# tinycrops/x-transformers-rl

Hardware: AMD Instinct MI355X
Metric: env-steps/s (rollout+update) (higher is better)
Workload: dtype f32; 1 GPU; C3: LunarLander-shaped VecSim (S=8, A=4, hazard 1/64), 1024 episodes x 128 steps per update per GPU, depth-4 d=256 4x16-head gated value-residual world-model policy, batch 128 episodes, 4 epochs, dropout 0.25; no EPO (BASELINE.json configs[2] names no gene pool: one policy, actor / critic heads on [embed | state embed], in = 2d); global_batch=1024, seq_len=128, parallelism=dp1, env_steps=1302236

## Files before the change

### include/xtrl_hip.h

```cpp
#ifndef XTRL_HIP_H
#define XTRL_HIP_H

#include <stdint.h>

#ifdef __cplusplus
extern "C" {
#endif

#define XTRL_OK 0
#define XTRL_E_ARG 1
#define XTRL_E_HIP 2

#define XTRL_ABI_VERSION 25

int xtrl_abi_version(void);
int64_t xtrl_struct_size(const char* name);
const char* xtrl_last_error(void);
const char* xtrl_source_hash(void);

#define XTRL_ACT_NONE 0
#define XTRL_ACT_GELU 1
#define XTRL_ACT_SILU 2
#define XTRL_ACT_RELU 3

int xtrl_gemm_f32(const float* X, int ldx, const float* W, int ldw, const float* bias, const float* ln_gamma,
                  const float* R, int ldr, float* Y, int ldy, const int32_t* t_dev, int64_t y_t_stride, int M,
                  int N, int K, int act, void* stream);

int xtrl_gemm_ex(int trans_a, int trans_b, const float* A, int lda, const float* B, int ldb, const float* bias,
                 float* C, int ldc, int M, int N, int K, float beta, void* stream);

int xtrl_gemm_wgrad(const float* dY, int ldy, const float* X, int ldx, float* dW, int ldw, int M, int N, int K,
                    float beta, float* ws, int64_t ws_floats, void* stream);
int xtrl_gemm_wgrad_db(const float* dY, int ldy, const float* X, int ldx, float* dW, int ldw, int M, int N, int K,
                       float beta, float* ws, int64_t ws_floats, float* db, int db_n0, void* stream);

int xtrl_layernorm_f32(const float* X, int ldx, const float* gamma, float* Y, int ldy, int M, int D, void* stream);

typedef struct XtrlDecodeLayer {
  const float* ln_attn;
  const float* w_qkv;
  const float* b_qkv;
  const float* w_out;
  const float* ln_ff;
  const float* w_ff1;
  const float* b_ff1;
  const float* w_ff2;
  const float* b_ff2;
  float* k_cache;
  float* v_cache;
  const float* w_out_t;
  const uint16_t* w_ff1x;
  const uint16_t* w_ff2x;
  const float* w_qkv_t;
  const float* w_ff1_t;
  const float* w_ff2_t;
  const float* w_ff1f;
  const float* w_ff2f;
  const float* mem_k;
  const float* mem_v;
} XtrlDecodeLayer;

typedef struct XtrlRngState {
  uint64_t seed;
  uint32_t update;
  uint32_t slot_offset;
} XtrlRngState;

typedef struct XtrlDecodeDesc {
  int E, S, A, B, d, L, H, dh, Tmax, G, ff, in_dim, n_qkv;
  int continuous, squash, evolutionary, gate_values, value_residual, learned_mix;
  int rotary_abs;
  int rot_dim;
  int sim_mode;
  int hazard_log2;
  int no_reward_cond;
  int state_only;
  float rs_eps;
  float clamp_lo, clamp_hi; int has_clamp;
  const float* w_pin; const float* b_pin;
  const float* act_emb; const float* act_emb_b;
  const float* reward_embed;
  const float* w_se; const float* b_se;
  const float* ln_final;
  const float* w_h1; const float* b_h1;
  const float* w_h2; const float* b_h2;
  const float* inv_freq;
  const XtrlDecodeLayer* layers;
  const float* rs_mean; const float* rs_var;
  float* state;
  int32_t* prev_action;
  float* prev_action_f;
  float* prev_reward;
  uint8_t* alive;
  int32_t* lens;
  double* cum_reward;
// ... 186 lines not shown
  float* flat;
  float* grad;
  int64_t w_pin, act_emb, act_emb_b, reward_embed, w_se, b_se, ln_final;
  int64_t w_pd, b_pd;
  int64_t w_pred2, b_pred2, w_lat, b_lat, w_h1, b_h1, w_a2, b_a2, w_c2, b_c2;
  const float* inv_freq;
  const float* swr;
  const int32_t* prev_action;
  const int32_t* next_action;
  const float* prev_action_f;
  const float* next_action_f;
  const float* latent;
  const int32_t* lens;
  float* raw;
  float* values;
  float* pred;
  float* done;
  float* x_final;
  float* st_final;
  float* ac_in;
  float* ewa;
  float* zp;
  float* hp;
  float* z1;
  float* h1;
  float* lat_e;
  const float* d_raw;
  const float* d_values;
  const float* d_pred;
  const float* d_done;
  float* dx;
  float* dx2;
  float* dxn;
  float* dff;
  float* dproj;
  float* dog;
  float* dvfirst;
  float* dz1;
  float* dac;
  float* dzp;
  float* dewa;
  float* delta;
  float* part;
  int64_t part_floats;
  float* ws;
  int64_t ws_floats;
  const XtrlTrainLayer* layers;
  void** prof_events;
  double* prof_flops;
  int prof_cap;
  int* prof_n;
  void** grad_events;
  int ld_ff;
  int scratch_per_layer;
  int ff_glu;
  int ld_u2;
  float* glu_dh;
  int qk_norm;
  float xpos_base;
  int rms_norm;
  int Tv;
  int32_t* vrows;
  int32_t* vinv;
  float* ewa_v;
  float* hp_v;
  float* zp_v;
  float* pred_v;
  float* d_pred_v;
  float* dzp_v;
  float* dewa_v;
  float* dq_part;
  int64_t dq_part_floats;
  int packed;
  int32_t* ep_off;
  float* pack_ws;
  int64_t pack_ws_floats;
  int attn_window;
  int Hkv;
  void* wimg;
  int64_t wimg_bytes;
  const XtrlWimgEntry* wimg_tab;
  const XtrlWimgEntry* wimg_tab_host;
  int wimg_n;
  int num_mem_kv;
  int add_zero_kv;
  float* sink_ws;
  int64_t sink_ws_floats;
} XtrlTrainDesc;

struct XtrlWimgEntry {
  int64_t w_off;
  int64_t img_off;
  int N, K, ld, trans_b, BN, blk0;
};
#define XTRL_WIMG_TILE_BYTES(BN) (3 * (BN) * 40 * 2)
int xtrl_train_wimg_plan(const XtrlTrainDesc* desc, XtrlWimgEntry* tab, int cap, int64_t* bytes);
int xtrl_wimg_build(const float* flat, const XtrlWimgEntry* tab_host, const XtrlWimgEntry* tab_dev, int n,
                    void* arena, int64_t arena_bytes, void* stream);

int64_t xtrl_wimg_launch_count(void);

int xtrl_train_forward(const XtrlTrainDesc* desc, void* stream);
int xtrl_train_backward(const XtrlTrainDesc* desc, void* stream);

typedef struct XtrlFractalTrainLevel {
  int64_t w_qkv;
  int64_t w_out, w_gv, w_go;
  int64_t ln1_w, ln1_b, ln2_w, ln2_b, ln3_w, ln3_b;
  int64_t w_ff1, b_ff1, w_ff2, b_ff2, w_proj, b_proj, level_embed;
  float* xin;
  float* qkv;
  float* o;
  float* lse;
  float* s1; float* x1; float* st1;
  float* g;
  float* gv;
  float* s2; float* x2; float* st2;
  float* h; float* u;
  float* s3; float* x3; float* st3;
  float* mean;
} XtrlFractalTrainLevel;

typedef struct XtrlFractalTrainDesc {
  int levels;
  int64_t b_in;
  int64_t g_init, w_gu, b_gu, w_fa0, b_fa0, w_fa2, b_fa2;
  const float* scale_embeds;
  float* le;
  float* bias0;
  float* cat;
  float* hfa;
  float* dxa; float* dxb; float* dmean;
  float* ds;
  float* dga;
  float* dgb;
  float* dgv;
  float* dz;
  float* dqkv;
  float* dob;
  float* dcat;
  float* dhfa;
  const XtrlFractalTrainLevel* level;
} XtrlFractalTrainDesc;

int xtrl_fractal_train_forward(const XtrlTrainDesc* base, const XtrlFractalTrainDesc* f, void* stream);
int xtrl_fractal_train_backward(const XtrlTrainDesc* base, const XtrlFractalTrainDesc* f, void* stream);
int xtrl_linear_gelu_drop(const float* X, int ldx, const float* W, const float* bias, float* Y, int ldy, float* deriv,
                          int ld_deriv, int M, int N, int K, float p, uint64_t seed, uint32_t offset, uint32_t layer,
                          void* stream);
int xtrl_ff_dropout_mask(uint8_t* mask, int M, int N, float p, uint64_t seed, uint32_t offset, uint32_t layer,
                         void* stream);
int xtrl_glu_drop_fwd(const float* u, int ldu, float* h, int ldh, int M, int ff, float p, uint64_t seed,
                      uint32_t offset, uint32_t layer, void* stream);
int xtrl_glu_drop_bwd(const float* dh, int lddh, const float* u, int ldu, float* du, int lddu, int M, int ff, float p,
                      uint64_t seed, uint32_t offset, uint32_t layer, void* stream);
int64_t xtrl_train_part_floats(int T, int b, int d, int A);
int64_t xtrl_train_pack_floats(int T, int S, int A, int n_out, int B);

typedef struct XtrlBatchDesc {
  int N, Tmax, n, b, S, A, B, continuous;
  const float* states;
  const int32_t* actions;
  const float* actions_f;
  const float* rewards;
  const float* logp;
  const uint8_t* bounds;
  const float* values;
  const float* returns;
  const int32_t* lens;
  const int64_t* idx;
  const float* rs_mean;
  const float* rs_var;
  float* swr;
  int32_t* prev_action;
  int32_t* action;
  float* prev_action_f;
  float* action_f;
  float* old_logp;
  float* mb_returns;
  float* old_values;
  uint8_t* dones;
  int32_t* mb_lens;
  float* rs_part;
// ... 78 lines not shown
```

### x-transformers-rl_amd/csrc/attn.hip

```cpp
#include "kernels.h"
#include "philox.h"

namespace xtrl {
namespace {

constexpr int TQ = 64, TK = 64, PST = 66;

typedef float f32x4v __attribute__((ext_vector_type(4)));

__device__ __forceinline__ f32x4v mfma16(float a, float b, f32x4v c) {
  return __builtin_amdgcn_mfma_f32_16x16x4f32(a, b, c, 0, 0, 0);
}

__device__ __forceinline__ uint32_t keep_word(uint64_t seed, uint32_t off, uint32_t c3, int i, int j) {
  const u32x4_t r = philox4x32_10((uint32_t)(i >> 2), (uint32_t)j, off, c3, seed);
  const int w = i & 3;
  return w == 0 ? r.x : (w == 1 ? r.y : (w == 2 ? r.z : r.w));
}
__device__ __forceinline__ uint32_t qword(const u32x4_t& u, int r) {
  return r == 0 ? u.x : (r == 1 ? u.y : (r == 2 ? u.z : u.w));
}
__device__ __forceinline__ uint32_t qbyte(const u32x4_t& u, int word, int r) {
  return (qword(u, word) >> (8 * r)) & 0xFFu;
}
// ... 589 lines not shown
        for (int sub = 0; sub < 4; ++sub) {
          f32x4v st = f32x4v{0.f, 0.f, 0.f, 0.f}, dpt = f32x4v{0.f, 0.f, 0.f, 0.f};
#pragma unroll
          for (int s = 0; s < KS; ++s) {
            st = mfma16(ka[s], Qs[16 * sub + lr][4 * s + lg], st);
            dpt = mfma16(va[s], dOs[16 * sub + lr][4 * s + lg], dpt);
          }
          const int il = 16 * sub + lr, i = qt * TQ + il;
          uint32_t kq[4] = {0u, 0u, 0u, 0u};
          if (a.thresh8) {
            const u32x4_t kb = philox4x32_10((uint32_t)(i >> 2), (uint32_t)((j0 >> 6) * 16 + 4 * lg + (lr & 3)), off,
                                             a.c3, a.seed);
            const uint32_t wd = qword(kb, w);
#pragma unroll
            for (int c = 0; c < 4; ++c) kq[c] = (wd >> (8 * c)) & 0xFFu;
            quad_transpose(kq, lane);
          } else if (a.thresh) {
            const u32x4_t kb = philox4x32_10((uint32_t)(i >> 2), (uint32_t)(j0 + 16 * w + 4 * lg + (lr & 3)), off,
                                             a.c3, a.seed);
            kq[0] = kb.x;
            kq[1] = kb.y;
            kq[2] = kb.z;
            kq[3] = kb.w;
            quad_transpose(kq, lane);
          }
#pragma unroll
          for (int r = 0; r < 4; ++r) {
            const int j = j0 + 16 * w + 4 * lg + r;
            const bool ok = ((unsigned)(i - j) <= (unsigned)a.window) && (j < len) && (i < n);
            const float p = ok ? expf(st[r] * a.scale - Ls[il]) : 0.f;
            float z = 1.f;
            if (a.thresh8 && ok) z = (kq[r] >= a.thresh8) ? a.inv_keep : 0.f;
            else if (a.thresh && ok) z = (kq[r] >= a.thresh) ? a.inv_keep : 0.f;
            Ps[w][4 * lg + r][il] = p * z;
            dsr[sub][r] = p * (dpt[r] * z - Dls[il]);
          }
        }
        wave_sync();
#pragma unroll
        for (int d = 0; d < ND; ++d)
#pragma unroll
          for (int s = 0; s < TQ / 4; ++s) dv[d] = mfma16(Ps[w][lr][4 * s + lg], dOs[4 * s + lg][16 * d + lr], dv[d]);
        wave_sync();
#pragma unroll
        for (int sub = 0; sub < 4; ++sub)
#pragma unroll
          for (int r = 0; r < 4; ++r) Ps[w][4 * lg + r][16 * sub + lr] = dsr[sub][r];
        wave_sync();
#pragma unroll
        for (int d = 0; d < ND; ++d)
#pragma unroll
          for (int s = 0; s < TQ / 4; ++s) dk[d] = mfma16(Ps[w][lr][4 * s + lg], Qs[4 * s + lg][16 * d + lr], dk[d]);
        __syncthreads();
#pragma unroll
        for (int d = 0; d < ND; ++d)
#pragma unroll
          for (int s = 0; s < TK / 4; ++s) {
            const int j = 4 * s + lg;
            dq[qt][d] = mfma16(Ps[j >> 4][j & 15][16 * w + lr], Ks[j][16 * d + lr], dq[qt][d]);
          }
      }
    }
#pragma unroll
    for (int r = 0; r < 4; ++r) {
      const int j = j0 + 16 * w + 4 * lg + r;
      if (j < n) {
#pragma unroll
        for (int d = 0; d < ND; ++d) {
          a.dK[gb + (int64_t)j * gsi + 16 * d + lr] = dk[d][r] * a.scale;
          a.dV[gb + (int64_t)j * gsi + 16 * d + lr] = dv[d][r];
        }
      }
    }
  }
#pragma unroll
  for (int qt = 0; qt < FB_QT; ++qt)
#pragma unroll
    for (int r = 0; r < 4; ++r) {
      const int i = qt * TQ + 16 * w + 4 * lg + r;
      if (qt < nq && i < n) {
#pragma unroll
        for (int d = 0; d < ND; ++d) a.dQ[gb + (int64_t)i * gsi + 16 * d + lr] = dq[qt][d][r] * a.scale;
      }
    }
}

__device__ __forceinline__ float keep_scale(const AttnArgs& a, uint32_t off, int i, int j) {
  if (a.thresh8) {
    const u32x4_t r = philox4x32_10((uint32_t)(i >> 2), (uint32_t)(16 * (j >> 6) + (j & 15)), off, a.c3, a.seed);
    return qbyte(r, (j >> 4) & 3, i & 3) >= a.thresh8 ? a.inv_keep : 0.f;
  }
  if (a.thresh) return keep_word(a.seed, off, a.c3, i, j) >= a.thresh ? a.inv_keep : 0.f;
  return 1.f;
}

template <int DH, bool GQA = false>
__global__ __launch_bounds__(256) void k_attn_dead_fwd(const AttnArgs a) {
  const int c = threadIdx.x % DH, i = blockIdx.x * (256 / DH) + threadIdx.x / DH;
  const int bh = blockIdx.y, b = bh / a.H, h = bh - b * a.H, n = a.n;
  const int len = a.lens[b];
  if (len <= 0 || i >= n || i < len + a.window) return;
  const int64_t ob = ebase(a, a.out, b) + h * a.out.sh;
  const int64_t ib = GQA ? ebase(a, a.kv, b) + kv_head_of(h, a.Hkv) * a.kv.sh : ebase(a, a.in, b) + h * a.in.sh;
  const int isi = GQA ? a.kv.si : a.in.si;
  const uint32_t off = a.offset + (uint32_t)bh;
  float acc = 0.f;
  for (int j0 = 0; j0 < n; j0 += DH) {
    const float zm = j0 + c < n ? keep_scale(a, off, i, j0 + c) : 0.f;
    for (int jj = 0; jj < DH; ++jj) {
      const float z = __shfl(zm, jj, DH);
      if (j0 + jj < n) acc += z * a.V[ib + (int64_t)(j0 + jj) * isi + c];
    }
  }
  const float ov = acc / (float)n;
  const int64_t at = ob + (int64_t)i * a.out.si + c;
  a.Oout[at] = ov;
  if (a.OGout) a.OGout[at] = ov * sigmoidf_(a.G[ebase(a, a.gate, b) + h * a.gate.sh + (int64_t)i * a.gate.si + c]);
}

template <int DH, bool GQA = false>
__global__ __launch_bounds__(256) void k_attn_dead_bwd(const AttnArgs a) {
  const int c = threadIdx.x % DH, j = blockIdx.x * (256 / DH) + threadIdx.x / DH;
  const int nhk = GQA ? a.Hkv : a.H;
  const int b = blockIdx.y / nhk, hk = blockIdx.y - b * nhk, n = a.n;
  const int len = a.lens[b];
  if (len <= 0 || j >= n) return;
  const int64_t gb = GQA ? ebase(a, a.kvgrad, b) + hk * a.kvgrad.sh : ebase(a, a.grad, b) + hk * a.grad.sh;
  const int gsi = GQA ? a.kvgrad.si : a.grad.si;
  float acc = 0.f;
  for (int g = 0; g < (GQA ? a.H : 1); ++g) {
    const int h = GQA ? g : hk;
    if (GQA && kv_head_of(h, a.Hkv) != hk) continue;
    const int64_t ob = ebase(a, a.out, b) + h * a.out.sh;
    const uint32_t off = a.offset + (uint32_t)(b * a.H + h);
    for (int i0 = len + a.window; i0 < n; i0 += DH) {
      const float zm = i0 + c < n ? keep_scale(a, off, i0 + c, j) : 0.f;
      for (int ii = 0; ii < DH; ++ii) {
        const float z = __shfl(zm, ii, DH);
        if (i0 + ii < n) acc += z * a.dO[ob + (int64_t)(i0 + ii) * a.out.si + c];
      }
    }
  }
  if (len + a.window < n) a.dV[gb + (int64_t)j * gsi + c] += acc / (float)n;
}

constexpr int SB_ROWS = 256, SB_ST = kMaxMemKV + 1;
template <int DH>
__global__ __launch_bounds__(256) void k_attn_sink_bwd(const AttnArgs a) {
  constexpr int EU = kMaxMemKV * DH / 256;
  __shared__ float mk[kMaxMemKV][DH], mv[kMaxMemKV][DH];
  __shared__ float dSs[SB_ROWS][SB_ST], Pds[SB_ROWS][SB_ST];
  const int tid = threadIdx.x;
  const int bh = blockIdx.x, b = bh / a.H, h = bh - b * a.H, ns = a.n;
  const int len = a.lens[b];
  const int n = a.ep_off ? min(len, ns) : ns;
  const int M = a.M;
  const int64_t ib = ebase(a, a.in, b) + h * a.in.sh, ob = ebase(a, a.out, b) + h * a.out.sh, gb = ebase(a, a.grad, b) + h * a.grad.sh;
  const int isi = a.in.si, osi = a.out.si, gsi = a.grad.si;
  const uint32_t off = a.offset + (uint32_t)bh;
  {
    const int64_t mb = (int64_t)kv_head_of(h, a.Hkv) * M * DH;
    for (int x = tid; x < M * DH; x += 256) {
      mk[x / DH][x % DH] = a.MK[mb + x];
      mv[x / DH][x % DH] = a.MV[mb + x];
    }
  }
// ... 170 lines not shown
  a.LSEout = lse;
  a.G = gate;
  a.OGout = og;
  const bool gqa = is_gqa(p);
  dim3 grid((p.n + TQ - 1) / TQ, p.b * p.H);
  if (attn_has_sinks(p)) {
    if (p.dh == 16) hipLaunchKernelGGL((k_attn_fwd<16, true, true>), grid, dim3(256), 0, s, a);
    else if (p.dh == 32) hipLaunchKernelGGL((k_attn_fwd<32, true, true>), grid, dim3(256), 0, s, a);
    else hipLaunchKernelGGL((k_attn_fwd<64, true, true>), grid, dim3(256), 0, s, a);
  } else {
    XTRL_ATTN_LAUNCH_DH(k_attn_fwd, gqa, p.dh, grid);
  }
  XTRL_LAUNCHED("attn_fwd");
  if (has_dead_rows(p)) {
    dim3 dgrid((p.n + 256 / p.dh - 1) / (256 / p.dh), p.b * p.H);
    XTRL_ATTN_LAUNCH_DH(k_attn_dead_fwd, gqa, p.dh, dgrid);
    XTRL_LAUNCHED("attn_dead_fwd");
  }
  return XTRL_OK;
}

int attn_bwd_ex(const AttnProblem& p, const float* q, const float* k, const float* v, const float* o,
                const float* lse, const float* dout, float* dq, float* dk, float* dv, float* delta_ws,
                hipStream_t s) {
  AttnArgs a{};
  if (int rc = fill_args(a, p)) return rc;
  XTRL_REQUIRE(q && k && v && o && lse && dout && dq && dk && dv && delta_ws, "attn_bwd: null operand");
  XTRL_REQUIRE(p.causal, "attn_bwd: bidirectional attention is forward-only");
  a.Q = q;
  a.K = k;
  a.V = v;
  a.O = o;
  a.LSE = lse;
  a.dO = dout;
  a.Dl = delta_ws;
  a.Dout = delta_ws;
  a.dQ = dq;
  a.dK = dk;
  a.dV = dv;
  dim3 grid((p.n + TQ - 1) / TQ, p.b * p.H);
  const int64_t part_need = attn_dq_part_floats(p.b, p.H, p.n, p.dh);
  const bool gqa = is_gqa(p);
  if (gqa) {
    dim3 kgrid((p.n + TK - 1) / TK, p.b * p.Hkv);
    if (p.dh == 16 && p.dq_part && p.dq_part_floats >= part_need && attn_fused_bwd_on()) {
      a.dQp = p.dq_part;
      hipLaunchKernelGGL((k_attn_bwd_dkdv<16, true, true, true>), kgrid, dim3(256), 0, s, a);
      const int64_t units = (int64_t)p.b * p.H * p.n * 4;
      hipLaunchKernelGGL(k_attn_dq_reduce<16>, dim3((unsigned)((units + 255) / 256)), dim3(256), 0, s, a, p.b * p.H);
    } else {
      if (p.dh == 16) hipLaunchKernelGGL((k_attn_bwd_dkdv<16, false, true, true>), kgrid, dim3(256), 0, s, a);
      else if (p.dh == 32) hipLaunchKernelGGL((k_attn_bwd_dkdv<32, false, true, true>), kgrid, dim3(256), 0, s, a);
      else hipLaunchKernelGGL((k_attn_bwd_dkdv<64, false, true, true>), kgrid, dim3(256), 0, s, a);
      XTRL_ATTN_LAUNCH_DH(k_attn_bwd_dq, true, p.dh, grid);
    }
  } else if (p.dh == 16 && p.n <= FB_MAXN && attn_fused_bwd_on()) {
    hipLaunchKernelGGL(k_attn_bwd_fused<16>, dim3(p.b * p.H), dim3(256), 0, s, a);
  } else if (p.dh == 16 && p.dq_part && p.dq_part_floats >= part_need && attn_fused_bwd_on()) {
    a.dQp = p.dq_part;
    if (p.window > 0) hipLaunchKernelGGL((k_attn_bwd_dkdv<16, true>), grid, dim3(256), 0, s, a);
    else hipLaunchKernelGGL((k_attn_bwd_dkdv<16, true, false>), grid, dim3(256), 0, s, a);
    const int64_t units = (int64_t)p.b * p.H * p.n * 4;
    hipLaunchKernelGGL(k_attn_dq_reduce<16>, dim3((unsigned)((units + 255) / 256)), dim3(256), 0, s, a, p.b * p.H);
  } else if (p.dh == 16) {
    if (p.window > 0) hipLaunchKernelGGL(k_attn_bwd_dkdv<16>, grid, dim3(256), 0, s, a);
    else hipLaunchKernelGGL((k_attn_bwd_dkdv<16, false, false>), grid, dim3(256), 0, s, a);
    hipLaunchKernelGGL(k_attn_bwd_dq<16>, grid, dim3(256), 0, s, a);
  } else if (p.dh == 32) {
    hipLaunchKernelGGL(k_attn_bwd_dkdv<32>, grid, dim3(256), 0, s, a);
    hipLaunchKernelGGL(k_attn_bwd_dq<32>, grid, dim3(256), 0, s, a);
  } else {
    hipLaunchKernelGGL(k_attn_bwd_dkdv<64>, grid, dim3(256), 0, s, a);
    hipLaunchKernelGGL(k_attn_bwd_dq<64>, grid, dim3(256), 0, s, a);
  }
  XTRL_LAUNCHED("attn_bwd");
  if (has_dead_rows(p)) {
    dim3 dgrid((p.n + 256 / p.dh - 1) / (256 / p.dh), p.b * (gqa ? p.Hkv : p.H));
    XTRL_ATTN_LAUNCH_DH(k_attn_dead_bwd, gqa, p.dh, dgrid);
    XTRL_LAUNCHED("attn_dead_bwd");
  }
  return sink_bwd(a, p, s);
}

int64_t attn_dq_part_floats(int b, int H, int n, int dh) {
  return (int64_t)((n + TK - 1) / TK) * b * H * n * dh;
}

int64_t attn_sink_ws_floats(int b, int H, int mem_kv, int dh) { return 2 * (int64_t)b * H * mem_kv * dh; }

AttnProblem contiguous_problem(const int32_t* lens, int b, int H, int n, int dh, float scale, float p, uint64_t seed,
                               uint32_t offset, uint32_t sub, int window, int Hkv) {
  AttnProblem pr{b, H, n, dh, lens, scale, p, seed, offset, {}, {}, {}, {}};
  pr.sub = sub;
  pr.window = window;
  pr.in = pr.out = pr.grad = attn_layout_bhnd(H, n, dh);
  pr.Hkv = Hkv;
  if (Hkv > 0) pr.kv = pr.kvgrad = attn_layout_bhnd(Hkv, n, dh);
  return pr;
}

}

extern "C" int xtrl_attn_fwd_sink(const float* q, const float* k, const float* v, const int32_t* lens, float* o,
                                  float* lse, const float* mem_k, const float* mem_v, int b, int H, int Hkv, int n,
                                  int dh, float scale, float dropout_p, uint64_t seed, uint32_t offset, uint32_t sub,
                                  int window, int num_mem_kv, int add_zero_kv, void* stream) {
  XTRL_REQUIRE(Hkv >= 1, "attn_fwd: kv heads %d < 1", Hkv);
  xtrl::AttnProblem pr = xtrl::contiguous_problem(lens, b, H, n, dh, scale, dropout_p, seed, offset, sub, window, Hkv);
  pr.mem_k = mem_k;
  pr.mem_v = mem_v;
  pr.mem_kv = num_mem_kv;
  pr.zero_kv = add_zero_kv;
  return xtrl::attn_fwd_ex(pr, q, k, v, o, lse, nullptr, nullptr, xtrl::as_stream(stream));
}

extern "C" int xtrl_attn_fwd_gqa(const float* q, const float* k, const float* v, const int32_t* lens, float* o,
                                 float* lse, int b, int H, int Hkv, int n, int dh, float scale, float dropout_p,
                                 uint64_t seed, uint32_t offset, uint32_t sub, int window, void* stream) {
  return xtrl_attn_fwd_sink(q, k, v, lens, o, lse, nullptr, nullptr, b, H, Hkv, n, dh, scale, dropout_p, seed, offset,
                            sub, window, 0, 0, stream);
}

extern "C" int xtrl_attn_fwd_win(const float* q, const float* k, const float* v, const int32_t* lens, float* o,
                                 float* lse, int b, int H, int n, int dh, float scale, float dropout_p, uint64_t seed,
                                 uint32_t offset, uint32_t sub, int window, void* stream) {
  return xtrl_attn_fwd_gqa(q, k, v, lens, o, lse, b, H, H, n, dh, scale, dropout_p, seed, offset, sub, window, stream);
}

extern "C" int xtrl_attn_fwd(const float* q, const float* k, const float* v, const int32_t* lens, float* o,
                             float* lse, int b, int H, int n, int dh, float scale, float dropout_p, uint64_t seed,
                             uint32_t offset, uint32_t sub, void* stream) {
  return xtrl_attn_fwd_win(q, k, v, lens, o, lse, b, H, n, dh, scale, dropout_p, seed, offset, sub, 0, stream);
}

extern "C" int64_t xtrl_attn_bwd_part_floats(int b, int H, int n, int dh) {
  return xtrl::attn_dq_part_floats(b, H, n, dh);
}

extern "C" int64_t xtrl_attn_sink_ws_floats(int b, int H, int num_mem_kv, int dh) {
  return xtrl::attn_sink_ws_floats(b, H, num_mem_kv, dh);
}

extern "C" int xtrl_attn_bwd_part_sink(const float* q, const float* k, const float* v, const int32_t* lens,
                                       const float* o, const float* lse, const float* dout, float* dq, float* dk,
                                       float* dv, float* delta_ws, float* dq_part, int64_t dq_part_floats,
                                       const float* mem_k, const float* mem_v, float* dmem_k, float* dmem_v,
                                       float* sink_ws, int64_t sink_ws_floats, int b, int H, int Hkv, int n, int dh,
                                       float scale, float dropout_p, uint64_t seed, uint32_t offset, uint32_t sub,
                                       int window, int num_mem_kv, int add_zero_kv, void* stream) {
  XTRL_REQUIRE(Hkv >= 1, "attn_bwd: kv heads %d < 1", Hkv);
  xtrl::AttnProblem pr = xtrl::contiguous_problem(lens, b, H, n, dh, scale, dropout_p, seed, offset, sub, window, Hkv);
  pr.dq_part = dq_part;
  pr.dq_part_floats = dq_part_floats;
  pr.mem_k = mem_k;
  pr.mem_v = mem_v;
  pr.mem_kv = num_mem_kv;
  pr.zero_kv = add_zero_kv;
  pr.dmem_k = dmem_k;
  pr.dmem_v = dmem_v;
  pr.sink_ws = sink_ws;
  pr.sink_ws_floats = sink_ws_floats;
  return xtrl::attn_bwd_ex(pr, q, k, v, o, lse, dout, dq, dk, dv, delta_ws, xtrl::as_stream(stream));
}

extern "C" int xtrl_attn_bwd_sink(const float* q, const float* k, const float* v, const int32_t* lens, const float* o,
                                  const float* lse, const float* dout, float* dq, float* dk, float* dv, float* delta_ws,
                                  const float* mem_k, const float* mem_v, float* dmem_k, float* dmem_v, float* sink_ws,
                                  int64_t sink_ws_floats, int b, int H, int Hkv, int n, int dh, float scale,
                                  float dropout_p, uint64_t seed, uint32_t offset, uint32_t sub, int window,
                                  int num_mem_kv, int add_zero_kv, void* stream) {
  return xtrl_attn_bwd_part_sink(q, k, v, lens, o, lse, dout, dq, dk, dv, delta_ws, nullptr, 0, mem_k, mem_v, dmem_k,
                                 dmem_v, sink_ws, sink_ws_floats, b, H, Hkv, n, dh, scale, dropout_p, seed, offset, sub,
                                 window, num_mem_kv, add_zero_kv, stream);
}

extern "C" int xtrl_attn_bwd_part_gqa(const float* q, const float* k, const float* v, const int32_t* lens,
                                      const float* o, const float* lse, const float* dout, float* dq, float* dk,
                                      float* dv, float* delta_ws, float* dq_part, int64_t dq_part_floats, int b, int H,
                                      int Hkv, int n, int dh, float scale, float dropout_p, uint64_t seed,
                                      uint32_t offset, uint32_t sub, int window, void* stream) {
  return xtrl_attn_bwd_part_sink(q, k, v, lens, o, lse, dout, dq, dk, dv, delta_ws, dq_part, dq_part_floats, nullptr,
                                 nullptr, nullptr, nullptr, nullptr, 0, b, H, Hkv, n, dh, scale, dropout_p, seed,
                                 offset, sub, window, 0, 0, stream);
}

extern "C" int xtrl_attn_bwd_part_win(const float* q, const float* k, const float* v, const int32_t* lens,
                                      const float* o, const float* lse, const float* dout, float* dq, float* dk,
                                      float* dv, float* delta_ws, float* dq_part, int64_t dq_part_floats, int b, int H,
                                      int n, int dh, float scale, float dropout_p, uint64_t seed, uint32_t offset,
                                      uint32_t sub, int window, void* stream) {
  return xtrl_attn_bwd_part_gqa(q, k, v, lens, o, lse, dout, dq, dk, dv, delta_ws, dq_part, dq_part_floats, b, H, H, n,
                                dh, scale, dropout_p, seed, offset, sub, window, stream);
}

extern "C" int xtrl_attn_bwd_part(const float* q, const float* k, const float* v, const int32_t* lens, const float* o,
                                  const float* lse, const float* dout, float* dq, float* dk, float* dv, float* delta_ws,
                                  float* dq_part, int64_t dq_part_floats, int b, int H, int n, int dh, float scale,
                                  float dropout_p, uint64_t seed, uint32_t offset, uint32_t sub, void* stream) {
  return xtrl_attn_bwd_part_win(q, k, v, lens, o, lse, dout, dq, dk, dv, delta_ws, dq_part, dq_part_floats, b, H, n, dh,
                                scale, dropout_p, seed, offset, sub, 0, stream);
}

extern "C" int xtrl_attn_bwd_gqa(const float* q, const float* k, const float* v, const int32_t* lens, const float* o,
                                 const float* lse, const float* dout, float* dq, float* dk, float* dv, float* delta_ws,
                                 int b, int H, int Hkv, int n, int dh, float scale, float dropout_p, uint64_t seed,
                                 uint32_t offset, uint32_t sub, int window, void* stream) {
  return xtrl_attn_bwd_sink(q, k, v, lens, o, lse, dout, dq, dk, dv, delta_ws, nullptr, nullptr, nullptr, nullptr,
                            nullptr, 0, b, H, Hkv, n, dh, scale, dropout_p, seed, offset, sub, window, 0, 0, stream);
}

extern "C" int xtrl_attn_bwd_win(const float* q, const float* k, const float* v, const int32_t* lens, const float* o,
                                 const float* lse, const float* dout, float* dq, float* dk, float* dv, float* delta_ws,
                                 int b, int H, int n, int dh, float scale, float dropout_p, uint64_t seed,
                                 uint32_t offset, uint32_t sub, int window, void* stream) {
  return xtrl_attn_bwd_gqa(q, k, v, lens, o, lse, dout, dq, dk, dv, delta_ws, b, H, H, n, dh, scale, dropout_p, seed,
                           offset, sub, window, stream);
}

extern "C" int xtrl_attn_bwd(const float* q, const float* k, const float* v, const int32_t* lens, const float* o,
                             const float* lse, const float* dout, float* dq, float* dk, float* dv, float* delta_ws,
                             int b, int H, int n, int dh, float scale, float dropout_p, uint64_t seed,
                             uint32_t offset, uint32_t sub, void* stream) {
  return xtrl_attn_bwd_win(q, k, v, lens, o, lse, dout, dq, dk, dv, delta_ws, b, H, n, dh, scale, dropout_p, seed,
                           offset, sub, 0, stream);
}

extern "C" int xtrl_attn_fwd_tokens(const float* q, int ldq, const float* k, int ldk, const float* v, int ldv,
                                    const int32_t* lens, float* o, int ldo, float* lse, int b, int H, int n, int dh,
                                    float scale, int causal, void* stream) {
  XTRL_REQUIRE(ldq == ldk && ldk == ldv, "attn_fwd_tokens: q, k, v share one row stride (got %d %d %d)", ldq, ldk,
               ldv);
  xtrl::AttnProblem pr{b, H, n, dh, lens, scale, 0.f, 0, 0, {}, {}, {}, {}};
  pr.in = xtrl::attn_layout_tokens(n, ldq, dh);
  pr.out = xtrl::attn_layout_tokens(n, ldo, dh);
  pr.causal = causal;
  return xtrl::attn_fwd_ex(pr, q, k, v, o, lse, nullptr, nullptr, (hipStream_t)stream);
}
```

### x-transformers-rl_amd/csrc/common.h

```cpp
#pragma once
#include <hip/hip_runtime.h>
#include <stdint.h>

#include "../../include/xtrl_hip.h"

namespace xtrl {

constexpr int kWave = 64;

typedef float f32x4 __attribute__((ext_vector_type(4)));
typedef float f32x16 __attribute__((ext_vector_type(16)));

void set_error(const char* fmt, ...);
int check_launch(const char* what);

#define XTRL_REQUIRE(cond, ...)                                                                   \
  do {                                                                                            \
    if (!(cond)) {                                                                                \
      ::xtrl::set_error(__VA_ARGS__);                                                             \
      return XTRL_E_ARG;                                                                          \
    }                                                                                             \
  } while (0)

#define XTRL_LAUNCHED(what)                                                                       \
// ... 24 lines not shown
__device__ __forceinline__ float dpp_mov(float v) {
  return __builtin_bit_cast(float, __builtin_amdgcn_update_dpp(0, __builtin_bit_cast(int, v), CTRL, 0xF, 0xF, false));
}
#ifndef XTRL_DPP_BCAST
#define XTRL_DPP_BCAST 1
#endif
template <int CTRL, int ROWS>
__device__ __forceinline__ float dpp_bcast(float v, float fill) {
  return __builtin_bit_cast(float, __builtin_amdgcn_update_dpp(__builtin_bit_cast(int, fill), __builtin_bit_cast(int, v),
                                                                CTRL, ROWS, 0xF, false));
}
__device__ __forceinline__ float wave_sum_dpp(float v) {
  v += dpp_mov<0xB1>(v);
  v += dpp_mov<0x4E>(v);
  v += dpp_mov<0x141>(v);
  v += dpp_mov<0x140>(v);
#if XTRL_DPP_BCAST
  v += dpp_bcast<0x142, 0xA>(v, 0.f);
  v += dpp_bcast<0x143, 0xC>(v, 0.f);
  return __builtin_bit_cast(float, __builtin_amdgcn_readlane(__builtin_bit_cast(int, v), 63));
#else
  v += __shfl_xor(v, 16, kWave);
  v += __shfl_xor(v, 32, kWave);
  return v;
#endif
}
__device__ __forceinline__ float wave_max_dpp(float v) {
  v = fmaxf(v, dpp_mov<0xB1>(v));
  v = fmaxf(v, dpp_mov<0x4E>(v));
  v = fmaxf(v, dpp_mov<0x141>(v));
  v = fmaxf(v, dpp_mov<0x140>(v));
#if XTRL_DPP_BCAST
  v = fmaxf(v, dpp_bcast<0x142, 0xA>(v, -INFINITY));
  v = fmaxf(v, dpp_bcast<0x143, 0xC>(v, -INFINITY));
  return __builtin_bit_cast(float, __builtin_amdgcn_readlane(__builtin_bit_cast(int, v), 63));
#else
  v = fmaxf(v, __shfl_xor(v, 16, kWave));
  v = fmaxf(v, __shfl_xor(v, 32, kWave));
  return v;
#endif
}

template <typename T>
__device__ __forceinline__ void quad_transpose(T (&x)[4], int lane) {
  const bool b1 = (lane & 2) != 0, b0 = (lane & 1) != 0;
  T s0 = b1 ? x[0] : x[2], s1 = b1 ? x[1] : x[3];
  T r0 = __shfl_xor(s0, 2, kWave), r1 = __shfl_xor(s1, 2, kWave);
  if (b1) {
    x[0] = r0;
    x[1] = r1;
  } else {
    x[2] = r0;
    x[3] = r1;
  }
  s0 = b0 ? x[0] : x[1];
  s1 = b0 ? x[2] : x[3];
  r0 = __shfl_xor(s0, 1, kWave);
  r1 = __shfl_xor(s1, 1, kWave);
  if (b0) {
    x[0] = r0;
    x[2] = r1;
  } else {
    x[1] = r0;
    x[3] = r1;
  }
}

__device__ __forceinline__ void wave_sync() {
  __builtin_amdgcn_fence(__ATOMIC_RELEASE, "wavefront");
  __builtin_amdgcn_wave_barrier();
  __builtin_amdgcn_fence(__ATOMIC_ACQUIRE, "wavefront");
}

__device__ __forceinline__ float norm_rstd(float sq, float d, bool rms) {
  return rms ? sqrtf(d) / fmaxf(sqrtf(sq), 1e-12f) : 1.0f / sqrtf(sq / d + 1e-5f);
}
__device__ __forceinline__ float sigmoidf_(float x) { return 1.0f / (1.0f + expf(-x)); }
__device__ __forceinline__ float geluf_(float x) { return 0.5f * x * (1.0f + erff(x * 0.70710678118654752f)); }
__device__ __forceinline__ float siluf_(float x) { return x / (1.0f + expf(-x)); }
__device__ __forceinline__ float lerpf_(float s, float e, float w) {
  return (fabsf(w) < 0.5f) ? s + w * (e - s) : e - (e - s) * (1.0f - w);
}

}
```

### x-transformers-rl_amd/csrc/kernels.h

```cpp
#pragma once
#include "common.h"

namespace xtrl {

enum GemmEpi : int {
  EPI_NONE = 0,
  EPI_GELU = 1,
  EPI_SILU = 2,
  EPI_GELU_DROP = 3,
  EPI_SILU_SAVE = 4,
  EPI_MUL_AUX = 5,
  EPI_RELU = 8,
  EPI_DGATE = 7,
  EPI_RES_LN = 9,
  EPI_LN_BWD = 10,
  EPI_MASK_POS = 11,
  EPI_LN_BWD2 = 12,
};

struct GemmArgs {
  const float* A = nullptr;
  const float* B = nullptr;
  const float* bias = nullptr;
  const float* gamma = nullptr;
// ... 92 lines not shown
  const float* gamma = nullptr; int ln_k = 0;
  int ln_rms = 0;
  const float* R = nullptr; int ldr = 0;
  float* C = nullptr; int ldc = 0;
  const int32_t* row_map = nullptr;
  const int32_t* m_dev = nullptr;
  int M = 0, N = 0, K = 0;
  int n_split = 1 << 30;
  float* C2 = nullptr; int ldc2 = 0;
  const int32_t* row_map2 = nullptr;
};
int dgemm_run(const DGemmArgs& a, int rows, int epi, hipStream_t s);
int dg_ks(int N, int K);
int64_t dgemm_packed_floats(int N, int K);
int dgemm_pack(const float* W, int ldw, int N, int K, float* Wp, hipStream_t s);

void rows_add_launch(const float* x, int ldx, const float* v, float* y, int ldy, int M, int D, hipStream_t s);
void add_layernorm_launch(const float* x, int ldx, const float* r, int ldr, const float* g, const float* b, float* y,
                          int ldy, int M, int D, float eps, hipStream_t s);

inline uint32_t dropout_thresh8(float p) {
  const double t = (double)p * 256.0;
  return (t >= 1.0 && t <= 255.0 && t == (double)(int)t) ? (uint32_t)t : 0u;
}

inline uint32_t dropout_thresh(float p) {
  if (!(p > 0.f)) return 0u;
  const double th = (double)p * 4294967296.0;
  const uint32_t t = (uint32_t)fmin(th, 4294967295.0);
  return t ? t : 1u;
}

struct AttnLayout {
  int64_t sb, sh;
  int si;
};
inline AttnLayout attn_layout_bhnd(int H, int n, int dh) {
  return AttnLayout{(int64_t)H * n * dh, (int64_t)n * dh, dh};
}
inline AttnLayout attn_layout_tokens(int n, int ld, int dh) {
  return AttnLayout{(int64_t)n * ld, (int64_t)dh, ld};
}

struct AttnProblem {
  int b, H, n, dh;
  const int32_t* lens;
  float scale, dropout;
  uint64_t seed;
  uint32_t offset;
  AttnLayout in, out, grad;
  AttnLayout gate;
  int causal = 1;
  uint32_t sub = 0;
  float* dq_part = nullptr;
  int64_t dq_part_floats = 0;
  const int32_t* ep_off = nullptr;
  int window = 0;
  int Hkv = 0;
  AttnLayout kv = {}, kvgrad = {};
  const float *mem_k = nullptr, *mem_v = nullptr;
  int mem_kv = 0, zero_kv = 0;
  float *dmem_k = nullptr, *dmem_v = nullptr;
  int dmem_accum = 0;
  float* sink_ws = nullptr;
  int64_t sink_ws_floats = 0;
};
constexpr int kMaxMemKV = 16;
inline bool attn_has_sinks(const AttnProblem& p) { return p.mem_kv > 0 || p.zero_kv != 0; }
int64_t attn_sink_ws_floats(int b, int H, int mem_kv, int dh);
__host__ __device__ inline int kv_head_of(int h, int Hkv) { return h % Hkv; }
__host__ __device__ inline bool kv_head_owner(int h, int Hkv) {
  for (int x = 0; x < h; ++x)
    if (kv_head_of(x, Hkv) == kv_head_of(h, Hkv)) return false;
  return true;
}
int64_t attn_dq_part_floats(int b, int H, int n, int dh);

int attn_fwd_ex(const AttnProblem& p, const float* q, const float* k, const float* v, float* o, float* lse,
                const float* gate, float* og, hipStream_t s);
int attn_bwd_ex(const AttnProblem& p, const float* q, const float* k, const float* v, const float* o,
                const float* lse, const float* dout, float* dq, float* dk, float* dv, float* delta_ws,
                hipStream_t s);

}
```

### x-transformers-rl_amd/csrc/train.hip

```cpp
#include <cstdlib>
#include <vector>

#include <hip/hip_ext.h>

#include "kernels.h"
#include "philox.h"

namespace xtrl {
namespace {

constexpr int kMaxDPerLane = 8;

__device__ __forceinline__ float ldg(const float* p) { return __builtin_nontemporal_load(p); }

struct EmbedArgs {
  const float *swr, *w_pin, *act_emb, *act_emb_b, *reward_embed, *w_se, *b_se, *lat_e, *prev_af, *next_af;
  const int32_t *prev_a, *next_a;
  float *x0, *ac_in, *ewa;
  int T, n, S, A, d, in_dim, continuous, evolutionary;
  float keep;
  const float* ln_g;
  float *xn, *st;
  int rms;
  const int32_t* rows;
};

constexpr int EMB_TOK = 32, EMB_U = 8, EMB_MAXS = 32;
template <int S_>
__global__ __launch_bounds__(256) void k_embed(const EmbedArgs a) {
  constexpr int MS = S_ > 0 ? S_ : EMB_MAXS;
  const int S = S_ > 0 ? S_ : a.S;
  for (int c = threadIdx.x; c < a.d; c += 256) {
    float wp[MS], ws[MS];
#pragma unroll
    for (int s = 0; s < MS; ++s) {
      wp[s] = s < S ? a.w_pin[(int64_t)c * S + s] : 0.f;
      ws[s] = s < S ? a.w_se[(int64_t)c * S + s] : 0.f;
    }
    const float bse = a.b_se[c], re = a.reward_embed[c];
    const float bemb = a.continuous ? a.act_emb_b[c] : 0.f;
    for (int t0 = blockIdx.x * EMB_TOK; t0 < min(a.T, (int)(blockIdx.x + 1) * EMB_TOK); t0 += EMB_U) {
      float pin[EMB_U], se[EMB_U], rw[EMB_U], ap[EMB_U], an[EMB_U], le[EMB_U];
#pragma unroll
      for (int u = 0; u < EMB_U; ++u) {
        const int t = min(t0 + u, a.T - 1);
        const float* st = a.swr + (int64_t)t * (S + 1);
        float sp = 0.f, ss = 0.f;
#pragma unroll
        for (int s = 0; s < MS; ++s) {
          if (s < S) {
            const float x = st[s];
            sp += x * wp[s];
            ss += x * ws[s];
          }
        }
        pin[u] = sp;
        se[u] = ss + bse;
        rw[u] = st[S];
        if (a.continuous) {
          const float* w = a.act_emb + (int64_t)c * a.A;
          float p = 0.f, q = 0.f;
          for (int k = 0; k < a.A; ++k) {
            p += a.prev_af[(int64_t)t * a.A + k] * w[k];
            q += a.next_af[(int64_t)t * a.A + k] * w[k];
          }
          ap[u] = p + bemb;
          an[u] = q + bemb;
        } else {
          const int p = a.prev_a[t], q = a.next_a[t];
          ap[u] = p >= 0 ? a.act_emb[(int64_t)p * a.d + c] : 0.f;
          an[u] = q >= 0 ? a.act_emb[(int64_t)q * a.d + c] : 0.f;
        }
        le[u] = a.evolutionary ? a.lat_e[(int64_t)((a.rows ? a.rows[t] : t) / a.n) * a.d + c] : 0.f;
      }
#pragma unroll
      for (int u = 0; u < EMB_U; ++u) {
        const int t = t0 + u;
        if (t >= a.T) break;
        a.x0[(int64_t)t * a.d + c] = pin[u] + (ap[u] + (rw[u] * re) * a.keep);
        a.ac_in[(int64_t)t * a.in_dim + a.d + c] = se[u];
        a.ewa[(int64_t)t * 2 * a.d + a.d + c] = an[u];
        if (a.evolutionary) a.ac_in[(int64_t)t * a.in_dim + 2 * a.d + c] = le[u];
      }
// ... 157 lines not shown
    db[k] = 0.f;
  }
  const int r0 = blockIdx.x * LN_ROWS;
  for (int rb = w * LN_R; rb < LN_ROWS; rb += LN_WAVES * LN_R) {
    float g[LN_R][DPL], xv[LN_R][DPL], dr[LN_R][DPL], rs[LN_R], mu[LN_R];
#pragma unroll
    for (int q = 0; q < LN_R; ++q) {
      const int t = r0 + rb + q;
      const bool ok = t < T;
      mu[q] = ok ? stats[2 * t] : 0.f;
      rs[q] = ok ? stats[2 * t + 1] : 0.f;
#pragma unroll
      for (int k = 0; k < DPL; ++k) {
        const int c = lane + 64 * k;
        const bool in = ok && c < d;
        float gv = in ? s1 * g1[(int64_t)t * ldg1 + c] : 0.f;
        if (g2 && in) gv += g2[(int64_t)t * ldg2 + c];
        g[q][k] = gv;
        xv[q][k] = in ? x[(int64_t)t * d + c] : 0.f;
        dr[q][k] = (dres && in) ? dres[(int64_t)t * d + c] : 0.f;
      }
    }
#pragma unroll
    for (int q = 0; q < LN_R; ++q) {
      const int t = r0 + rb + q;
      float sa = 0.f, sb = 0.f;
      float gm[DPL], xh[DPL];
#pragma unroll
      for (int k = 0; k < DPL; ++k) {
        const int c = lane + 64 * k;
        xh[k] = c < d ? (xv[q][k] - mu[q]) * rs[q] : 0.f;
        gm[k] = g[q][k] * gam[k];
        dg[k] += g[q][k] * xh[k];
        db[k] += g[q][k];
        sa += gm[k];
        sb += gm[k] * xh[k];
      }
      const float ma = rms ? 0.f : wave_sum(sa) / (float)d, mb = wave_sum(sb) / (float)d;
      if (t < T) {
#pragma unroll
        for (int k = 0; k < DPL; ++k) {
          const int c = lane + 64 * k;
          if (c < d) {
            float v = rs[q] * (gm[k] - ma - xh[k] * mb);
            if (dres) v += dr[q][k];
            dx[(int64_t)t * d + c] = v;
          }
        }
      }
    }
  }
#pragma unroll
  for (int k = 0; k < DPL; ++k) red[w][lane + 64 * k] = dg[k];
  __syncthreads();
  for (int c = threadIdx.x; c < d; c += 64 * LN_WAVES) {
    float v = 0.f;
#pragma unroll
    for (int j = 0; j < LN_WAVES; ++j) v += red[j][c];
    part[(int64_t)blockIdx.x * pstride + c] = v;
  }
  if (!part_b) return;
  __syncthreads();
#pragma unroll
  for (int k = 0; k < DPL; ++k) red[w][lane + 64 * k] = db[k];
  __syncthreads();
  for (int c = threadIdx.x; c < d; c += 64 * LN_WAVES) {
    float v = 0.f;
#pragma unroll
    for (int j = 0; j < LN_WAVES; ++j) v += red[j][c];
    part_b[(int64_t)blockIdx.x * pstride + c] = v;
  }
}

struct PrepArgs {
  const float* proj;
  const float* vfirst;
  float* qkv;
  const float* inv_freq;
  int T, n, H, dh, I, n_qkv, ld_vfirst, rot_dim, mix_col;
  int qk_norm;
  float xpos_base;
  const int32_t* rows;
  int Ikv;
};

__device__ __forceinline__ void qkv_segment(int col, int I, int Ikv, int& seg, int& within) {
  seg = col < I ? 0 : (col < I + Ikv ? 1 : 2);
  within = col - (seg == 0 ? 0 : (seg == 1 ? I : I + Ikv));
}

__device__ __forceinline__ float xpos_factor(int j, int rot, int pos, int n, float base) {
  const float sc = ((float)j + 0.4f * (float)rot) / (1.4f * (float)rot);
  return powf(sc, (float)(pos - n / 2) / base);
}

__device__ __forceinline__ float head_norm(float2 x, int dh) {
  float ss = x.x * x.x + x.y * x.y;
  for (int o = dh >> 2; o > 0; o >>= 1) ss += __shfl_xor(ss, o, 64);
  return fmaxf(sqrtf(ss), 1e-12f);
}

constexpr int PREP_T = 128;
__global__ __launch_bounds__(PREP_T) void k_qkv_prep(const PrepArgs a) {
  const int P = (a.I + 2 * a.Ikv) / 2;
  const int pair = blockIdx.x * PREP_T + threadIdx.x;
  if (pair >= P) return;
  const int t = a.rows ? (int)blockIdx.y : blockIdx.z * a.n + blockIdx.y;
  const int pos = a.rows ? a.rows[t] % a.n : (int)blockIdx.y, col = 2 * pair;
  int seg, within;
  qkv_segment(col, a.I, a.Ikv, seg, within);
  const int h = within / a.dh, j = within - h * a.dh;
  float2 x = *reinterpret_cast<const float2*>(a.proj + (int64_t)t * a.n_qkv + col);
  float2 y;
  if (seg < 2) {
    if (a.qk_norm) {
      const float nrm = head_norm(x, a.dh);
      x.x = x.x / nrm;
      x.y = x.y / nrm;
    }
    if (j < a.rot_dim) {
      const float f = (float)pos * a.inv_freq[j >> 1];
      float sn, cs;
      sincosf(f, &sn, &cs);
      y.x = x.x * cs + (-x.y) * sn;
      y.y = x.y * cs + x.x * sn;
      if (a.xpos_base > 0.f) {
        const float xf = xpos_factor(j, a.rot_dim, pos, a.n, a.xpos_base);
        const float sf = seg == 0 ? xf : 1.0f / xf;
        y.x *= sf;
        y.y *= sf;
      }
    } else {
      y = x;
    }
  } else if (a.mix_col >= 0) {
    const float m = sigmoidf_(a.proj[(int64_t)t * a.n_qkv + a.mix_col + h]);
    const float2 vf = *reinterpret_cast<const float2*>(a.vfirst + (int64_t)t * a.ld_vfirst + a.I + a.Ikv + within);
    y.x = lerpf_(x.x, vf.x, m);
    y.y = lerpf_(x.y, vf.y, m);
  } else {
    y = x;
  }
  *reinterpret_cast<float2*>(a.qkv + (int64_t)t * (a.I + 2 * a.Ikv) + col) = y;
}

struct PrepBwdArgs {
  float* dproj;
  const float* proj;
  const float* vfirst;
  float* dvfirst;
  const float* inv_freq;
  int T, n, H, dh, I, n_qkv, ld_vfirst, rot_dim, mix_col, first_layer, accumulate;
  int qk_norm;
  float xpos_base;
  const int32_t* rows;
  int Ikv;
};

__global__ __launch_bounds__(PREP_T) void k_qkv_prep_bwd(const PrepBwdArgs a) {
  const int P = (a.I + 2 * a.Ikv) / 2;
  const int pair0 = blockIdx.x * PREP_T + threadIdx.x;
  const bool valid = pair0 < P;
  const int pair = valid ? pair0 : 0;
  const int t = a.rows ? (int)blockIdx.y : blockIdx.z * a.n + blockIdx.y;
  const int pos = a.rows ? a.rows[t] % a.n : (int)blockIdx.y, col = 2 * pair;
  int seg, within;
  qkv_segment(col, a.I, a.Ikv, seg, within);
  const int h = within / a.dh, j = within - h * a.dh;
  float* g = a.dproj + (int64_t)t * a.n_qkv + col;
  float dm = 0.f, m = 0.f;
  float2 gqk = make_float2(0.f, 0.f);
  if (valid) {
    float2 gv = *reinterpret_cast<float2*>(g);
    if (seg < 2) {
      if (j < a.rot_dim) {
        const float f = (float)pos * a.inv_freq[j >> 1];
        float sn, cs;
        sincosf(f, &sn, &cs);
        float g0 = gv.x, g1 = gv.y;
        if (a.xpos_base > 0.f) {
          const float xf = xpos_factor(j, a.rot_dim, pos, a.n, a.xpos_base);
          const float sf = seg == 0 ? xf : 1.0f / xf;
          g0 *= sf;
          g1 *= sf;
        }
        gv.x = g0 * cs + g1 * sn;
        gv.y = g1 * cs + (-g0) * sn;
        if (!a.qk_norm) *reinterpret_cast<float2*>(g) = gv;
      }
      gqk = gv;
    } else {
      float2* dvf = reinterpret_cast<float2*>(a.dvfirst + (int64_t)t * a.Ikv + within);
      if (a.mix_col >= 0) {
        const float* pr = a.proj + (int64_t)t * a.n_qkv;
        m = sigmoidf_(pr[a.mix_col + h]);
        const float2 v = *reinterpret_cast<const float2*>(pr + col);
        const float2 vf = *reinterpret_cast<const float2*>(a.vfirst + (int64_t)t * a.ld_vfirst + col);
        dm = gv.x * (vf.x - v.x) + gv.y * (vf.y - v.y);
        float2 f;
        f.x = gv.x * m;
        f.y = gv.y * m;
        if (a.accumulate) {
          const float2 o = *dvf;
          f.x += o.x;
          f.y += o.y;
        }
        *dvf = f;
        gv.x = gv.x * (1.0f - m);
        gv.y = gv.y * (1.0f - m);
        *reinterpret_cast<float2*>(g) = gv;
      } else if (a.first_layer && a.accumulate) {
        const float2 o = *dvf;
        gv.x += o.x;
        gv.y += o.y;
        *reinterpret_cast<float2*>(g) = gv;
      }
    }
  }
  if (a.qk_norm) {
    const float2 x = valid ? *reinterpret_cast<const float2*>(a.proj + (int64_t)t * a.n_qkv + col) : make_float2(0.f, 0.f);
    float ss = x.x * x.x + x.y * x.y;
    for (int o = a.dh >> 2; o > 0; o >>= 1) ss += __shfl_xor(ss, o, 64);
    const float r = sqrtf(ss), nrm = fmaxf(r, 1e-12f);
    const float hx = x.x / nrm, hy = x.y / nrm;
    const float2 gg = gqk;
    float dot = hx * gg.x + hy * gg.y;
    for (int o = a.dh >> 2; o > 0; o >>= 1) dot += __shfl_xor(dot, o, 64);
    if (valid && seg < 2) {
      float2 dx;
      if (r >= 1e-12f) {
        dx.x = (gg.x - hx * dot) / nrm;
        dx.y = (gg.y - hy * dot) / nrm;
      } else {
        dx.x = gg.x / nrm;
        dx.y = gg.y / nrm;
      }
      *reinterpret_cast<float2*>(g) = dx;
    }
  }
  if (a.mix_col >= 0) {
    for (int o = a.dh >> 2; o > 0; o >>= 1) dm += __shfl_xor(dm, o, 64);
    if (valid && seg == 2 && j == 0) a.dproj[(int64_t)t * a.n_qkv + a.mix_col + h] = dm * (1.0f - m) * m;
  }
}

__global__ __launch_bounds__(256) void k_colsum_part(const float* src, int ld, int rows, int cols, int chunk_rows,
                                                     const float* rw, int ld_rw, float rw_scale, float* part) {
  const int c = blockIdx.x * 256 + threadIdx.x;
  if (c >= cols) return;
  const int r0 = blockIdx.y * chunk_rows, r1 = min(rows, r0 + chunk_rows);
  float s = 0.f;
  if (rw) {
#pragma unroll 8
    for (int r = r0; r < r1; ++r) s += src[(int64_t)r * ld + c] * (rw[(int64_t)r * ld_rw] * rw_scale);
  } else {
#pragma unroll 8
    for (int r = r0; r < r1; ++r) s += src[(int64_t)r * ld + c];
  }
  part[(int64_t)blockIdx.y * cols + c] = s;
}

constexpr int CS_WAVES = 16, CS_COLS = 16, CS_G = 64 * CS_WAVES / CS_COLS;
__device__ __forceinline__ void colsum_final_body(const float* part, int chunks, int cols, float* dst, int bx) {
  __shared__ float red[CS_G][CS_COLS];
  const int lane = threadIdx.x & 63, w = threadIdx.x >> 6;
  const int cl = lane % CS_COLS, g = w * (64 / CS_COLS) + lane / CS_COLS;
  const int c = bx * CS_COLS + cl;
  float s0 = 0.f, s1 = 0.f, s2 = 0.f, s3 = 0.f;
  if (c < cols) {
    int k = g;
    for (; k + 3 * CS_G < chunks; k += 4 * CS_G) {
      s0 += part[(int64_t)k * cols + c];
      s1 += part[(int64_t)(k + CS_G) * cols + c];
      s2 += part[(int64_t)(k + 2 * CS_G) * cols + c];
      s3 += part[(int64_t)(k + 3 * CS_G) * cols + c];
    }
    for (; k < chunks; k += CS_G) s0 += part[(int64_t)k * cols + c];
  }
  red[g][cl] = (s0 + s1) + (s2 + s3);
  __syncthreads();
  if (threadIdx.x < CS_COLS) {
    const int cc = bx * CS_COLS + threadIdx.x;
    if (cc < cols) {
      float v = 0.f;
#pragma unroll 8
      for (int j2 = 0; j2 < CS_G; ++j2) v += red[j2][threadIdx.x];
      dst[cc] += v;
    }
  }
}
__global__ __launch_bounds__(64 * CS_WAVES) void k_colsum_final(const float* part, int chunks, int cols, float* dst) {
  colsum_final_body(part, chunks, cols, dst, blockIdx.x);
}

constexpr int kMaxColsumJobs = 16;
struct ColsumJobs {
  const float* part[kMaxColsumJobs];
  float* dst[kMaxColsumJobs];
  int chunks[kMaxColsumJobs];
  int cols[kMaxColsumJobs];
};
__global__ __launch_bounds__(64 * CS_WAVES) void k_colsum_final_multi(const ColsumJobs J) {
  const int j = blockIdx.y;
  if ((int)blockIdx.x * CS_COLS >= J.cols[j]) return;
  colsum_final_body(J.part[j], J.chunks[j], J.cols[j], J.dst[j], blockIdx.x);
}
struct ColsumQueue {
  ColsumJobs J{};
  int n = 0, max_cols = 0;
  float* base = nullptr;
  int64_t cap = 0, used = 0;
  float* take_or_flush(int chunks, int cols, float* dst, hipStream_t s, int* rc) {
    *rc = XTRL_OK;
    float* P = take(chunks, cols, dst);
    if (!P && base && n > 0) {
      if ((*rc = flush(s))) return nullptr;
      P = take(chunks, cols, dst);
    }
    return P;
  }
  float* take(int chunks, int cols, float* dst) {
    const int64_t need = (int64_t)chunks * cols;
    if (!base || n == kMaxColsumJobs || used + need > cap) return nullptr;
    float* P = base + used;
    used += (need + 3) & ~(int64_t)3;
// ... 420 lines not shown
bool ln_fusable(const XtrlTrainDesc* D) {
  static const bool on = [] {
    const char* e = getenv("XTRL_FUSED_LN");
    return !(e && atoi(e) == 0);
  }();
  if (!on || D->d % 4 || D->d > 256 || (D->H * D->dh) % 4 || D->ff % 4 || D->in_dim % 4) return false;
  for (int li = 0; li < D->L; ++li)
    if (D->layers[li].n_qkv % 4) return false;
  return true;
}

int linear_res_ln(const Ctx& c, const float* A, int lda, const float* W, const float* bias, const float* R,
                  float* x_out, int K, const float* gamma, float* y1, int ld1, float* y2, int ld2, float* st) {
  const int d = c.D->d;
  GemmArgs g;
  g.A = A; g.lda = lda; g.B = W; g.ldb = K; g.bias = bias; g.C = x_out; g.ldc = d; g.M = c.T; g.N = d; g.K = K;
  g.R = R; g.ldr = d; g.ln_g = gamma; g.ln_y1 = y1; g.ln_ld1 = ld1; g.ln_y2 = y2; g.ln_ld2 = ld2; g.ln_stats = st;
  g.ln_rms = c.D->rms_norm;
  c.img(g, 0, EPI_RES_LN);
  return gemm_run(g, 0, 0, EPI_RES_LN, c.s);
}

int dgrad_ln_bwd(const Ctx& c, const float* dY, int ldy, const float* W, int N, const float* x, const float* st,
                 const float* gamma, const float* dres, float* dx, float* dgamma, ColsumQueue* cq = nullptr) {
  const int d = c.D->d, nb = (c.T + gemm_ln_rows(d) - 1) / gemm_ln_rows(d);
  XTRL_REQUIRE((int64_t)nb * d <= c.D->part_floats, "train: partial-sum workspace too small");
  int rc = XTRL_OK;
  float* P = cq ? cq->take_or_flush(nb, d, dgamma, c.s, &rc) : nullptr;
  if (rc) return rc;
  GemmArgs g;
  g.A = dY; g.lda = ldy; g.B = W; g.ldb = d; g.C = dx; g.ldc = d; g.M = c.T; g.N = d; g.K = N;
  g.ln_g = gamma; g.ln_x = x; g.ln_stats = const_cast<float*>(st); g.ln_dres = dres; g.ln_part = P ? P : c.D->part;
  g.ln_rms = c.D->rms_norm;
  c.img(g, 1, EPI_LN_BWD);
  if ((rc = gemm_run(g, 0, 1, EPI_LN_BWD, c.s))) return rc;
  if (!P)
    hipLaunchKernelGGL(k_colsum_final, dim3(blocks(d, CS_COLS)), dim3(64 * CS_WAVES), 0, c.s, c.D->part, nb, d, dgamma);
  XTRL_LAUNCHED("train dgrad_ln_bwd");
  return XTRL_OK;
}

inline int kv_heads(const XtrlTrainDesc* D) { return D->Hkv > 0 ? D->Hkv : D->H; }
inline int kv_inner(const XtrlTrainDesc* D) { return kv_heads(D) * D->dh; }

AttnProblem attn_problem(const Ctx& c, const XtrlTrainLayer& Ly, int li) {
  const XtrlTrainDesc* D = c.D;
  const int I = D->H * D->dh;
  AttnProblem p{};
  p.b = D->b;
  p.H = D->H;
  p.n = D->n;
  p.dh = D->dh;
  p.lens = D->lens;
  p.scale = D->attn_scale;
  p.dropout = D->dropout;
  p.seed = D->seed;
  p.offset = D->attn_offset;
  p.sub = (uint32_t)li;
  p.in = attn_layout_tokens(D->n, I + 2 * kv_inner(D), D->dh);
  p.out = attn_layout_tokens(D->n, I, D->dh);
  p.grad = attn_layout_tokens(D->n, Ly.n_qkv, D->dh);
  p.gate = attn_layout_tokens(D->n, Ly.n_qkv, D->dh);
  p.ep_off = D->packed ? D->ep_off : nullptr;
  p.dq_part = D->dq_part;
  p.dq_part_floats = D->dq_part_floats;
  p.window = D->attn_window;
  p.Hkv = kv_heads(D);
  p.kv = p.in;
  p.kvgrad = p.grad;
  p.mem_kv = D->num_mem_kv;
  p.zero_kv = D->add_zero_kv;
  if (D->num_mem_kv > 0) {
    p.mem_k = c.P(Ly.mem_k);
    p.mem_v = c.P(Ly.mem_v);
    p.dmem_k = c.G(Ly.mem_k);
    p.dmem_v = c.G(Ly.mem_v);
    p.dmem_accum = 1;
    p.sink_ws = D->sink_ws;
    p.sink_ws_floats = D->sink_ws_floats;
  }
  return p;
}

int validate(const XtrlTrainDesc* D) {
  XTRL_REQUIRE(D && D->layers && D->flat && D->grad, "train: null descriptor / layers / parameters");
  XTRL_REQUIRE(D->b > 0 && D->n > 0 && D->d > 0 && D->L > 0 && D->H > 0 && D->dh > 0, "train: bad sizes");
  XTRL_REQUIRE(D->d <= 64 * kMaxDPerLane, "train: d = %d > %d unsupported", D->d, 64 * kMaxDPerLane);
  XTRL_REQUIRE(D->dh % 2 == 0 && D->rot_dim <= D->dh, "train: bad rotary dims");
  XTRL_REQUIRE(D->Hkv >= 0 && D->Hkv <= D->H && D->H % kv_heads(D) == 0, "train: Hkv %d must divide H %d (0 = H)", D->Hkv,
               D->H);
  XTRL_REQUIRE(D->num_mem_kv >= 0 && D->num_mem_kv <= kMaxMemKV, "train: num_mem_kv %d outside [0, %d]", D->num_mem_kv,
               kMaxMemKV);
  for (int li = 0; li < D->L; ++li)
    XTRL_REQUIRE(D->num_mem_kv == 0 || (D->layers[li].mem_k >= 0 && D->layers[li].mem_v >= 0 && D->sink_ws),
                 "train: layer %d num_mem_kv %d without mem_k / mem_v offsets or the sink workspace", li, D->num_mem_kv);
  for (int li = 0; li < D->L; ++li)
    XTRL_REQUIRE(D->layers[li].n_qkv == D->H * D->dh + 2 * kv_inner(D) + (D->gate_values ? D->H * D->dh : 0) +
                                            (D->layers[li].mix ? kv_heads(D) : 0),
                 "train: layer %d n_qkv %d is not I + 2 Ikv (+ I gate) (+ Hkv mix)", li, D->layers[li].n_qkv);
  XTRL_REQUIRE(D->in_dim == D->d * (D->evolutionary ? 3 : 2), "train: in_dim mismatch");
  XTRL_REQUIRE(D->ld_ff == 0 || (D->ld_ff >= D->ff && D->ld_ff % 4 == 0), "train: ld_ff %d (ff %d)", D->ld_ff, D->ff);
  XTRL_REQUIRE(!D->ff_glu || (D->ld_u2 >= 2 * D->ff && D->ld_u2 % 4 == 0 && D->glu_dh),
               "train: ff_glu needs ld_u2 >= 2 ff (a multiple of 4) and glu_dh");
  XTRL_REQUIRE(!D->evolutionary || (D->latent && D->lat_e), "train: evolutionary needs latent buffers");
  XTRL_REQUIRE(D->S <= EMB_MAXS, "train: state_dim %d > %d unsupported", D->S, EMB_MAXS);
  XTRL_REQUIRE(D->continuous || D->A <= EMB_MAXA, "train: %d discrete actions > %d unsupported", D->A, EMB_MAXA);
  XTRL_REQUIRE(D->continuous ? (D->prev_action_f && D->next_action_f) : (D->prev_action && D->next_action),
               "train: missing action inputs");
  return XTRL_OK;
}

}

namespace {
constexpr int VR_MAXB = 4096;
__global__ __launch_bounds__(1024) void k_valid_rows(const int32_t* lens, int b, int n, int Tv, int32_t* vrows,
                                                     int32_t* vinv, int32_t* ep_off = nullptr) {
  __shared__ int off[VR_MAXB + 1];
  for (int e = threadIdx.x; e < b; e += 1024) off[e + 1] = min(max(lens[e], 0), n);
  __syncthreads();
  if (threadIdx.x == 0) {
    off[0] = 0;
    for (int e = 0; e < b; ++e) off[e + 1] += off[e];
  }
  __syncthreads();
  for (int r = threadIdx.x; r < b * n; r += 1024) {
    const int e = r / n, t = r - e * n;
    const int j = off[e] + t;
    if (t < off[e + 1] - off[e] && j < Tv) {
      vrows[j] = r;
      vinv[r] = j;
    } else {
      vinv[r] = -1;
    }
  }
  for (int j = off[b] + threadIdx.x; j < Tv; j += 1024) vrows[j] = 0;
  if (ep_off)
    for (int e = threadIdx.x; e <= b; e += 1024) ep_off[e] = min(off[e], Tv);
}
template <int V>
__global__ void k_gather_rows(const float* src, int lds, const int32_t* rows, int nr, int cols, float* dst, int ldd) {
  const int cv = cols / V;
  const int64_t i = (int64_t)blockIdx.x * 256 + threadIdx.x;
  if (i >= (int64_t)nr * cv) return;
  const int r = (int)(i / cv), c = V * (int)(i - (int64_t)r * cv);
  const float* sp = src + (int64_t)rows[r] * lds + c;
  float* dp = dst + (int64_t)r * ldd + c;
  if constexpr (V == 4) *reinterpret_cast<float4*>(dp) = *reinterpret_cast<const float4*>(sp);
  else *dp = *sp;
}
template <int V>
__global__ void k_scatter_rows(const float* src, int lds, const int32_t* inv, int T, int cols, float* dst, int ldd) {
  const int cv = cols / V;
  const int64_t i = (int64_t)blockIdx.x * 256 + threadIdx.x;
  if (i >= (int64_t)T * cv) return;
  const int r = (int)(i / cv), c = V * (int)(i - (int64_t)r * cv);
  const int j = inv[r];
  float* dp = dst + (int64_t)r * ldd + c;
  if constexpr (V == 4)
    *reinterpret_cast<float4*>(dp) = j >= 0 ? *reinterpret_cast<const float4*>(src + (int64_t)j * lds + c)
                                            : make_float4(0.f, 0.f, 0.f, 0.f);
  else
    *dp = j >= 0 ? src[(int64_t)j * lds + c] : 0.f;
}
bool vec4_ok(const float* a, int lda, const float* b, int ldb, int cols) {
  return cols % 4 == 0 && lda % 4 == 0 && ldb % 4 == 0 && ((uintptr_t)a % 16) == 0 && ((uintptr_t)b % 16) == 0;
// ... 79 lines not shown
    return rc;
  if ((rc = F.fork())) return rc;
  if ((rc = wgrad(cw, D->dz1, 4 * d, D->ac_in, D->in_dim, c.G(D->w_h1), T, 4 * d, D->in_dim, c.G(D->b_h1)))) return rc;
  if (embed_cols) {
    if ((rc = linear_dgrad(c, D->dz1, 4 * d, c.P(D->w_h1), D->dac, D->in_dim, T, 4 * d, D->in_dim, EPI_NONE))) return rc;
  } else {
    GemmArgs g;
    g.A = D->dz1; g.lda = 4 * d; g.B = c.P(D->w_h1) + d; g.ldb = D->in_dim; g.C = D->dac + d; g.ldc = D->in_dim;
    g.M = T; g.N = D->in_dim - d; g.K = 4 * d;
    c.img(g, 1, EPI_NONE);
    if ((rc = gemm_run(g, 0, 1, EPI_NONE, c.s))) return rc;
  }
  if ((rc = F.fork())) return rc;
  if ((rc = wgrad(cw, D->dac + d, D->in_dim, D->swr, D->S + 1, c.G(D->w_se), T, d, D->S, c.G(D->b_se)))) return rc;
  if (D->evolutionary) {
    XTRL_REQUIRE((int64_t)D->b * d <= D->part_floats, "train: partial-sum workspace too small");
    hipLaunchKernelGGL(k_latent_grad, dim3(D->b, (d + 63) / 64), dim3(64 * LG_G), 0, s, D->dac, D->in_dim, 2 * d,
                       D->b, D->n, d, D->part, D->packed ? D->ep_off : nullptr);
    hipLaunchKernelGGL(k_latent_wgrad, dim3(blocks(d * (D->G + 1), 256)), dim3(256), 0, s, D->part, D->latent, D->b,
                       d, D->G, c.G(D->w_lat), c.G(D->b_lat));
    XTRL_LAUNCHED("train latent grad");
  }
  if (cmp) {
    const int Tv = D->Tv;
    if ((rc = wgrad(cw, D->d_pred_v, S1x2, D->hp_v, ldp, c.G(D->w_pred2), Tv, S1x2, d, c.G(D->b_pred2)))) return rc;
    if ((rc = linear_dgrad(c, D->d_pred_v, S1x2, c.P(D->w_pred2), D->dzp_v, ldp, Tv, S1x2, d, EPI_MUL_AUX, D->zp_v,
                           ldp)))
      return rc;
    if ((rc = F.fork())) return rc;
    if ((rc = wgrad(cw, D->dzp_v, ldp, D->ewa_v, 2 * d, c.G(D->w_pd), Tv, d + 1, 2 * d, c.G(D->b_pd)))) return rc;
    if ((rc = linear_dgrad(c, D->dzp_v, ldp, c.P(D->w_pd), D->dewa_v, 2 * d, Tv, d + 1, 2 * d, EPI_NONE))) return rc;
    scatter_rows(D->dewa_v, 2 * d, D->vinv, T, 2 * d, D->dewa, 2 * d, s);
    XTRL_LAUNCHED("train heads backward (compact)");
    return XTRL_OK;
  }
  if ((rc = wgrad(cw, D->d_pred, S1x2, D->hp, ldp, c.G(D->w_pred2), T, S1x2, d, c.G(D->b_pred2)))) return rc;
  if ((rc = linear_dgrad(c, D->d_pred, S1x2, c.P(D->w_pred2), D->dzp, ldp, T, S1x2, d, EPI_MUL_AUX, D->zp, ldp))) return rc;
  hipLaunchKernelGGL(k_copy_col, dim3(blocks(T, 256)), dim3(256), 0, s, D->d_done, 1, D->dzp + d, ldp, T);
  if ((rc = F.fork())) return rc;
  if ((rc = wgrad(cw, D->dzp, ldp, D->ewa, 2 * d, c.G(D->w_pd), T, d + 1, 2 * d, c.G(D->b_pd)))) return rc;
  if ((rc = linear_dgrad(c, D->dzp, ldp, c.P(D->w_pd), D->dewa, 2 * d, T, d + 1, 2 * d, EPI_NONE))) return rc;
  return XTRL_OK;
}

int train_forward_rows(const XtrlTrainDesc* D, int Trows, hipStream_t s) {
  if (int rc = validate(D)) return rc;
  const Ctx c{D, s, Trows};
  const int32_t* rows = D->packed ? D->vrows : nullptr;
  const int T = c.T, d = D->d, I = D->H * D->dh, ff = D->ff, lf = ld_ff(D);
  const int Ikv = kv_inner(D), nq3 = I + 2 * Ikv;
  int rc;
  if (D->wimg && D->wimg_tab && D->wimg_tab_host && D->wimg_n > 0 && wimg_enabled())
    if ((rc = wimg_build(D->flat, D->wimg_tab_host, D->wimg_tab, D->wimg_n, D->wimg, D->wimg_bytes, s))) return rc;
  if (D->evolutionary) {
    hipLaunchKernelGGL(k_latent_embed, dim3(blocks(D->b * d, 256)), dim3(256), 0, s, D->latent, c.P(D->w_lat),
                       c.P(D->b_lat), D->lat_e, D->b, D->G, d);
  }
  EmbedArgs ea{D->swr, c.P(D->w_pin), c.P(D->act_emb), c.P(D->act_emb_b), c.P(D->reward_embed), c.P(D->w_se),
               c.P(D->b_se), D->lat_e, D->prev_action_f, D->next_action_f, D->prev_action, D->next_action,
               D->layers[0].x_attn, D->ac_in, D->ewa, T, D->n, D->S, D->A, d, D->in_dim, D->continuous,
               D->evolutionary, D->reward_keep, nullptr, nullptr, nullptr, D->rms_norm, rows};
  const bool fuse = ln_fusable(D);
  if (fuse) {
    const XtrlTrainLayer& L0 = D->layers[0];
    ea.ln_g = c.P(L0.ln_attn);
    ea.xn = L0.xn_attn;
    ea.st = L0.st_attn;
    if (D->S == 8) hipLaunchKernelGGL(k_embed_ln<8>, dim3(blocks(T, EMB_LN_TOK)), dim3(256), 0, s, ea);
    else hipLaunchKernelGGL(k_embed_ln<0>, dim3(blocks(T, EMB_LN_TOK)), dim3(256), 0, s, ea);
  } else if (D->S == 8) {
    hipLaunchKernelGGL(k_embed<8>, dim3(blocks(T, EMB_TOK)), dim3(256), 0, s, ea);
  } else {
    hipLaunchKernelGGL(k_embed<0>, dim3(blocks(T, EMB_TOK)), dim3(256), 0, s, ea);
  }
  XTRL_LAUNCHED("train embed");
  for (int li = 0; li < D->L; ++li) {
    const XtrlTrainLayer& Ly = D->layers[li];
    if (!fuse)
      if ((rc = ln_fwd(c, Ly.x_attn, c.P(Ly.ln_attn), Ly.xn_attn, d, nullptr, 0, Ly.st_attn))) return rc;
    if ((rc = linear_fwd(c, Ly.xn_attn, d, c.P(Ly.w_proj), c.P(Ly.b_proj), Ly.proj, Ly.n_qkv, T, Ly.n_qkv, d,
                         EPI_NONE, nullptr, nullptr, 0, 1 << 30, nq3)))
      return rc;
    const int mix_col = Ly.mix ? nq3 + (D->gate_values ? I : 0) : -1;
    PrepArgs pa{Ly.proj, D->layers[0].proj, Ly.qkv, D->inv_freq, T, D->n, D->H, D->dh, I, Ly.n_qkv,
                D->layers[0].n_qkv, D->rot_dim, mix_col, D->qk_norm, D->xpos_base, rows, Ikv};
    const dim3 pg = rows ? dim3(blocks(nq3 / 2, PREP_T), T) : dim3(blocks(nq3 / 2, PREP_T), D->n, D->b);
    hipLaunchKernelGGL(k_qkv_prep, pg, dim3(PREP_T), 0, s, pa);
    XTRL_LAUNCHED("train qkv_prep");
    const AttnProblem ap = attn_problem(c, Ly, li);
    if ((rc = attn_fwd_ex(ap, Ly.qkv, Ly.qkv + I, Ly.qkv + I + Ikv, Ly.o, Ly.lse,
                          D->gate_values ? Ly.proj + nq3 : nullptr, D->gate_values ? Ly.og : nullptr, s)))
      return rc;
    if (fuse) {
      if ((rc = linear_res_ln(c, D->gate_values ? Ly.og : Ly.o, I, c.P(Ly.w_out), nullptr, Ly.x_attn, Ly.x_ff, I,
                              c.P(Ly.ln_ff), Ly.xn_ff, d, nullptr, 0, Ly.st_ff)))
        return rc;
    } else {
      if ((rc = linear_fwd(c, D->gate_values ? Ly.og : Ly.o, I, c.P(Ly.w_out), nullptr, Ly.x_ff, d, T, d, I, EPI_NONE,
                           Ly.x_attn)))
        return rc;
      if ((rc = ln_fwd(c, Ly.x_ff, c.P(Ly.ln_ff), Ly.xn_ff, d, nullptr, 0, Ly.st_ff))) return rc;
    }
    if (D->ff_glu) {
      if ((rc = linear_fwd(c, Ly.xn_ff, d, c.P(Ly.w_ff1), c.P(Ly.b_ff1), Ly.u, D->ld_u2, T, 2 * ff, d, EPI_NONE)))
        return rc;
      if ((rc = glu_fwd(Ly.u, D->ld_u2, Ly.hd, lf, T, ff, D->dropout, D->seed, D->ff_offset, (uint32_t)li, s)))
        return rc;
    } else if ((rc = linear_fwd(c, Ly.xn_ff, d, c.P(Ly.w_ff1), c.P(Ly.b_ff1), Ly.hd, lf, T, ff, d, EPI_GELU_DROP,
                                nullptr, Ly.u, lf, 1 << 30, 0, D->ff_offset, (uint32_t)li))) {
      return rc;
    }
    float* x_out = li + 1 < D->L ? D->layers[li + 1].x_attn : D->x_final;
    if (fuse && li + 1 < D->L) {
      const XtrlTrainLayer& Ln = D->layers[li + 1];
      if ((rc = linear_res_ln(c, Ly.hd, lf, c.P(Ly.w_ff2), c.P(Ly.b_ff2), Ly.x_ff, x_out, ff, c.P(Ln.ln_attn),
                              Ln.xn_attn, d, nullptr, 0, Ln.st_attn)))
        return rc;
    } else if (fuse) {
      if ((rc = linear_res_ln(c, Ly.hd, lf, c.P(Ly.w_ff2), c.P(Ly.b_ff2), Ly.x_ff, x_out, ff, c.P(D->ln_final),
                              D->ac_in, D->in_dim, D->ewa, 2 * d, D->st_final)))
        return rc;
    } else {
      if ((rc = linear_fwd(c, Ly.hd, lf, c.P(Ly.w_ff2), c.P(Ly.b_ff2), x_out, d, T, d, ff, EPI_NONE, Ly.x_ff))) return rc;
    }
  }
  if (!fuse)
    if ((rc = ln_fwd(c, D->x_final, c.P(D->ln_final), D->ac_in, D->in_dim, D->ewa, 2 * d, D->st_final))) return rc;
  if ((rc = heads_forward(c))) return rc;
  XTRL_LAUNCHED("train forward");
  return XTRL_OK;
}

int train_backward_rows(const XtrlTrainDesc* D, int Trows, hipStream_t s) {
  if (int rc = validate(D)) return rc;
  XTRL_REQUIRE(D->d_raw && D->d_values && D->d_pred && D->d_done, "train: missing loss gradients");
  const Ctx c{D, s, Trows};
  const int32_t* rows = D->packed ? D->vrows : nullptr;
  const int T = c.T, d = D->d, I = D->H * D->dh, ff = D->ff, lf = ld_ff(D);
  const int Ikv = kv_inner(D), nq3 = I + 2 * Ikv;
  int rc;
  SideStream& side = side_stream();
  const bool two = side.ok && side.ensure(side_events_needed(D->L));
  Fork F{s, side.s, two ? &side : nullptr};
  static const bool defer = [] {
    const char* e = getenv("XTRL_SPLITK_DEFER");
    return !(e && atoi(e) == 0);
  }();
  static const bool cs_defer = [] {
    const char* e = getenv("XTRL_LN_COLSUM_DEFER");
    return !(e && atoi(e) == 0);
  }();
  ColsumQueue csq;
  if (cs_defer && ln_fusable(D) && D->scratch_per_layer) {
    csq.base = D->part;
    csq.cap = D->part_floats;
  }
  SplitKQueue skq;
  const Ctx cw{D, two ? side.s : s, T, defer ? &skq : nullptr};
  int bucket = 0;
  auto bucket_done = [&]() -> int {
    if (!D->grad_events) return XTRL_OK;
    if (int rc = csq.flush(s)) return rc;
    if (int rc = splitk_flush(skq, cw.s)) return rc;
    if (hipEventRecord((hipEvent_t)D->grad_events[2 * bucket], s) != hipSuccess ||
        hipEventRecord((hipEvent_t)D->grad_events[2 * bucket + 1], cw.s) != hipSuccess) {
      set_error("train: gradient bucket event record failed");
      return XTRL_E_HIP;
    }
    ++bucket;
    return XTRL_OK;
  };
  const bool per_layer = ln_fusable(D) && D->scratch_per_layer;
  float* dx_top = per_layer ? D->dx + (int64_t)D->L * T * d : D->dx;
  const bool fold = ln_fusable(D);
  if ((rc = heads_backward(c, cw, F, !fold))) return rc;
  if (fold) {
    const int nb = (T + gemm_ln_rows(d) - 1) / gemm_ln_rows(d);
    XTRL_REQUIRE((int64_t)nb * d <= D->part_floats, "train: partial-sum workspace too small");
    GemmArgs g;
    g.A = D->dz1; g.lda = 4 * d; g.B = c.P(D->w_h1); g.ldb = D->in_dim; g.C = dx_top; g.ldc = d;
    g.M = T; g.N = d; g.K = 4 * d;
    g.ln_g = c.P(D->ln_final); g.ln_x = D->x_final; g.ln_stats = D->st_final; g.ln_rms = D->rms_norm;
    float* P = csq.take_or_flush(nb, d, c.G(D->ln_final), s, &rc);
    if (rc) return rc;
    g.ln_gpre = D->dewa; g.ln_ldg = 2 * d; g.ln_gscale = D->frac_head_grad; g.ln_part = P ? P : D->part;
    c.img(g, 1, EPI_LN_BWD2);
    if ((rc = gemm_run(g, 0, 1, EPI_LN_BWD2, s))) return rc;
    if (!P)
      hipLaunchKernelGGL(k_colsum_final, dim3(blocks(d, CS_COLS)), dim3(64 * CS_WAVES), 0, s, D->part, nb, d,
                         c.G(D->ln_final));
    XTRL_LAUNCHED("train final-norm backward");
  } else if ((rc = ln_bwd(c, D->dac, D->in_dim, D->frac_head_grad, D->dewa, 2 * d, D->x_final, D->st_final,
                          c.P(D->ln_final), nullptr, dx_top, c.G(D->ln_final)))) {
    return rc;
  }
  if ((rc = bucket_done())) return rc;
  const bool fuse = ln_fusable(D);
  XTRL_REQUIRE(!fuse || D->dx2, "train: fused LayerNorm backward needs dx2");
  const bool per = per_layer;
  int maxq = 0;
  for (int li = 0; li < D->L; ++li) maxq = std::max(maxq, D->layers[li].n_qkv);
  const int64_t Td = (int64_t)T * d;
  auto Gx = [&](int slot) { return per ? D->dx + slot * Td : D->dx; };
  auto Gx2 = [&](int li) { return per ? D->dx2 + li * Td : D->dx2; };
  const int f1 = D->ff_glu ? 2 * ff : ff, ld_f1 = D->ff_glu ? D->ld_u2 : lf;
  auto Gff = [&](int li) { return per ? D->dff + (int64_t)li * T * ld_f1 : D->dff; };
  auto Gpr = [&](int li) { return per ? D->dproj + (int64_t)li * T * maxq : D->dproj; };
  auto wait = [&](hipEvent_t e) { return per ? XTRL_OK : F.wait(e); };
  hipEvent_t e_ff1 = nullptr, e_proj = nullptr, e_out_prev = nullptr;
  for (int li = D->L - 1; li >= 0; --li) {
    const XtrlTrainLayer& Ly = D->layers[li];
    float* gout = Gx(li + 1);
    float* dff = Gff(li);
    float* dproj = Gpr(li);
    if ((rc = F.fork())) return rc;
    if ((rc = wgrad(cw, gout, d, Ly.hd, lf, c.G(Ly.w_ff2), T, d, ff, c.G(Ly.b_ff2)))) return rc;
    hipEvent_t e_ff2 = F.mark();
    if ((rc = wait(e_ff1))) return rc;
    if (D->ff_glu) {
      if ((rc = linear_dgrad(c, gout, d, c.P(Ly.w_ff2), D->glu_dh, lf, T, d, ff, EPI_NONE))) return rc;
      if ((rc = glu_bwd(D->glu_dh, lf, Ly.u, D->ld_u2, dff, ld_f1, T, ff, D->dropout, D->seed, D->ff_offset,
                        (uint32_t)li, s)))
        return rc;
    } else if ((rc = linear_dgrad(c, gout, d, c.P(Ly.w_ff2), dff, lf, T, d, ff, EPI_MUL_AUX, Ly.u, lf))) {
      return rc;
    }
    if ((rc = F.fork())) return rc;
    if ((rc = wgrad(cw, dff, ld_f1, Ly.xn_ff, d, c.G(Ly.w_ff1), T, f1, d, c.G(Ly.b_ff1)))) return rc;
    e_ff1 = F.mark();
    float* xg = D->dx;
    if (fuse) {
      if ((rc = wait(e_out_prev))) return rc;
      if ((rc = dgrad_ln_bwd(c, dff, ld_f1, c.P(Ly.w_ff1), f1, Ly.x_ff, Ly.st_ff, c.P(Ly.ln_ff), gout, Gx2(li),
                             c.G(Ly.ln_ff), &csq)))
        return rc;
      xg = Gx2(li);
    } else {
      if ((rc = linear_dgrad(c, dff, ld_f1, c.P(Ly.w_ff1), D->dxn, d, T, f1, d, EPI_NONE))) return rc;
      if ((rc = F.wait(e_ff2))) return rc;
      if ((rc = ln_bwd(c, D->dxn, d, 1.f, nullptr, 0, Ly.x_ff, Ly.st_ff, c.P(Ly.ln_ff), D->dx, D->dx, c.G(Ly.ln_ff))))
        return rc;
    }
    if ((rc = F.fork())) return rc;
    if ((rc = wgrad(cw, xg, d, D->gate_values ? Ly.og : Ly.o, I, c.G(Ly.w_out), T, d, I))) return rc;
    hipEvent_t e_out = F.mark();
    if ((rc = wait(e_proj))) return rc;
    if (D->gate_values) {
      if ((rc = linear_dgrad(c, xg, d, c.P(Ly.w_out), D->dog, I, T, d, I, EPI_DGATE, Ly.o, I, 1 << 30,
                             Ly.proj + nq3, Ly.n_qkv, dproj + nq3, Ly.n_qkv)))
        return rc;
    } else {
      if ((rc = linear_dgrad(c, xg, d, c.P(Ly.w_out), D->dog, I, T, d, I, EPI_NONE))) return rc;
    }
    const AttnProblem ap = attn_problem(c, Ly, li);
    if ((rc = attn_bwd_ex(ap, Ly.qkv, Ly.qkv + I, Ly.qkv + I + Ikv, Ly.o, Ly.lse, D->dog, dproj, dproj + I,
                          dproj + I + Ikv, D->delta, s)))
      return rc;
    const int mix_col = Ly.mix ? nq3 + (D->gate_values ? I : 0) : -1;
    const bool any_mix = [&] {
      for (int j = 1; j < D->L; ++j)
        if (D->layers[j].mix) return true;
      return false;
    }();
    bool deeper_mix = false;
    for (int j = li + 1; j < D->L; ++j) deeper_mix = deeper_mix || D->layers[j].mix;
    PrepBwdArgs pb{dproj, Ly.proj, D->layers[0].proj, D->dvfirst, D->inv_freq, T, D->n, D->H, D->dh, I,
                   Ly.n_qkv, D->layers[0].n_qkv, D->rot_dim, mix_col, li == 0 ? 1 : 0,
                   (li == 0 ? any_mix : deeper_mix) ? 1 : 0, D->qk_norm, D->xpos_base, rows, Ikv};
    const dim3 pg = rows ? dim3(blocks(nq3 / 2, PREP_T), T) : dim3(blocks(nq3 / 2, PREP_T), D->n, D->b);
    hipLaunchKernelGGL(k_qkv_prep_bwd, pg, dim3(PREP_T), 0, s, pb);
    XTRL_LAUNCHED("train qkv_prep_bwd");
    if ((rc = F.fork())) return rc;
    if ((rc = wgrad(cw, dproj, Ly.n_qkv, Ly.xn_attn, d, c.G(Ly.w_proj), T, Ly.n_qkv, d, c.G(Ly.b_proj), nq3)))
      return rc;
    e_proj = F.mark();
    if (fuse) {
      if ((rc = wait(e_ff2))) return rc;
      if ((rc = dgrad_ln_bwd(c, dproj, Ly.n_qkv, c.P(Ly.w_proj), Ly.n_qkv, Ly.x_attn, Ly.st_attn, c.P(Ly.ln_attn),
                             Gx2(li), Gx(li), c.G(Ly.ln_attn), &csq)))
        return rc;
      e_out_prev = e_out;
    } else {
      if ((rc = linear_dgrad(c, dproj, Ly.n_qkv, c.P(Ly.w_proj), D->dxn, d, T, Ly.n_qkv, d, EPI_NONE))) return rc;
      if ((rc = F.wait(e_out))) return rc;
      if ((rc = ln_bwd(c, D->dxn, d, 1.f, nullptr, 0, Ly.x_attn, Ly.st_attn, c.P(Ly.ln_attn), D->dx, D->dx,
                       c.G(Ly.ln_attn))))
        return rc;
    }
    if ((rc = bucket_done())) return rc;
  }
  if ((rc = csq.flush(s))) return rc;
  static const bool wpin_main = [] {
    const char* e = getenv("XTRL_WPIN_MAIN");
    return !(e && atoi(e) == 0);
  }();
  const bool wpin_on_main = wpin_main && !D->continuous && !D->grad_events && skq.used < D->ws_floats;
  if (wpin_on_main) {
    const int64_t used0 = skq.used;
    if ((rc = splitk_flush(skq, cw.s))) return rc;
    if ((rc = gemm_wgrad(D->dx, d, D->swr, D->S + 1, c.G(D->w_pin), D->S, T, d, D->S, 1.f, D->ws + used0,
                         D->ws_floats - used0, s, nullptr, 0, nullptr, nullptr)))
      return rc;
  } else {
    if ((rc = F.fork())) return rc;
    if ((rc = wgrad(cw, D->dx, d, D->swr, D->S + 1, c.G(D->w_pin), T, d, D->S))) return rc;
  }
  if ((rc = colsum(c, D->dx, d, T, d, c.G(D->reward_embed), D->swr + D->S, D->S + 1, D->reward_keep))) return rc;
  if (D->continuous) {
    if ((rc = wgrad(cw, D->dx, d, D->prev_action_f, D->A, c.G(D->act_emb), T, d, D->A))) return rc;
    if ((rc = wgrad(cw, D->dewa + d, 2 * d, D->next_action_f, D->A, c.G(D->act_emb), T, d, D->A))) return rc;
    if ((rc = colsum(c, D->dx, d, T, d, c.G(D->act_emb_b)))) return rc;
    if ((rc = colsum(c, D->dewa + d, 2 * d, T, d, c.G(D->act_emb_b)))) return rc;
  } else {
    int chunks = std::min<int64_t>(std::min(1024, std::max(1, T / 16)),
                                   std::max<int64_t>(1, D->part_floats / ((int64_t)D->A * d)));
    const int chunk_rows = (T + chunks - 1) / chunks;
    chunks = (T + chunk_rows - 1) / chunk_rows;
    XTRL_REQUIRE((int64_t)chunks * D->A * d <= D->part_floats, "train: partial-sum workspace too small");
    const dim3 eg(blocks(d, 256), chunks);
    if (D->A <= 4)
      hipLaunchKernelGGL(k_embed_grad_part<4>, eg, dim3(256), 0, s, D->dx, d, D->prev_action, D->dewa + d, 2 * d,
                         D->next_action, T, d, D->A, chunk_rows, D->part);
    else if (D->A <= 8)
      hipLaunchKernelGGL(k_embed_grad_part<8>, eg, dim3(256), 0, s, D->dx, d, D->prev_action, D->dewa + d, 2 * d,
                         D->next_action, T, d, D->A, chunk_rows, D->part);
    else
      hipLaunchKernelGGL(k_embed_grad_part<EMB_MAXA>, eg, dim3(256), 0, s, D->dx, d, D->prev_action, D->dewa + d,
                         2 * d, D->next_action, T, d, D->A, chunk_rows, D->part);
    hipLaunchKernelGGL(k_colsum_final, dim3(blocks(D->A * d, CS_COLS)), dim3(64 * CS_WAVES), 0, s, D->part, chunks, D->A * d,
                       c.G(D->act_emb));
    XTRL_LAUNCHED("train embed grad");
  }
  if ((rc = splitk_flush(skq, cw.s))) return rc;
  if ((rc = bucket_done())) return rc;
  if ((rc = F.wait(F.mark()))) return rc;
  XTRL_REQUIRE(!F.failed, "train: side-stream event record failed");
  XTRL_REQUIRE(!F.on() || (size_t)F.next == side_events_needed(D->L) - (wpin_on_main ? 1 : 0),
               "train: side events %d != %d", F.next, (int)side_events_needed(D->L) - (wpin_on_main ? 1 : 0));
  return XTRL_OK;
}

namespace {
struct PackBufs {
  float *swr, *pa, *na, *raw, *values, *pred, *done, *d_raw, *d_values, *d_pred, *d_done;
  int64_t floats;
};
int64_t r4(int64_t x) { return (x + 3) & ~int64_t(3); }
PackBufs pack_bufs(float* base, int T, int S, int A, int n_out, int B) {
  PackBufs P{};
  int64_t at = 0;
  auto take = [&](int cols) {
    float* q = base ? base + at : nullptr;
    at += r4((int64_t)T * cols);
    return q;
// ... 416 lines not shown

extern "C" int xtrl_fractal_train_backward(const XtrlTrainDesc* base, const XtrlFractalTrainDesc* f, void* stream) {
  return xtrl::fractal_train_backward(base, f, xtrl::as_stream(stream));
}

extern "C" int64_t xtrl_train_part_floats(int T, int b, int d, int A) {
  if (T <= 0 || d <= 0) return 0;
  const int64_t ln = (int64_t)((T + xtrl::LN_ROWS - 1) / xtrl::LN_ROWS) * d;
  const int64_t cs = (int64_t)std::min(1024, std::max(1, T / 16)) * d;
  const int64_t lat = (int64_t)std::max(b, 1) * d;
  const int64_t emb = (int64_t)std::max(A, 1) * d;
  return std::max(std::max(ln, cs), std::max(lat, emb));
}

extern "C" int xtrl_train_wimg_plan(const XtrlTrainDesc* D, XtrlWimgEntry* tab, int cap, int64_t* bytes) {
  int n = 0, blk = 0;
  int64_t at = 0;
  auto add = [&](int64_t w_off, int trans_b, int N, int K, int ld, int epi) {
    if (w_off < 0 || N <= 0 || K <= 0) return;
    XtrlWimgEntry E{};
    E.w_off = w_off; E.img_off = at; E.N = N; E.K = K; E.ld = ld; E.trans_b = trans_b;
    E.BN = xtrl::wimg_tile_bn(N, epi); E.blk0 = blk;
    const int64_t tiles = (int64_t)((N + E.BN - 1) / E.BN) * ((K + 31) / 32);
    if (tab && n < cap) tab[n] = E;
    ++n;
    blk += (int)tiles;
    at += tiles * XTRL_WIMG_TILE_BYTES(E.BN);
  };
  if (D && D->layers && D->L > 0 && D->d > 0 && xtrl::ln_fusable(D)) {
    const int d = D->d, I = D->H * D->dh, f1 = D->ff_glu ? 2 * D->ff : D->ff;
    for (int li = 0; li < D->L; ++li) {
      const XtrlTrainLayer& Ly = D->layers[li];
      add(Ly.w_out, 0, d, I, I, xtrl::EPI_RES_LN);
      add(Ly.w_ff2, 0, d, D->ff, D->ff, xtrl::EPI_RES_LN);
      add(Ly.w_ff1, 1, d, f1, d, xtrl::EPI_LN_BWD);
      add(Ly.w_proj, 1, d, Ly.n_qkv, d, xtrl::EPI_LN_BWD);
    }
    add(D->w_h1, 1, d, 4 * d, D->in_dim, xtrl::EPI_LN_BWD2);
    if (D->w_h1 >= 0) add(D->w_h1 + d, 1, D->in_dim - d, 4 * d, D->in_dim, xtrl::EPI_NONE);
  }
  if (bytes) *bytes = at;
  return n;
}

extern "C" int64_t xtrl_train_pack_floats(int T, int S, int A, int n_out, int B) {
  if (T <= 0) return 0;
  return xtrl::pack_bufs(nullptr, T, S, A, n_out, B).floats;
}

extern "C" int xtrl_linear_gelu_drop(const float* X, int ldx, const float* W, const float* bias, float* Y, int ldy,
                                     float* deriv, int ld_deriv, int M, int N, int K, float p, uint64_t seed,
                                     uint32_t offset, uint32_t layer, void* stream) {
  XTRL_REQUIRE(layer < (1u << 22), "linear_gelu_drop: layer %u out of range", layer);
  XTRL_REQUIRE(X && W && Y && deriv && M >= 0 && N > 0 && K > 0 && p >= 0.f && p < 1.f && ldx >= K && ldy >= N &&
                   ld_deriv >= N,
               "linear_gelu_drop: bad arguments");
  if (M == 0) return XTRL_OK;
  xtrl::GemmArgs g;
  g.A = X; g.lda = ldx; g.B = W; g.ldb = K; g.bias = bias; g.C = Y; g.ldc = ldy; g.M = M; g.N = N; g.K = K;
  g.aux_out = deriv; g.ld_aux_out = ld_deriv;
  g.seed = seed; g.drop_off = offset; g.drop_layer = layer;
  g.drop_thresh = xtrl::dropout_thresh(p);
  g.drop_thresh8 = xtrl::dropout_thresh8(p);
  g.inv_keep = p > 0.f ? 1.f / (1.f - p) : 1.f;
  return xtrl::gemm_run(g, 0, 0, xtrl::EPI_GELU_DROP, xtrl::as_stream(stream));
}

extern "C" int xtrl_glu_drop_fwd(const float* u, int ldu, float* h, int ldh, int M, int ff, float p, uint64_t seed,
                                 uint32_t offset, uint32_t layer, void* stream) {
  XTRL_REQUIRE(layer < (1u << 22), "glu_drop_fwd: layer %u out of range", layer);
  XTRL_REQUIRE(u && h && M >= 0 && ff > 0 && ldu >= 2 * ff && ldh >= ff && p >= 0.f && p < 1.f,
               "glu_drop_fwd: bad arguments");
  return xtrl::glu_fwd(u, ldu, h, ldh, M, ff, p, seed, offset, layer, xtrl::as_stream(stream));
}

extern "C" int xtrl_glu_drop_bwd(const float* dh, int lddh, const float* u, int ldu, float* du, int lddu, int M, int ff,
                                 float p, uint64_t seed, uint32_t offset, uint32_t layer, void* stream) {
  XTRL_REQUIRE(layer < (1u << 22), "glu_drop_bwd: layer %u out of range", layer);
  XTRL_REQUIRE(dh && u && du && M >= 0 && ff > 0 && lddh >= ff && ldu >= 2 * ff && lddu >= 2 * ff && p >= 0.f && p < 1.f,
               "glu_drop_bwd: bad arguments");
  return xtrl::glu_bwd(dh, lddh, u, ldu, du, lddu, M, ff, p, seed, offset, layer, xtrl::as_stream(stream));
}

extern "C" int xtrl_ff_dropout_mask(uint8_t* mask, int M, int N, float p, uint64_t seed, uint32_t offset,
                                    uint32_t layer, void* stream) {
  XTRL_REQUIRE(layer < (1u << 22), "ff_dropout_mask: layer %u out of range", layer);
  XTRL_REQUIRE(mask && M >= 0 && N >= 0 && p >= 0.f && p < 1.f, "ff_dropout_mask: bad arguments");
  if ((int64_t)M * N == 0) return XTRL_OK;
  hipLaunchKernelGGL(xtrl::k_ff_mask, dim3((unsigned)(((int64_t)M * N + 255) / 256)), dim3(256), 0,
                     xtrl::as_stream(stream), mask, M, N, xtrl::dropout_thresh(p), xtrl::dropout_thresh8(p), seed, offset, layer);
  XTRL_LAUNCHED("ff_dropout_mask");
  return XTRL_OK;
}
```

### x-transformers-rl_amd/xtrl_amd/_lib.py

```python
from __future__ import annotations

import ctypes as C
import os
from pathlib import Path

import torch

LIB_PATH = Path(os.environ.get('XTRL_LIB', Path(__file__).resolve().parent / 'libxtrl_hip.so'))
ABI_VERSION = 25

P = C.c_void_p
I32, I64, U32, U64, F32 = C.c_int, C.c_int64, C.c_uint32, C.c_uint64, C.c_float

ACT_NONE, ACT_GELU, ACT_SILU, ACT_RELU = 0, 1, 2, 3

LS = dict(loss=0, actor=1, critic=2, autoreg=3, done=4, adv_mean=5, adv_den=6, L=7, Lc=8, nmask=9, nwm=10,
          kcrit=11, dL=12, dLc=13)
LOSS_TOK, LOSS_STATS = 30, 32


class DecodeLayer(C.Structure):
    _fields_ = [(n, P) for n in ('ln_attn', 'w_qkv', 'b_qkv', 'w_out', 'ln_ff', 'w_ff1', 'b_ff1', 'w_ff2', 'b_ff2',
                                 'k_cache', 'v_cache', 'w_out_t', 'w_ff1x', 'w_ff2x', 'w_qkv_t', 'w_ff1_t', 'w_ff2_t',
                                 'w_ff1f', 'w_ff2f', 'mem_k', 'mem_v')]


class RngState(C.Structure):
    _fields_ = [('seed', U64), ('update', U32), ('slot_offset', U32)]


class DecodeDesc(C.Structure):
    _fields_ = ([(n, I32) for n in ('E', 'S', 'A', 'B', 'd', 'L', 'H', 'dh', 'Tmax', 'G', 'ff', 'in_dim', 'n_qkv',
                                    'continuous', 'squash', 'evolutionary', 'gate_values', 'value_residual',
                                    'learned_mix', 'rotary_abs', 'rot_dim', 'sim_mode', 'hazard_log2', 'no_reward_cond',
                                    'state_only')]
                + [('rs_eps', F32), ('clamp_lo', F32), ('clamp_hi', F32), ('has_clamp', I32)]
                + [(n, P) for n in ('w_pin', 'b_pin', 'act_emb', 'act_emb_b', 'reward_embed', 'w_se', 'b_se',
                                    'ln_final', 'w_h1', 'b_h1', 'w_h2', 'b_h2', 'inv_freq')]
                + [('layers', C.POINTER(DecodeLayer))]
                + [(n, P) for n in ('rs_mean', 'rs_var', 'state', 'prev_action', 'prev_action_f', 'prev_reward',
                                    'alive', 'lens', 'cum_reward', 'episode_of_slot', 'slot_of_row', 'rng', 'traj_states',
                                    'traj_actions', 'traj_actions_f', 'traj_logp', 'traj_rewards', 'traj_bounds',
                                    'traj_values', 'x', 'qkv', 'att', 'hff', 'ac_in', 'logits', 'v1', 'xn', 'live_rows', 'live_count',
                                    'mlp_part', 'mlp_cnt', 'lat_embed')]
                + [('prof_events', C.POINTER(C.c_void_p))]
                + [(n, P) for n in ('w_h1_t', 'w_h2_t')]
                + [('layers_dev', C.POINTER(DecodeLayer))]
                + [(n, P) for n in ('w_h1x', 'heads_part', 'heads_cnt', 'row_part', 'row_cnt')]
                + [('ff_glu', I32), ('hglu', P), ('qk_norm', I32), ('attn_scale', F32), ('xpos_base', F32),
                   ('rms_norm', I32), ('act_host', P), ('attn_window', I32), ('Hkv', I32),
                   ('num_mem_kv', I32), ('add_zero_kv', I32)])


class FractalLevel(C.Structure):
    _fields_ = [(n, P) for n in ('w_qkv', 'w_out', 'ln1_w', 'ln1_b', 'w_c', 'ln2_w', 'ln2_b', 'w_ff1', 'b_ff1',
                                 'w_ff2', 'b_ff2', 'ln3_w', 'ln3_b', 'w_pg', 'b_pg', 'level_emb', 'sums')]


class FractalDesc(C.Structure):
    _fields_ = ([('levels', I32), ('ln_eps', F32), ('level', C.POINTER(FractalLevel))]
                + [(n, P) for n in ('g_init', 'c0', 'w_fa0', 'b_fa0', 'w_fa2', 'b_fa2', 'g', 'c2', 'tmp', 'x2', 'mean',
                                    'allf', 'hagg')])


class LossDesc(C.Structure):
    _fields_ = ([(n, I32) for n in ('b', 'n', 'A', 'B', 'S1', 'continuous', 'squash', 'hl_reduction_mean')]
                + [(n, F32) for n in ('eps_clip', 'value_clip', 'entropy_weight', 'w_actor', 'w_critic', 'w_autoreg',
                                      'lo', 'hi', 'sigma')]
                + [(n, P) for n in ('raw_actions', 'values', 'pred_raw', 'done_logit', 'actions', 'actions_f',
                                    'old_logp', 'returns', 'old_values', 'dones', 'lens', 'real', 'support', 'centers',
                                    'tok', 'stats', 'd_raw_actions', 'd_values', 'd_pred_raw', 'd_done_logit')])


class TrainLayer(C.Structure):
    _fields_ = ([(n, I64) for n in ('ln_attn', 'w_proj', 'b_proj', 'w_out', 'ln_ff', 'w_ff1', 'b_ff1', 'w_ff2',
                                    'b_ff2')]
                + [('n_qkv', I32), ('mix', I32)]
                + [(n, P) for n in ('x_attn', 'x_ff', 'xn_attn', 'xn_ff', 'st_attn', 'st_ff', 'proj', 'qkv', 'o', 'og',
                                    'lse', 'u', 'hd')]
                + [('mem_k', I64), ('mem_v', I64)])


class WimgEntry(C.Structure):
    _fields_ = [('w_off', I64), ('img_off', I64), ('N', I32), ('K', I32), ('ld', I32), ('trans_b', I32), ('BN', I32),
                ('blk0', I32)]


WIMG_XRS = 40


def wimg_tile_bytes(bn: int) -> int:
    return 3 * bn * WIMG_XRS * 2


class TrainDesc(C.Structure):
    _fields_ = ([(n, I32) for n in ('b', 'n', 'S', 'A', 'd', 'L', 'H', 'dh', 'ff', 'B', 'in_dim', 'n_out', 'G',
                                    'continuous', 'evolutionary', 'gate_values', 'rot_dim')]
                + [(n, F32) for n in ('dropout', 'frac_head_grad', 'reward_keep', 'attn_scale')]
                + [('seed', U64), ('attn_offset', U32), ('ff_offset', U32), ('flat', P), ('grad', P)]
                + [(n, I64) for n in ('w_pin', 'act_emb', 'act_emb_b', 'reward_embed', 'w_se', 'b_se', 'ln_final',
                                      'w_pd', 'b_pd', 'w_pred2', 'b_pred2', 'w_lat', 'b_lat', 'w_h1', 'b_h1', 'w_a2',
                                      'b_a2', 'w_c2', 'b_c2')]
                + [(n, P) for n in ('inv_freq', 'swr', 'prev_action', 'next_action', 'prev_action_f',
                                    'next_action_f', 'latent', 'lens', 'raw', 'values', 'pred', 'done', 'x_final',
                                    'st_final', 'ac_in', 'ewa', 'zp', 'hp', 'z1', 'h1', 'lat_e', 'd_raw', 'd_values',
                                    'd_pred', 'd_done', 'dx', 'dx2', 'dxn', 'dff', 'dproj', 'dog', 'dvfirst', 'dz1', 'dac',
                                    'dzp', 'dewa', 'delta', 'part')]
                + [('part_floats', I64), ('ws', P), ('ws_floats', I64), ('layers', C.POINTER(TrainLayer)),
                   ('prof_events', C.POINTER(C.c_void_p)), ('prof_flops', P), ('prof_cap', I32), ('prof_n', P),
                   ('grad_events', C.POINTER(C.c_void_p)), ('ld_ff', I32),
                   ('scratch_per_layer', I32), ('ff_glu', I32), ('ld_u2', I32), ('glu_dh', P),
                   ('qk_norm', I32), ('xpos_base', F32), ('rms_norm', I32),
                   ('Tv', I32), ('vrows', P), ('vinv', P), ('ewa_v', P), ('hp_v', P), ('zp_v', P), ('pred_v', P),
                   ('d_pred_v', P), ('dzp_v', P), ('dewa_v', P), ('dq_part', P), ('dq_part_floats', I64),
                   ('packed', I32), ('ep_off', P), ('pack_ws', P), ('pack_ws_floats', I64), ('attn_window', I32),
                   ('Hkv', I32), ('wimg', P), ('wimg_bytes', I64), ('wimg_tab', P),
                   ('wimg_tab_host', C.POINTER(WimgEntry)), ('wimg_n', I32),
                   ('num_mem_kv', I32), ('add_zero_kv', I32), ('sink_ws', P), ('sink_ws_floats', I64)])


class FractalTrainLevel(C.Structure):
    _fields_ = ([(n, I64) for n in ('w_qkv', 'w_out', 'w_gv', 'w_go', 'ln1_w', 'ln1_b', 'ln2_w', 'ln2_b', 'ln3_w',
                                    'ln3_b', 'w_ff1', 'b_ff1', 'w_ff2', 'b_ff2', 'w_proj', 'b_proj', 'level_embed')]
                + [(n, P) for n in ('xin', 'qkv', 'o', 'lse', 's1', 'x1', 'st1', 'g', 'gv', 's2', 'x2', 'st2', 'h', 'u',
                                    's3', 'x3', 'st3', 'mean')])


class FractalTrainDesc(C.Structure):
    _fields_ = ([('levels', I32)]
                + [(n, I64) for n in ('b_in', 'g_init', 'w_gu', 'b_gu', 'w_fa0', 'b_fa0', 'w_fa2', 'b_fa2')]
                + [(n, P) for n in ('scale_embeds', 'le', 'bias0', 'cat', 'hfa', 'dxa', 'dxb', 'dmean', 'ds',
                                    'dga', 'dgb', 'dgv', 'dz', 'dqkv', 'dob', 'dcat', 'dhfa')]
                + [('level', C.POINTER(FractalTrainLevel))])


class BatchDesc(C.Structure):
    _fields_ = ([(n, I32) for n in ('N', 'Tmax', 'n', 'b', 'S', 'A', 'B', 'continuous')]
                + [(n, P) for n in ('states', 'actions', 'actions_f', 'rewards', 'logp', 'bounds', 'values', 'returns',
                                    'lens', 'idx', 'rs_mean', 'rs_var', 'swr', 'prev_action', 'action',
                                    'prev_action_f', 'action_f', 'old_logp', 'mb_returns', 'old_values', 'dones',
                                    'mb_lens', 'rs_part', 'rs_m')])


SIGNATURES = {
    'xtrl_abi_version': (I32, []),
    'xtrl_struct_size': (C.c_int64, [C.c_char_p]),
    'xtrl_last_error': (C.c_char_p, []),
    'xtrl_gemm_f32': (I32, [P, I32, P, I32, P, P, P, I32, P, I32, P, I64, I32, I32, I32, I32, P]),
    'xtrl_gemm_ex': (I32, [I32, I32, P, I32, P, I32, P, P, I32, I32, I32, I32, F32, P]),
    'xtrl_gemm_wgrad': (I32, [P, I32, P, I32, P, I32, I32, I32, I32, F32, P, I64, P]),
    'xtrl_gemm_wgrad_db': (I32, [P, I32, P, I32, P, I32, I32, I32, I32, F32, P, I64, P, I32, P]),
    'xtrl_linear_gelu_drop': (I32, [P, I32, P, P, P, I32, P, I32, I32, I32, I32, F32, U64, U32, U32, P]),
    'xtrl_layernorm_f32': (I32, [P, I32, P, P, I32, I32, I32, P]),
    'xtrl_rollout_begin': (I32, [C.POINTER(DecodeDesc), P]),
    'xtrl_decode_step': (I32, [C.POINTER(DecodeDesc), I32, P]),
    'xtrl_decode_step_rows': (I32, [C.POINTER(DecodeDesc), I32, I32, P]),
    'xtrl_row_stamps': (I32, [I32, P, I32, P]),
    'xtrl_host_decode': (I32, [C.POINTER(DecodeDesc), I32, I32, P, P]),
    'xtrl_host_feedback': (I32, [C.POINTER(DecodeDesc), I32, P, P, I32, I32, P]),
    'xtrl_rollout_env_feedback': (I32, [C.POINTER(DecodeDesc), I32, P, P, P, P, I32, I32, P]),
    'xtrl_host_row_step': (I32, [C.POINTER(DecodeDesc), I32, P, I32, I32, P, P]),
    'xtrl_host_wait': (I32, [P, C.c_uint32, C.c_double]),
    'xtrl_dgemm': (I32, [P, I32, P, P, P, I32, P, I32, P, I32, P, P, I32, I32, I32, I32, P]),
    'xtrl_dgemm_pack': (I32, [P, I32, I32, I32, P, P]),
    'xtrl_fractal_decode_step': (I32, [C.POINTER(DecodeDesc), C.POINTER(FractalDesc), I32, P]),
    'xtrl_dgemm_packed_floats': (I64, [I32, I32]),
    'xtrl_dgemm_pack_x6': (I32, [P, I32, I32, I32, P, P]),
    'xtrl_dgemm_packed_x6_elems': (I64, [I32, I32]),
    'xtrl_dgemm_pack_f8': (I32, [P, I32, I32, I32, P, P]),
    'xtrl_glu_drop_fwd': (I32, [P, I32, P, I32, I32, I32, F32, U64, U32, U32, P]),
    'xtrl_glu_drop_bwd': (I32, [P, I32, P, I32, P, I32, I32, I32, F32, U64, U32, U32, P]),
    'xtrl_dgemm_packed_f8_floats': (I64, [I32, I32]),
    'xtrl_hlgauss_gae': (I32, [P, I64, P, P, I64, P, P, P, I32, I32, I32, F32, F32, P, P, P]),
    'xtrl_attn_fwd': (I32, [P, P, P, P, P, P, I32, I32, I32, I32, F32, F32, U64, U32, U32, P]),
    'xtrl_attn_bwd': (I32, [P, P, P, P, P, P, P, P, P, P, P, I32, I32, I32, I32, F32, F32, U64, U32, U32, P]),
    'xtrl_attn_bwd_part_floats': (I64, [I32, I32, I32, I32]),
    'xtrl_train_pack_floats': (I64, [I32, I32, I32, I32, I32]),
    'xtrl_attn_bwd_part': (I32, [P, P, P, P, P, P, P, P, P, P, P, P, I64, I32, I32, I32, I32, F32, F32, U64, U32, U32,
                                  P]),
    'xtrl_attn_fwd_win': (I32, [P, P, P, P, P, P, I32, I32, I32, I32, F32, F32, U64, U32, U32, I32, P]),
    'xtrl_attn_bwd_win': (I32, [P, P, P, P, P, P, P, P, P, P, P, I32, I32, I32, I32, F32, F32, U64, U32, U32, I32, P]),
    'xtrl_attn_bwd_part_win': (I32, [P, P, P, P, P, P, P, P, P, P, P, P, I64, I32, I32, I32, I32, F32, F32, U64, U32,
                                      U32, I32, P]),
    'xtrl_attn_fwd_gqa': (I32, [P, P, P, P, P, P, I32, I32, I32, I32, I32, F32, F32, U64, U32, U32, I32, P]),
    'xtrl_attn_bwd_gqa': (I32, [P, P, P, P, P, P, P, P, P, P, P, I32, I32, I32, I32, I32, F32, F32, U64, U32, U32, I32,
                                 P]),
    'xtrl_attn_bwd_part_gqa': (I32, [P, P, P, P, P, P, P, P, P, P, P, P, I64, I32, I32, I32, I32, I32, F32, F32, U64,
                                      U32, U32, I32, P]),
    'xtrl_attn_sink_ws_floats': (I64, [I32, I32, I32, I32]),
    'xtrl_attn_fwd_sink': (I32, [P, P, P, P, P, P, P, P, I32, I32, I32, I32, I32, F32, F32, U64, U32, U32, I32, I32, I32,
                                 P]),
    'xtrl_attn_bwd_sink': (I32, [P, P, P, P, P, P, P, P, P, P, P, P, P, P, P, P, I64, I32, I32, I32, I32, I32, F32, F32,
                                 U64, U32, U32, I32, I32, I32, P]),
    'xtrl_attn_bwd_part_sink': (I32, [P, P, P, P, P, P, P, P, P, P, P, P, I64, P, P, P, P, P, I64, I32, I32, I32, I32,
                                      I32, F32, F32, U64, U32, U32, I32, I32, I32, P]),
    'xtrl_loss_fwd': (I32, [C.POINTER(LossDesc), P]),
    'xtrl_loss_bwd': (I32, [C.POINTER(LossDesc), F32, P]),
    'xtrl_grad_norm': (I32, [P, I64, P, F32, P, P]),
    'xtrl_adopt_atan2': (I32, [P, P, P, P, P, I64, P, I32, P, I32, P, P, F32, F32, F32, F32, F32, F32, F32, F32, F32,
                               I32, P]),
    'xtrl_ema_lerp': (I32, [P, P, I64, F32, P]),
    'xtrl_sim_reset': (I32, [P, I32, I32, U64, U32, P, P]),
    'xtrl_train_forward': (I32, [C.POINTER(TrainDesc), P]),
    'xtrl_train_backward': (I32, [C.POINTER(TrainDesc), P]),
    'xtrl_ff_dropout_mask': (I32, [P, I32, I32, F32, U64, U32, U32, P]),
    'xtrl_train_part_floats': (C.c_int64, [I32, I32, I32, I32]),
    'xtrl_train_wimg_plan': (I32, [C.POINTER(TrainDesc), C.POINTER(WimgEntry), I32, C.POINTER(I64)]),
    'xtrl_wimg_launch_count': (I64, []),
    'xtrl_wimg_build': (I32, [P, C.POINTER(WimgEntry), P, I32, P, I64, P]),
    'xtrl_minibatch_gather': (I32, [C.POINTER(BatchDesc), P]),
    'xtrl_rsnorm_update': (I32, [P, P, P, I32, I32, P]),
    'xtrl_attn_fwd_tokens': (I32, [P, I32, P, I32, P, I32, P, P, I32, P, I32, I32, I32, I32, F32, I32, P]),
    'xtrl_rows_add': (I32, [P, I32, P, P, I32, I32, I32, P]),
    'xtrl_add_layernorm': (I32, [P, I32, P, I32, I32, P, P, P, I32, I32, I32, F32, P]),
    'xtrl_seq_mean': (I32, [P, I32, I32, I32, I32, P, I32, P]),
    'xtrl_safe_embed': (I32, [P, I32, P, I32, P, I32, P]),
    'xtrl_wm_post': (I32, [P, I32, I32, I32, P, P, I32, P, P]),
    'xtrl_rng_uniform': (F32, [U64, U32, U32, U32, U32, U32]),
    'xtrl_rng_normal': (F32, [U64, U32, U32, U32, U32, U32]),
    'xtrl_source_hash': (C.c_char_p, []),
    'xtrl_fractal_train_forward': (I32, [C.POINTER(TrainDesc), C.POINTER(FractalTrainDesc), P]),
    'xtrl_fractal_train_backward': (I32, [C.POINTER(TrainDesc), C.POINTER(FractalTrainDesc), P]),
}

STRUCTS = {'XtrlDecodeLayer': DecodeLayer, 'XtrlRngState': RngState, 'XtrlDecodeDesc': DecodeDesc,
           'XtrlTrainLayer': TrainLayer, 'XtrlTrainDesc': TrainDesc, 'XtrlBatchDesc': BatchDesc,
           'XtrlLossDesc': LossDesc, 'XtrlFractalLevel': FractalLevel, 'XtrlFractalDesc': FractalDesc,
           'XtrlFractalTrainLevel': FractalTrainLevel, 'XtrlFractalTrainDesc': FractalTrainDesc,
           'XtrlWimgEntry': WimgEntry}

_lib = None


def load():
    global _lib
    if _lib is None:
        if not LIB_PATH.exists():
            raise RuntimeError(f'{LIB_PATH} is missing: build it with `make -C x-transformers-rl_amd` '
                               f'or __graft_entry__.build() (the MI355X path has no CPU fallback)')
        lib = C.CDLL(str(LIB_PATH))
        for name, (res, args) in SIGNATURES.items():
            fn = getattr(lib, name)
            fn.restype, fn.argtypes = res, args
        if lib.xtrl_abi_version() != ABI_VERSION:
            raise RuntimeError(f'libxtrl_hip ABI {lib.xtrl_abi_version()} != {ABI_VERSION}')
        from ._srchash import source_hash
        built, here = lib.xtrl_source_hash().decode(), source_hash()
        if built != here and 'XTRL_LIB' not in os.environ:
            raise RuntimeError(f'{LIB_PATH} was built from sources {built}, the tree holds {here}: rebuild it '
                               f'with `make -C x-transformers-rl_amd` or __graft_entry__.build()')
        for cname, py in STRUCTS.items():
            got = lib.xtrl_struct_size(cname.encode())
            if got != C.sizeof(py):
                raise RuntimeError(f'libxtrl_hip {cname} is {got} bytes, the binding {C.sizeof(py)}: rebuild')
        _lib = lib
    return _lib


def lib():
    if not torch.cuda.is_available():
        raise RuntimeError('xtrl_amd needs a ROCm GPU (gfx950); no CPU fallback exists by design')
    return load()


def check(rc, what=''):
    if rc != 0:
        msg = load().xtrl_last_error().decode(errors='replace')
        raise RuntimeError(f'libxtrl_hip {what} failed (code {rc}): {msg}')


def ptr(t):
    return None if t is None else C.c_void_p(t.data_ptr())


def stream():
    return C.c_void_p(torch.cuda.current_stream().cuda_stream)


def rng_uniform(seed, update, slot, t, field, sub=0):
    return load().xtrl_rng_uniform(seed & 0xFFFFFFFFFFFFFFFF, update, slot, t, field, sub)


FIELD_STATE, FIELD_REWARD, FIELD_TERM, FIELD_SAMPLE, FIELD_COIN, FIELD_DROPOUT, FIELD_FF_DROPOUT = 1, 2, 3, 4, 5, 6, 7
```

### x-transformers-rl_amd/xtrl_amd/ops.py

```python
from __future__ import annotations

import ctypes as C

import torch

from . import _lib as L


def _f32c(t):
    assert t.dtype == torch.float32 and t.is_cuda and t.is_contiguous(), (t.dtype, t.device, t.shape)
    return t




def gemm(x, w, bias=None, ln_gamma=None, residual=None, act=L.ACT_NONE, out=None):
    lib = L.lib()
    M, K = x.shape
    N = w.shape[0]
    assert w.shape[1] == K and x.stride(1) == 1 and w.is_contiguous()
    if out is None:
        out = torch.empty(M, N, device=x.device, dtype=torch.float32)
    if bias is not None:
        assert bias.shape == (N,) and bias.is_contiguous()
# ... 75 lines not shown
        N = w.shape[0]
        x2 = x.reshape(-1, K)
        if not x2.is_contiguous():
            x2 = x2.contiguous()
        M = x2.shape[0]
        assert w.is_contiguous() and (b is None or b.is_contiguous())
        y = torch.empty(M, N, device=x.device, dtype=torch.float32)
        deriv = torch.empty(M, N, device=x.device, dtype=torch.float32)
        L.check(L.lib().xtrl_linear_gelu_drop(L.ptr(x2), K, L.ptr(w), L.ptr(b), L.ptr(y), N, L.ptr(deriv), N, M, N, K,
                                              float(p), int(seed) & (2 ** 64 - 1), int(offset) & 0xFFFFFFFF,
                                              int(layer), L.stream()), 'linear_gelu_drop')
        ctx.save_for_backward(x2, w, deriv)
        ctx.extra = (wg, bg, ws, x.shape)
        return y.view(*x.shape[:-1], N)

    @staticmethod
    def backward(ctx, dh):
        x2, w, deriv = ctx.saved_tensors
        wg, bg, ws, xshape = ctx.extra
        N, K = w.shape
        g = (dh.reshape(-1, N) * deriv).contiguous()
        M = g.shape[0]
        dx = None
        if ctx.needs_input_grad[0]:
            dx = torch.empty(M, K, device=g.device, dtype=torch.float32)
            if M:
                gemm_ex(g, w, 0, 1, M, K, N, dx)
            dx = dx.view(xshape)
        if wg is not None and M:
            L.check(L.lib().xtrl_gemm_wgrad_db(L.ptr(g), N, L.ptr(x2), K, L.ptr(wg), K, M, N, K, 1., L.ptr(ws), ws.numel(),
                                               L.ptr(bg), 0, L.stream()), 'gemm_wgrad_db')
        elif bg is not None:
            bg.add_(g.sum(0))
        return dx, None, None, None, None, None, None, None, None, None


def linear_gelu_drop(x, w, b, wg, bg, ws, p, seed, offset, layer):
    return LinearGeluDropFn.apply(x, w, b, wg, bg, ws, p, seed, offset, layer)


class GluDropFn(torch.autograd.Function):

    @staticmethod
    def forward(ctx, u, p, seed, offset, layer):
        F2 = u.shape[-1]
        assert F2 % 2 == 0
        ff = F2 // 2
        u2 = _f32c(u.reshape(-1, F2).contiguous())
        M = u2.shape[0]
        h = torch.empty(M, ff, device=u.device, dtype=torch.float32)
        args = (float(p), int(seed) & (2 ** 64 - 1), int(offset) & 0xFFFFFFFF, int(layer))
        L.check(L.lib().xtrl_glu_drop_fwd(L.ptr(u2), F2, L.ptr(h), ff, M, ff, *args, L.stream()), 'glu_drop_fwd')
        ctx.save_for_backward(u2)
        ctx.extra = (args, u.shape)
        return h.view(*u.shape[:-1], ff)

    @staticmethod
    def backward(ctx, dh):
        (u2,) = ctx.saved_tensors
        args, ushape = ctx.extra
        M, F2 = u2.shape
        ff = F2 // 2
        dh2 = dh.reshape(-1, ff).contiguous()
        du = torch.empty(M, F2, device=dh.device, dtype=torch.float32)
        L.check(L.lib().xtrl_glu_drop_bwd(L.ptr(dh2), ff, L.ptr(u2), F2, L.ptr(du), F2, M, ff, *args, L.stream()),
                'glu_drop_bwd')
        return du.view(ushape), None, None, None, None


def glu_drop(u, p, seed, offset, layer):
    return GluDropFn.apply(u, p, seed, offset, layer)


def layernorm(x, gamma, out=None):
    lib = L.lib()
    M, D = x.shape
    if out is None:
        out = torch.empty(M, D, device=x.device, dtype=torch.float32)
    L.check(lib.xtrl_layernorm_f32(L.ptr(x), x.stride(0), L.ptr(gamma), L.ptr(out), out.stride(0), M, D,
                                   L.stream()), 'layernorm')
    return out




def kv_head_index(heads, kv_heads, device=None):
    return torch.arange(heads, device=device) % kv_heads


class AttentionFn(torch.autograd.Function):

    @staticmethod
    def forward(ctx, q, k, v, lens, scale, dropout_p, seed, offset, sub, window=0, mem_k=None, mem_v=None,
                add_zero_kv=False):
        lib = L.lib()
        b, H, n, dh = q.shape
        Hkv = k.shape[1]
        assert 1 <= Hkv <= H and H % Hkv == 0, f'kv heads {Hkv} must divide heads {H}'
        for t, heads in ((q, H), (k, Hkv), (v, Hkv)):
            _f32c(t)
            assert t.shape == (b, heads, n, dh)
        assert lens.dtype == torch.int32 and lens.shape == (b,)
        assert (mem_k is None) == (mem_v is None), 'mem_k and mem_v go together'
        M = 0 if mem_k is None else mem_k.shape[1]
        for t in (mem_k, mem_v):
            if t is not None:
                _f32c(t)
                assert t.shape == (Hkv, M, dh), f'memory key / values must be [Hkv][M][dh], not {tuple(t.shape)}'
        o = torch.empty_like(q)
        lse = torch.empty(b, H, n, device=q.device, dtype=torch.float32)
        L.check(lib.xtrl_attn_fwd_sink(L.ptr(q), L.ptr(k), L.ptr(v), L.ptr(lens), L.ptr(o), L.ptr(lse),
                                       L.ptr(mem_k) if M else None, L.ptr(mem_v) if M else None, b, H, Hkv, n, dh,
                                       float(scale), float(dropout_p), int(seed), int(offset), int(sub), int(window),
                                       M, int(bool(add_zero_kv)), L.stream()), 'attn_fwd')
        ctx.save_for_backward(q, k, v, lens, o, lse, *((mem_k, mem_v) if M else ()))
        ctx.cfg = (float(scale), float(dropout_p), int(seed), int(offset), int(sub), int(window), M,
                   int(bool(add_zero_kv)))
        return o

    @staticmethod
    def backward(ctx, do):
        lib = L.lib()
        q, k, v, lens, o, lse = ctx.saved_tensors[:6]
        scale, p, seed, offset, sub, window, M, Z = ctx.cfg
        mem_k, mem_v = ctx.saved_tensors[6:] if M else (None, None)
        b, H, n, dh = q.shape
        do = do.contiguous()
        dq, dk, dv = torch.empty_like(q), torch.empty_like(k), torch.empty_like(v)
        delta = torch.empty(b, H, n, device=q.device, dtype=torch.float32)
        dmk = dmv = ws = None
        ws_floats = 0
        if M:
            dmk, dmv = torch.empty_like(mem_k), torch.empty_like(mem_v)
            ws_floats = int(lib.xtrl_attn_sink_ws_floats(b, H, M, dh))
            ws = torch.empty(ws_floats, device=q.device, dtype=torch.float32)
        pm = lambda t: L.ptr(t) if t is not None else None
        L.check(lib.xtrl_attn_bwd_sink(L.ptr(q), L.ptr(k), L.ptr(v), L.ptr(lens), L.ptr(o), L.ptr(lse), L.ptr(do),
                                       L.ptr(dq), L.ptr(dk), L.ptr(dv), L.ptr(delta), pm(mem_k), pm(mem_v), pm(dmk),
                                       pm(dmv), pm(ws), ws_floats, b, H, k.shape[1], n, dh, scale, p, seed, offset, sub,
                                       window, M, Z, L.stream()), 'attn_bwd')
        return dq, dk, dv, None, None, None, None, None, None, None, dmk, dmv, None


def attention(q, k, v, lens, scale, dropout_p=0., seed=0, offset=0, sub=0, window=0, mem_k=None, mem_v=None,
              add_zero_kv=False):
    if mem_k is not None:
        mem_k, mem_v = mem_k.contiguous(), mem_v.contiguous()
    return AttentionFn.apply(q.contiguous(), k.contiguous(), v.contiguous(), lens, scale, dropout_p, seed, offset,
                             sub, window, mem_k, mem_v, add_zero_kv)




class LossConsts:

    def __init__(self, *, actions, old_logp, returns, old_values, dones, lens, real, support, centers, continuous,
                 squash, hl_mean, eps_clip, value_clip, entropy_weight, w_actor, w_critic, w_autoreg, lo, hi, sigma):
        self.__dict__.update(locals())
        del self.__dict__['self']


class LossFn(torch.autograd.Function):
    @staticmethod
    def forward(ctx, raw_actions, values, pred_raw, done_logit, K: LossConsts):
        lib = L.lib()
        b, n, B = values.shape
# ... 93 lines not shown
```

### x-transformers-rl_amd/xtrl_amd/train.py

```python
from __future__ import annotations

import ctypes as C
import os

import torch

from . import _lib as L
from .params import FlatParams


WIMG_DEFAULT = os.environ.get('XTRL_WIMG', '0') == '1'


def ld_ff(ff):
    return ff + 16 if ff % 256 == 0 else ff


def _off(flat, name):
    return flat.index[name][0] if name in flat.index else -1


def _span_off(flat, names):
    flat.span(names)
    return flat.index[names[0]][0]
# ... 68 lines not shown
        f32 = dict(device=dev, dtype=torch.float32)
        E = lambda *shape: torch.empty(*shape, **f32)
        off = lambda name: flat.index[name][0] if name in flat.index else -1
        pre = 'transformer.attn_layers.layers.'

        def span_off(names):
            a0 = flat.index[names[0]][0]
            flat.span(names)
            return a0

        self.layers_py = []
        self.ld_ff = lff = ld_ff(ff)
        glu = bool(getattr(c, 'ff_glu', False))
        lu2 = ld_ff(2 * ff) if glu else lff
        layers = (L.TrainLayer * L_)()
        X = [E(T, d) for _ in range(L_ + 1)]
        max_qkv = 0
        nw = 'g' if c.rms_norm else 'gamma'
        for li in range(L_):
            mix = bool(c.value_residual and c.learned_mix and li > 0)
            pa, pf = f'{pre}{2 * li}.', f'{pre}{2 * li + 1}.'
            wn = [pa + '1.to_q.weight', pa + '1.to_k.weight', pa + '1.to_v.weight']
            wn += [pa + '1.to_v_gate.weight'] if c.gate_values else []
            wn += [pa + '1.to_value_residual_mix.0.weight'] if mix else []
            bn = ([pa + '1.to_v_gate.bias'] if c.gate_values else []) + \
                 ([pa + '1.to_value_residual_mix.0.bias'] if mix else [])
            n_qkv = I + 2 * Ikv + (I if c.gate_values else 0) + (c.n_kv_heads if mix else 0)
            max_qkv = max(max_qkv, n_qkv)
            bufs = dict(x_attn=X[li], x_ff=E(T, d), xn_attn=E(T, d), xn_ff=E(T, d), st_attn=E(T, 2), st_ff=E(T, 2),
                        proj=E(T, n_qkv), qkv=E(T, I + 2 * Ikv), o=E(T, I), lse=E(b_max * H * n_max), u=E(T, lu2),
                        hd=E(T, lff))
            bufs['og'] = E(T, I) if c.gate_values else bufs['o']
            self.layers_py.append(bufs)
            Ly = layers[li]
            Ly.ln_attn, Ly.w_proj = off(pa + '0.0.' + nw), span_off(wn)
            Ly.b_proj = span_off(bn) if bn else -1
            Ly.w_out, Ly.ln_ff = off(pa + '1.to_out.weight'), off(pf + '0.0.' + nw)
            f1 = pf + ('1.ff.0.proj.' if glu else '1.ff.0.0.')
            Ly.w_ff1, Ly.b_ff1 = off(f1 + 'weight'), off(f1 + 'bias')
            Ly.w_ff2, Ly.b_ff2 = off(pf + '1.ff.2.weight'), off(pf + '1.ff.2.bias')
            Ly.n_qkv, Ly.mix = n_qkv, int(mix)
            Ly.mem_k, Ly.mem_v = off(pa + '1.mem_k'), off(pa + '1.mem_v')
            for k, t in bufs.items():
                setattr(Ly, k, t.data_ptr())
        self.layers = layers
        self.X = X
        ldp = d + 4
        self.buf = dict(x_final=X[L_], st_final=E(T, 2), ac_in=E(T, c.in_dim), ewa=E(T, 2 * d), zp=E(T, ldp),
                        hp=E(T, ldp), z1=E(T, 4 * d), h1=E(T, 4 * d), lat_e=E(max(b_max, 1), d),
                        raw=E(T, n_out), values=E(T, B), pred=E(T, 2 * (S + 1)), done=E(T),
                        d_raw=E(T, n_out), d_values=E(T, B), d_pred=E(T, 2 * (S + 1)), d_done=E(T),
                        dx=E(L_ + 1, T, d), dx2=E(L_, T, d), dxn=E(T, d), dff=E(L_, T, lu2), dproj=E(L_, T, max_qkv),
                        dog=E(T, I), dvfirst=E(T, Ikv),
                        dz1=E(T, 4 * d), dac=E(T, c.in_dim), dzp=E(T, ldp), dewa=E(T, 2 * d),
                        delta=E(b_max * H * n_max))
        if glu:
            self.buf['glu_dh'] = E(T, lff)
        part = max(256 * max((2 if glu else 1) * ff, 4 * d, B, max_qkv), 1024 * max(A, 1) * d,
                   int(L.lib().xtrl_train_part_floats(T, b_max, d, A)))
        self.buf['part'] = E(part)
        self.tok = torch.empty(b_max, n_max, L.LOSS_TOK, **f32)
        self.stats = torch.zeros(L.LOSS_STATS, **f32)

        D = L.TrainDesc()
        D.S, D.A, D.d, D.L, D.H, D.dh, D.ff, D.B = S, A, d, L_, H, dh, ff, B
        D.in_dim, D.n_out, D.G = c.in_dim, n_out, c.dim_gene if c.evolutionary else 0
        D.continuous, D.evolutionary, D.gate_values, D.rot_dim = int(c.continuous), int(c.evolutionary), \
            int(c.gate_values), rot
        D.frac_head_grad = float(c.frac_head_grad)
        D.attn_scale = float(c.qk_norm_scale) if c.qk_norm else float(dh ** -0.5)
        D.qk_norm, D.xpos_base = int(c.qk_norm), float(c.xpos_scale_base) if c.rotary_xpos else 0.
        D.flat, D.grad = flat.flat.data_ptr(), flat.grad.data_ptr()
        D.w_pin = off('transformer.project_in.weight')
        _heads_desc(D, c, flat)
        D.ln_final = off('transformer.attn_layers.final_norm.' + nw)
        D.rms_norm = int(c.rms_norm)
        D.attn_window = int(c.attn_window)
        D.Hkv = int(c.n_kv_heads)
        D.num_mem_kv, D.add_zero_kv = int(getattr(c, 'num_mem_kv', 0)), int(bool(getattr(c, 'add_zero_kv', False)))
        if D.num_mem_kv:
            self.sink_ws = E(int(L.lib().xtrl_attn_sink_ws_floats(b_max, H, D.num_mem_kv, dh)))
            D.sink_ws, D.sink_ws_floats = self.sink_ws.data_ptr(), self.sink_ws.numel()
        D.inv_freq = self.inv_freq.data_ptr()
        for k, t in self.buf.items():
            setattr(D, k, t.data_ptr())
        D.part_floats = self.buf['part'].numel()
        D.ws, D.ws_floats = ws.data_ptr(), ws.numel()
        D.layers = C.cast(layers, C.POINTER(L.TrainLayer))
        D.ld_ff = lff
        D.scratch_per_layer = 1
        D.ff_glu, D.ld_u2 = int(glu), (lu2 if glu else 0)
        self.cbuf = _compact_bufs(D, c, T, dev, b_max, n_max)
        self.D = D
        self.wimg = None
        if WIMG_DEFAULT:
            self.use_weight_images(True)

    def use_weight_images(self, on: bool):
        D = self.D
        if not on or isinstance(self, FractalTrainStep):
            D.wimg, D.wimg_bytes, D.wimg_tab, D.wimg_tab_host, D.wimg_n = None, 0, None, None, 0
            return
        if self.wimg is None:
            self.wimg = _alloc_wimg(D, self.dev)
        w = self.wimg
        if w is not None:
            D.wimg, D.wimg_bytes = w['arena'].data_ptr(), w['arena'].numel()
            D.wimg_tab, D.wimg_tab_host, D.wimg_n = w['tab_dev'].data_ptr(), C.cast(w['tab'], C.POINTER(L.WimgEntry)), \
                len(w['tab'])

    def forward(self, swr, prev_action, next_action, latent, lens, reward_keep, seed, attn_offset, ff_offset,
                dropout, Tv=0, packed=False):
        self._bind_inputs(swr, prev_action, next_action, latent, lens, reward_keep, seed, attn_offset, ff_offset,
                          dropout, Tv)
        D = self.D
        D.packed = 0
        if packed:
            assert 0 < Tv <= D.b * D.n, (Tv, D.b, D.n)
            D.Tv, D.packed = int(Tv), 1
            if self.cbuf.get('pack_ws') is None:
                c = self.cfg
                nf = int(L.lib().xtrl_train_pack_floats(self.T_max, c.state_dim, c.num_actions, D.n_out, c.num_bins))
                self.cbuf['pack_ws'] = torch.empty(nf, device=self.dev, dtype=torch.float32)
                D.pack_ws, D.pack_ws_floats = self.cbuf['pack_ws'].data_ptr(), nf
        L.check(L.lib().xtrl_train_forward(C.byref(self.D), L.stream()), 'train_forward')
        return self._outputs()

    def _bind_inputs(self, swr, prev_action, next_action, latent, lens, reward_keep, seed, attn_offset, ff_offset,
                     dropout, Tv=0):
        c, D = self.cfg, self.D
        b, n = swr.shape[0], swr.shape[1]
        assert b <= self.b_max and n <= self.n_max, (b, n, self.b_max, self.n_max)
        assert 0 <= Tv <= b * n, (Tv, b, n)
        D.Tv = int(Tv) if Tv < b * n else 0
        for t in (swr, prev_action, next_action, lens):
            assert t.is_cuda and t.is_contiguous()
        self._keep = [swr, prev_action, next_action, latent, lens]
        D.b, D.n = b, n
        D.dropout, D.reward_keep = float(dropout), float(reward_keep)
        D.seed, D.attn_offset, D.ff_offset = int(seed) & (2 ** 64 - 1), int(attn_offset) & 0xFFFFFFFF, \
            int(ff_offset) & 0xFFFFFFFF
        D.swr, D.lens = swr.data_ptr(), lens.data_ptr()
        if c.continuous:
            D.prev_action_f, D.next_action_f, D.prev_action, D.next_action = prev_action.data_ptr(), \
                next_action.data_ptr(), None, None
        else:
            assert prev_action.dtype == torch.int32 and next_action.dtype == torch.int32
            D.prev_action, D.next_action, D.prev_action_f, D.next_action_f = prev_action.data_ptr(), \
                next_action.data_ptr(), None, None
        D.latent = latent.contiguous().data_ptr() if latent is not None else None
        if latent is not None:
            self._keep.append(latent.contiguous())
            D.latent = self._keep[-1].data_ptr()

    def _outputs(self):
        b, n = self.D.b, self.D.n
        T = b * n
        bf = self.buf
        return (bf['raw'][:T].view(b, n, -1), bf['values'][:T].view(b, n, -1), bf['pred'][:T].view(b, n, -1),
                bf['done'][:T].view(b, n))

    def loss(self, K, stats=None):
        c, D = self.cfg, self.D
        b, n = D.b, D.n
        T = b * n
        bf = self.buf
# ... 200 lines not shown
```

Before: 444,800 env-steps/s.

## Fold QKV rotary/value-mix prep into dh=16 attention kernels and precompute rotary table

Adds fused attention forward and backward kernels for head dim 16 that read the raw projection directly, applying rotary embedding and value-residual mixing on the fly. The backward kernel also writes gradients straight into the projection gradient, undoing the rotation and handling the mix. This removes the separate qkv_prep and qkv_prep_bwd launches and the materialised qkv buffer. A precomputed sin/cos rotary table replaces per-element trig. The fold is on by default through an environment variable and falls back to the old path when its limits are exceeded. The cost is extra redundant rotation work inside the attention tiles and more shared memory per block.

```diff
diff --git a/include/xtrl_hip.h b/include/xtrl_hip.h
--- a/include/xtrl_hip.h
+++ b/include/xtrl_hip.h
@@ -11,7 +11,7 @@
 #define XTRL_E_ARG 1
 #define XTRL_E_HIP 2
 
-#define XTRL_ABI_VERSION 25
+#define XTRL_ABI_VERSION 26
 
 int xtrl_abi_version(void);
 int64_t xtrl_struct_size(const char* name);
@@ -364,6 +364,8 @@
   const XtrlWimgEntry* wimg_tab;
   const XtrlWimgEntry* wimg_tab_host;
   int wimg_n;
+  int rot_tab_n;
+  const float* rot_tab;
   int num_mem_kv;
   int add_zero_kv;
   float* sink_ws;
@@ -381,6 +383,30 @@
                     void* arena, int64_t arena_bytes, void* stream);
 
 int64_t xtrl_wimg_launch_count(void);
+
+int xtrl_rotary_table(const float* inv_freq, int half, int n_max, float* out, void* stream);
+int xtrl_qkv_prep(const float* proj, int n_qkv, const float* vfirst, int ld_vfirst, float* qkv, const float* inv_freq,
+                  const float* rot_tab, int rot_tab_n, int b, int n, int H, int dh, int rot_dim, int mix_col,
+                  void* stream);
+int xtrl_qkv_prep_bwd(float* dproj, const float* proj, int n_qkv, const float* vfirst, int ld_vfirst, float* dvfirst,
+                      const float* inv_freq, const float* rot_tab, int rot_tab_n, int b, int n, int H, int dh,
+                      int rot_dim, int mix_col, int first_layer, int accumulate, void* stream);
+int xtrl_attn_fwd_rows(const float* qkv, const int32_t* lens, float* o, float* lse, const float* gate, int ld_gate,
+                       float* og, int b, int H, int n, int dh, float scale, float dropout_p, uint64_t seed,
+                       uint32_t offset, uint32_t sub, void* stream);
+int xtrl_attn_bwd_rows(const float* qkv, const int32_t* lens, const float* o, const float* lse, const float* dout,
+                       float* dproj, int ldp, float* delta_ws, int b, int H, int n, int dh, float scale,
+                       float dropout_p, uint64_t seed, uint32_t offset, uint32_t sub, void* stream);
+int xtrl_attn_fwd_fold(const float* proj, int ldp, const float* vfirst, int ld_vfirst, const int32_t* lens, float* o,
+                       float* lse, int gate_col, float* og, const float* inv_freq, const float* rot_tab, int rot_tab_n,
+                       int rot_dim, int mix_col, int b, int H, int n, int dh, float scale, float dropout_p,
+                       uint64_t seed, uint32_t offset, uint32_t sub, void* stream);
+int xtrl_attn_bwd_fold(const float* proj, int ldp, const float* vfirst, int ld_vfirst, const int32_t* lens,
+                       const float* o, const float* lse, const float* dout, float* dproj, float* dvfirst,
+                       float* delta_ws, const float* inv_freq, const float* rot_tab, int rot_tab_n, int rot_dim,
+                       int mix_col, int first_layer, int accumulate, int b, int H, int n, int dh, float scale,
+                       float dropout_p, uint64_t seed, uint32_t offset, uint32_t sub, void* stream);
+int64_t xtrl_attn_fold_launch_count(void);
 
 int xtrl_train_forward(const XtrlTrainDesc* desc, void* stream);
 int xtrl_train_backward(const XtrlTrainDesc* desc, void* stream);
diff --git a/x-transformers-rl_amd/csrc/attn.hip b/x-transformers-rl_amd/csrc/attn.hip
--- a/x-transformers-rl_amd/csrc/attn.hip
+++ b/x-transformers-rl_amd/csrc/attn.hip
@@ -695,6 +695,347 @@
 #pragma unroll
         for (int d = 0; d < ND; ++d) a.dQ[gb + (int64_t)i * gsi + 16 * d + lr] = dq[qt][d][r] * a.scale;
       }
+    }
+}
+
+struct FoldArgs {
+  AttnArgs a;
+  const float* proj;
+  const float* vfirst;
+  float* dvfirst;
+  const float2* tab;
+  const float* inv_freq;
+  int ldp, ldvf, I, mix_col, rot_dim, first_layer, accumulate;
+};
+
+__device__ __forceinline__ void fold_stage_rot(const FoldArgs& f, float2* rt, int npos, int tid) {
+  const int half = f.rot_dim >> 1;
+  for (int x = tid; x < npos * half; x += 256) {
+    const int pos = x / half;
+    rt[x] = rot_sincos(f.tab, half, f.inv_freq, pos, x - pos * half);
+  }
+}
+__device__ __forceinline__ float2 fold_rot_pair(const FoldArgs& f, const float2* rt, const float* p, int c0, int pos) {
+  const float2 x = *reinterpret_cast<const float2*>(p + c0);
+  return c0 < f.rot_dim ? rot_pair(x, rt[pos * (f.rot_dim >> 1) + (c0 >> 1)]) : x;
+}
+__device__ __forceinline__ float2 fold_v_pair(const FoldArgs& f, int64_t t, int h, int c0) {
+  const float* pr = f.proj + t * f.ldp;
+  float2 x = *reinterpret_cast<const float2*>(pr + 2 * f.I + h * 16 + c0);
+  if (f.mix_col >= 0) {
+    const float m = sigmoidf_(pr[f.mix_col + h]);
+    const float2 vf = *reinterpret_cast<const float2*>(f.vfirst + t * f.ldvf + 2 * f.I + h * 16 + c0);
+    x.x = lerpf_(x.x, vf.x, m);
+    x.y = lerpf_(x.y, vf.y, m);
+  }
+  return x;
+}
+__device__ __forceinline__ float fold_unrot(const FoldArgs& f, const float2* rt, float g, int lr, int pos) {
+  const float go = __shfl_xor(g, 1, 64);
+  const int c0 = lr & ~1;
+  if (c0 >= f.rot_dim) return g;
+  const bool odd = lr & 1;
+  const float2 y = rot_pair_inv(odd ? make_float2(go, g) : make_float2(g, go),
+                                rt[pos * (f.rot_dim >> 1) + (c0 >> 1)]);
+  return odd ? y.y : y.x;
+}
+
+__global__ __launch_bounds__(256) void k_attn_fwd_fold(const FoldArgs f) {
+  constexpr int DH = 16, KS = DH / 4, KST = DH + 2;
+  const AttnArgs& a = f.a;
+  __shared__ float Ks[TK][KST], Vs[TK][KST];
+  __shared__ float Ps[4][16][PST];
+  const int lane = threadIdx.x & 63, w = threadIdx.x >> 6, tid = threadIdx.x;
+  const int bh = blockIdx.y, b = bh / a.H, n = a.n;
+  const int q0 = blockIdx.x * TQ;
+  const int len = a.lens[b];
+  const int h = bh - b * a.H;
+  const int64_t t0 = (int64_t)b * n;
+  const int64_t ob = (int64_t)b * a.out.sb + h * a.out.sh;
+  const int osi = a.out.si;
+  const int lr = lane & 15, lg = lane >> 4;
+  const uint32_t off = a.offset + (uint32_t)bh;
+  __shared__ float2 Rt[FB_MAXN * 8];
+  fold_stage_rot(f, Rt, min(n, q0 + TQ), tid);
+  __syncthreads();
+
+  float qa[KS];
+  {
+    const int i = q0 + 16 * w + lr;
+#pragma unroll
+    for (int s = 0; s < KS; ++s) {
+      const int c = 4 * s + lg;
+      float2 x = make_float2(0.f, 0.f);
+      if (i < n) x = fold_rot_pair(f, Rt, f.proj + (t0 + i) * f.ldp + h * DH, c & ~1, i);
+      qa[s] = (c & 1) ? x.y : x.x;
+    }
+  }
+  float m[4], l[4];
+  f32x4v o = f32x4v{0.f, 0.f, 0.f, 0.f};
+#pragma unroll
+  for (int r = 0; r < 4; ++r) {
+    m[r] = -INFINITY;
+    l[r] = 0.f;
+  }
+  const int last_key = min(min(q0 + TQ - 1, n - 1), len - 1);
+  for (int kt = 0; kt * TK <= last_key; ++kt) {
+    __syncthreads();
+    for (int x = tid; x < TK * DH / 2; x += 256) {
+      const int j = x / (DH / 2), c0 = 2 * (x - j * (DH / 2)), jj = kt * TK + j;
+      float2 kk = make_float2(0.f, 0.f), vv = make_float2(0.f, 0.f);
+      if (jj < n) {
+        kk = fold_rot_pair(f, Rt, f.proj + (t0 + jj) * f.ldp + f.I + h * DH, c0, jj);
+        vv = fold_v_pair(f, t0 + jj, h, c0);
+      }
+      *reinterpret_cast<float2*>(&Ks[j][c0]) = kk;
+      *reinterpret_cast<float2*>(&Vs[j][c0]) = vv;
+    }
+    __syncthreads();
+    f32x4v sacc[4];
+#pragma unroll
+    for (int sub = 0; sub < 4; ++sub) {
+      sacc[sub] = f32x4v{0.f, 0.f, 0.f, 0.f};
+#pragma unroll
+      for (int s = 0; s < KS; ++s) sacc[sub] = mfma16(qa[s], Ks[16 * sub + lr][4 * s + lg], sacc[sub]);
+    }
+    u32x4_t kws[4] = {};
+    if (a.thresh8) {
+      kws[0] = philox4x32_10((uint32_t)((q0 + 16 * w + 4 * lg) >> 2), (uint32_t)(kt * 16 + lr), off, a.c3, a.seed);
+    } else if (a.thresh) {
+#pragma unroll
+      for (int sub = 0; sub < 4; ++sub)
+        kws[sub] = philox4x32_10((uint32_t)((q0 + 16 * w + 4 * lg) >> 2), (uint32_t)(kt * TK + 16 * sub + lr), off,
+                                 a.c3, a.seed);
+    }
+#pragma unroll
+    for (int r = 0; r < 4; ++r) {
+      const int i = q0 + 16 * w + 4 * lg + r;
+      float sv[4];
+      float mx = -INFINITY;
+#pragma unroll
+      for (int sub = 0; sub < 4; ++sub) {
+        const int j = kt * TK + 16 * sub + lr;
+        const bool ok = (j <= i) && (j < len);
+        sv[sub] = ok ? sacc[sub][r] * a.scale : -INFINITY;
+        mx = fmaxf(mx, sv[sub]);
+      }
+#pragma unroll
+      for (int o2 = 1; o2 < 16; o2 <<= 1) mx = fmaxf(mx, __shfl_xor(mx, o2, 64));
+      const float mnew = fmaxf(m[r], mx);
+      const float alpha = (m[r] == -INFINITY) ? 0.f : expf(m[r] - mnew);
+      float rs = 0.f;
+#pragma unroll
+      for (int sub = 0; sub < 4; ++sub) {
+        const float p = (sv[sub] == -INFINITY) ? 0.f : expf(sv[sub] - mnew);
+        rs += p;
+        float pd = p;
+        if (a.thresh8) pd = (qbyte(kws[0], sub, r) >= a.thresh8) ? p * a.inv_keep : 0.f;
+        else if (a.thresh) pd = (qword(kws[sub], r) >= a.thresh) ? p * a.inv_keep : 0.f;
+        Ps[w][4 * lg + r][16 * sub + lr] = pd;
+      }
+#pragma unroll
+      for (int o2 = 1; o2 < 16; o2 <<= 1) rs += __shfl_xor(rs, o2, 64);
+      l[r] = l[r] * alpha + rs;
+      m[r] = mnew;
+      o[r] *= alpha;
+    }
+    wave_sync();
+#pragma unroll
+    for (int s = 0; s < TK / 4; ++s) o = mfma16(Ps[w][lr][4 * s + lg], Vs[4 * s + lg][lr], o);
+    wave_sync();
+  }
+#pragma unroll
+  for (int r = 0; r < 4; ++r) {
+    const int i = q0 + 16 * w + 4 * lg + r;
+    if (i < n) {
+      const int64_t at = ob + (int64_t)i * osi + lr;
+      const float ov = o[r] / l[r];
+      a.Oout[at] = ov;
+      if (a.OGout)
+        a.OGout[at] = ov * sigmoidf_(a.G[(int64_t)b * a.gate.sb + h * a.gate.sh + (int64_t)i * a.gate.si + lr]);
+      if (lr == 0) a.LSEout[(int64_t)bh * n + i] = m[r] + logf(l[r]);
+    }
+  }
+}
+
+__global__ __launch_bounds__(256) void k_attn_bwd_fold(const FoldArgs f) {
+  constexpr int DH = 16, KS = DH / 4, KST = DH + 2;
+  const AttnArgs& a = f.a;
+  __shared__ float Qs[TQ][KST], dOs[TQ][KST], Ks[TK][KST];
+  __shared__ float Ls[TQ], Dls[TQ];
+  __shared__ float Ps[4][16][PST];
+  const int lane = threadIdx.x & 63, w = threadIdx.x >> 6, tid = threadIdx.x;
+  const int bh = blockIdx.x, b = bh / a.H, n = a.n;
+  const int len = a.lens[b];
+  const int h = bh - b * a.H;
+  const int64_t t0 = (int64_t)b * n;
+  const int64_t ob = (int64_t)b * a.out.sb + h * a.out.sh, gb = (int64_t)b * a.grad.sb + h * a.grad.sh;
+  const int osi = a.out.si, gsi = a.grad.si;
+  const int lr = lane & 15, lg = lane >> 4;
+  const uint32_t off = a.offset + (uint32_t)bh;
+  const int nq = (n + TQ - 1) / TQ;
+  const float* qrow = f.proj + t0 * f.ldp + h * DH;
+  __shared__ float2 Rt[FB_MAXN * 8];
+  fold_stage_rot(f, Rt, n, tid);
+  __syncthreads();
+
+  f32x4v dq[FB_QT];
+#pragma unroll
+  for (int q = 0; q < FB_QT; ++q) dq[q] = f32x4v{0.f, 0.f, 0.f, 0.f};
+
+  for (int kt = 0; kt < nq; ++kt) {
+    const int j0 = kt * TK;
+    float ka[KS], va[KS];
+    {
+      const int j = j0 + 16 * w + lr;
+#pragma unroll
+      for (int s = 0; s < KS; ++s) {
+        const int c = 4 * s + lg;
+        float2 kk = make_float2(0.f, 0.f), vv = make_float2(0.f, 0.f);
+        if (j < n) {
+          kk = fold_rot_pair(f, Rt, qrow + (int64_t)j * f.ldp + f.I, c & ~1, j);
+          vv = fold_v_pair(f, t0 + j, h, c & ~1);
+        }
+        ka[s] = (c & 1) ? kk.y : kk.x;
+        va[s] = (c & 1) ? vv.y : vv.x;
+      }
+    }
+    f32x4v dk = f32x4v{0.f, 0.f, 0.f, 0.f}, dv = f32x4v{0.f, 0.f, 0.f, 0.f};
+    if (j0 < len) {
+#pragma unroll
+      for (int qt = 0; qt < FB_QT; ++qt) {
+        if (qt < kt || qt >= nq) continue;
+        __syncthreads();
+        for (int x = tid; x < TQ * DH / 2; x += 256) {
+          const int i = x / (DH / 2), c0 = 2 * (x - i * (DH / 2)), ii = qt * TQ + i, jj = j0 + i;
+          float2 qq = make_float2(0.f, 0.f), dd = make_float2(0.f, 0.f), kk = make_float2(0.f, 0.f);
+          if (ii < n) {
+            qq = fold_rot_pair(f, Rt, qrow + (int64_t)ii * f.ldp, c0, ii);
+            dd = *reinterpret_cast<const float2*>(a.dO + ob + (int64_t)ii * osi + c0);
+          }
+          if (jj < n) kk = fold_rot_pair(f, Rt, qrow + (int64_t)jj * f.ldp + f.I, c0, jj);
+          *reinterpret_cast<float2*>(&Qs[i][c0]) = qq;
+          *reinterpret_cast<float2*>(&dOs[i][c0]) = dd;
+          *reinterpret_cast<float2*>(&Ks[i][c0]) = kk;
+        }
+        float orow[DH];
+        if (tid < TQ) {
+          const int ii = qt * TQ + tid;
+          Ls[tid] = ii < n ? a.LSE[(int64_t)bh * n + ii] : 0.f;
+#pragma unroll
+          for (int c = 0; c < DH; ++c) orow[c] = ii < n ? a.O[ob + (int64_t)ii * osi + c] : 0.f;
+        }
+        __syncthreads();
+        if (tid < TQ) {
+          float dsum = 0.f;
+#pragma unroll
+          for (int c = 0; c < DH; ++c) dsum += dOs[tid][c] * orow[c];
+          Dls[tid] = dsum;
+          const int ii = qt * TQ + tid;
+          if (kt == 0 && ii < n) a.Dout[(int64_t)bh * n + ii] = dsum;
+        }
+        __syncthreads();
+        float dsr[4][4];
+#pragma unroll
+        for (int sub = 0; sub < 4; ++sub) {
+          f32x4v st = f32x4v{0.f, 0.f, 0.f, 0.f}, dpt = f32x4v{0.f, 0.f, 0.f, 0.f};
+#pragma unroll
+          for (int s = 0; s < KS; ++s) {
+            st = mfma16(ka[s], Qs[16 * sub + lr][4 * s + lg], st);
+            dpt = mfma16(va[s], dOs[16 * sub + lr][4 * s + lg], dpt);
+          }
+          const int il = 16 * sub + lr, i = qt * TQ + il;
+          uint32_t kq[4] = {0u, 0u, 0u, 0u};
+          if (a.thresh8) {
+            const u32x4_t kb = philox4x32_10((uint32_t)(i >> 2), (uint32_t)((j0 >> 6) * 16 + 4 * lg + (lr & 3)), off,
+                                             a.c3, a.seed);
+            const uint32_t wd = qword(kb, w);
+#pragma unroll
+            for (int c = 0; c < 4; ++c) kq[c] = (wd >> (8 * c)) & 0xFFu;
+            quad_transpose(kq, lane);
+          } else if (a.thresh) {
+            const u32x4_t kb = philox4x32_10((uint32_t)(i >> 2), (uint32_t)(j0 + 16 * w + 4 * lg + (lr & 3)), off,
+                                             a.c3, a.seed);
+            kq[0] = kb.x;
+            kq[1] = kb.y;
+            kq[2] = kb.z;
+            kq[3] = kb.w;
+            quad_transpose(kq, lane);
+          }
+#pragma unroll
+          for (int r = 0; r < 4; ++r) {
+            const int j = j0 + 16 * w + 4 * lg + r;
+            const bool ok = (j <= i) && (j < len) && (i < n);
+            const float p = ok ? expf(st[r] * a.scale - Ls[il]) : 0.f;
+            float z = 1.f;
+            if (a.thresh8 && ok) z = (kq[r] >= a.thresh8) ? a.inv_keep : 0.f;
+            else if (a.thresh && ok) z = (kq[r] >= a.thresh) ? a.inv_keep : 0.f;
+            Ps[w][4 * lg + r][il] = p * z;
+            dsr[sub][r] = p * (dpt[r] * z - Dls[il]);
+          }
+        }
+        wave_sync();
+#pragma unroll
+        for (int s = 0; s < TQ / 4; ++s) dv = mfma16(Ps[w][lr][4 * s + lg], dOs[4 * s + lg][lr], dv);
+        wave_sync();
+#pragma unroll
+        for (int sub = 0; sub < 4; ++sub)
+#pragma unroll
+          for (int r = 0; r < 4; ++r) Ps[w][4 * lg + r][16 * sub + lr] = dsr[sub][r];
+        wave_sync();
+#pragma unroll
+        for (int s = 0; s < TQ / 4; ++s) dk = mfma16(Ps[w][lr][4 * s + lg], Qs[4 * s + lg][lr], dk);
+        __syncthreads();
+#pragma unroll
+        for (int s = 0; s < TK / 4; ++s) {
+          const int j = 4 * s + lg;
+          dq[qt] = mfma16(Ps[j >> 4][j & 15][16 * w + lr], Ks[j][lr], dq[qt]);
+        }
+      }
+    }
+#pragma unroll
+    for (int r = 0; r < 4; ++r) {
+      const int j = j0 + 16 * w + 4 * lg + r;
+      const bool in = j < n;
+      const int jc = in ? j : 0;
+      const int64_t t = t0 + jc;
+      const float gk = fold_unrot(f, Rt, dk[r] * a.scale, lr, jc);
+      float gv = dv[r];
+      float* dvf = f.dvfirst + t * f.I + h * DH + lr;
+      if (f.mix_col >= 0) {
+        const float* pr = f.proj + t * f.ldp;
+        const int c0 = lr & ~1;
+        const bool odd = lr & 1;
+        const float mm = sigmoidf_(pr[f.mix_col + h]);
+        const float go = __shfl_xor(gv, 1, 64);
+        const float2 v = *reinterpret_cast<const float2*>(pr + 2 * f.I + h * DH + c0);
+        const float2 vf = *reinterpret_cast<const float2*>(f.vfirst + t * f.ldvf + 2 * f.I + h * DH + c0);
+        float dm = mix_dm_pair(odd ? make_float2(go, gv) : make_float2(gv, go), v, vf);
+#pragma unroll
+        for (int o2 = DH >> 1; o2 > 1; o2 >>= 1) dm += __shfl_xor(dm, o2, 64);
+        if (in) {
+          const float old = f.accumulate ? *dvf : 0.f;
+          *dvf = lerp_bwd_first(gv, mm, f.accumulate != 0, old);
+          if (lr == 0) a.dQ[t * gsi + f.mix_col + h] = mix_dlogit(dm, mm);
+        }
+        gv = lerp_bwd_self(gv, mm);
+      } else if (f.first_layer && f.accumulate) {
+        if (in) gv += *dvf;
+      }
+      if (in) {
+        a.dK[gb + (int64_t)j * gsi + lr] = gk;
+        a.dV[gb + (int64_t)j * gsi + lr] = gv;
+      }
+    }
+  }
+#pragma unroll
+  for (int qt = 0; qt < FB_QT; ++qt)
+#pragma unroll
+    for (int r = 0; r < 4; ++r) {
+      const int i = qt * TQ + 16 * w + 4 * lg + r;
+      const bool in = qt < nq && i < n;
+      const float g = fold_unrot(f, Rt, dq[qt][r] * a.scale, lr, in ? i : 0);
+      if (in) a.dQ[gb + (int64_t)i * gsi + lr] = g;
     }
 }
 
@@ -1031,6 +1372,94 @@
   return sink_bwd(a, p, s);
 }
 
+int64_t g_attn_fold_launches = 0;
+
+bool attn_fold_on() {
+  const char* e = getenv("XTRL_ATTN_FOLD");
+  return !(e && atoi(e) == 0);
+}
+
+const char* attn_fold_refusal(const AttnProblem& p, const AttnFold& f) {
+  if (!p.causal) return "bidirectional attention";
+  if (p.ep_off) return "packed rows";
+  if (p.dh != 16) return "dim_head != 16";
+  if (p.n > FB_MAXN) return "episodes longer than 128 steps";
+  if (is_gqa(p)) return "grouped-query attention (kv heads < heads)";
+  if (p.window > 0) return "a sliding window";
+  if (attn_has_sinks(p)) return "attention sinks";
+  if (f.qk_norm) return "qk norm";
+  if (f.xpos_base != 0.f) return "rotary xPos";
+  if ((f.ldp | f.ld_vfirst) & 1) return "an odd projection row stride";
+  if (f.rot_dim < 0 || f.rot_dim > p.dh || (f.rot_dim & 1)) return "a rotary width outside the head";
+  if (!attn_fused_bwd_on()) return "XTRL_ATTN_FUSED_BWD=0";
+  return nullptr;
+}
+bool attn_fold_ok(const AttnProblem& p, const AttnFold& f) { return attn_fold_on() && !attn_fold_refusal(p, f); }
+
+namespace {
+int fill_fold(FoldArgs& fa, const AttnProblem& p, const AttnFold& f, const char* who) {
+  const char* why = attn_fold_refusal(p, f);
+  XTRL_REQUIRE(!why, "%s: the folded kernels do not take %s", who, why);
+  if (int rc = fill_args(fa.a, p)) return rc;
+  XTRL_REQUIRE(f.proj && f.ldp >= 3 * p.H * p.dh, "%s: proj rows of %d columns hold no q | k | v of %d", who, f.ldp,
+               3 * p.H * p.dh);
+  XTRL_REQUIRE(f.mix_col < 0 || (f.vfirst && f.ld_vfirst >= 3 * p.H * p.dh && f.mix_col + p.H <= f.ldp),
+               "%s: the value mix needs vfirst and its H columns inside the row", who);
+  XTRL_REQUIRE(f.rot_dim == 0 || f.inv_freq || f.rot_tab, "%s: rotary without inv_freq or a table", who);
+  fa.proj = f.proj;
+  fa.vfirst = f.vfirst;
+  fa.dvfirst = f.dvfirst;
+  fa.tab = (f.rot_tab && f.rot_tab_n >= p.n) ? reinterpret_cast<const float2*>(f.rot_tab) : nullptr;
+  XTRL_REQUIRE(f.rot_dim == 0 || fa.tab || f.inv_freq, "%s: the rotary table holds %d < %d positions and inv_freq is null",
+               who, f.rot_tab_n, p.n);
+  fa.inv_freq = f.inv_freq;
+  fa.ldp = f.ldp;
+  fa.ldvf = f.ld_vfirst;
+  fa.I = p.H * p.dh;
+  fa.mix_col = f.mix_col;
+  fa.rot_dim = f.rot_dim;
+  fa.first_layer = f.first_layer;
+  fa.accumulate = f.accumulate;
+  return XTRL_OK;
+}
+}
+
+int attn_fwd_fold(const AttnProblem& p, const AttnFold& f, float* o, float* lse, const float* gate, float* og,
+                  hipStream_t s) {
+  FoldArgs fa{};
+  if (int rc = fill_fold(fa, p, f, "attn_fwd_fold")) return rc;
+  XTRL_REQUIRE(o && lse, "attn_fwd_fold: null operand");
+  XTRL_REQUIRE(!gate == !og, "attn_fwd_fold: gate and og go together");
+  fa.a.Oout = o;
+  fa.a.LSEout = lse;
+  fa.a.G = gate;
+  fa.a.OGout = og;
+  hipLaunchKernelGGL(k_attn_fwd_fold, dim3((p.n + TQ - 1) / TQ, p.b * p.H), dim3(256), 0, s, fa);
+  XTRL_LAUNCHED("attn_fwd_fold");
+  ++g_attn_fold_launches;
+  return XTRL_OK;
+}
+
+int attn_bwd_fold(const AttnProblem& p, const AttnFold& f, const float* o, const float* lse, const float* dout,
+                  float* delta_ws, hipStream_t s) {
+  FoldArgs fa{};
+  if (int rc = fill_fold(fa, p, f, "attn_bwd_fold")) return rc;
+  XTRL_REQUIRE(o && lse && dout && delta_ws && f.dproj, "attn_bwd_fold: null operand");
+  XTRL_REQUIRE(p.grad.si == f.ldp, "attn_bwd_fold: dproj rows of %d columns, proj rows of %d", p.grad.si, f.ldp);
+  XTRL_REQUIRE(f.dvfirst || (f.mix_col < 0 && !(f.first_layer && f.accumulate)), "attn_bwd_fold: null dvfirst");
+  fa.a.O = o;
+  fa.a.LSE = lse;
+  fa.a.dO = dout;
+  fa.a.Dout = delta_ws;
+  fa.a.dQ = f.dproj;
+  fa.a.dK = f.dproj + fa.I;
+  fa.a.dV = f.dproj + 2 * fa.I;
+  hipLaunchKernelGGL(k_attn_bwd_fold, dim3(p.b * p.H), dim3(256), 0, s, fa);
+  XTRL_LAUNCHED("attn_bwd_fold");
+  ++g_attn_fold_launches;
+  return XTRL_OK;
+}
+
 int64_t attn_dq_part_floats(int b, int H, int n, int dh) {
   return (int64_t)((n + TK - 1) / TK) * b * H * n * dh;
 }
@@ -1185,3 +1614,94 @@
   pr.causal = causal;
   return xtrl::attn_fwd_ex(pr, q, k, v, o, lse, nullptr, nullptr, (hipStream_t)stream);
 }
+
+namespace xtrl {
+namespace {
+__global__ __launch_bounds__(256) void k_rotary_table(const float* inv_freq, int half, int n_max, float2* out) {
+  const int x = blockIdx.x * 256 + threadIdx.x;
+  if (x >= n_max * half) return;
+  const int pos = x / half, p = x - pos * half;
+  out[x] = rot_sincos(nullptr, half, inv_freq, pos, p);
+}
+
+AttnProblem rows_problem(const int32_t* lens, int b, int H, int n, int dh, int ld_in, int ldp, float scale, float p,
+                         uint64_t seed, uint32_t offset, uint32_t sub) {
+  AttnProblem pr = contiguous_problem(lens, b, H, n, dh, scale, p, seed, offset, sub, 0, 0);
+  pr.in = attn_layout_tokens(n, ld_in, dh);
+  pr.out = attn_layout_tokens(n, H * dh, dh);
+  pr.grad = pr.gate = attn_layout_tokens(n, ldp, dh);
+  return pr;
+}
+}
+}
+
+extern "C" int xtrl_rotary_table(const float* inv_freq, int half, int n_max, float* out, void* stream) {
+  XTRL_REQUIRE(inv_freq && out && half > 0 && n_max > 0, "rotary_table: bad arguments");
+  hipLaunchKernelGGL(xtrl::k_rotary_table, dim3((n_max * half + 255) / 256), dim3(256), 0, xtrl::as_stream(stream),
+                     inv_freq, half, n_max, reinterpret_cast<float2*>(out));
+  XTRL_LAUNCHED("rotary_table");
+  return XTRL_OK;
+}
+
+extern "C" int64_t xtrl_attn_fold_launch_count(void) { return xtrl::g_attn_fold_launches; }
+
+extern "C" int xtrl_attn_fwd_rows(const float* qkv, const int32_t* lens, float* o, float* lse, const float* gate,
+                                  int ld_gate, float* og, int b, int H, int n, int dh, float scale, float dropout_p,
+                                  uint64_t seed, uint32_t offset, uint32_t sub, void* stream) {
+  const int I = H * dh;
+  const xtrl::AttnProblem pr = xtrl::rows_problem(lens, b, H, n, dh, 3 * I, ld_gate, scale, dropout_p, seed, offset, sub);
+  return xtrl::attn_fwd_ex(pr, qkv, qkv + I, qkv + 2 * I, o, lse, gate, og, xtrl::as_stream(stream));
+}
+
+extern "C" int xtrl_attn_bwd_rows(const float* qkv, const int32_t* lens, const float* o, const float* lse,
+                                  const float* dout, float* dproj, int ldp, float* delta_ws, int b, int H, int n, int dh,
+                                  float scale, float dropout_p, uint64_t seed, uint32_t offset, uint32_t sub,
+                                  void* stream) {
+  const int I = H * dh;
+  const xtrl::AttnProblem pr = xtrl::rows_problem(lens, b, H, n, dh, 3 * I, ldp, scale, dropout_p, seed, offset, sub);
+  return xtrl::attn_bwd_ex(pr, qkv, qkv + I, qkv + 2 * I, o, lse, dout, dproj, dproj + I, dproj + 2 * I, delta_ws,
+                           xtrl::as_stream(stream));
+}
+
+extern "C" int xtrl_attn_fwd_fold(const float* proj, int ldp, const float* vfirst, int ld_vfirst, const int32_t* lens,
+                                  float* o, float* lse, int gate_col, float* og, const float* inv_freq,
+                                  const float* rot_tab, int rot_tab_n, int rot_dim, int mix_col, int b, int H, int n,
+                                  int dh, float scale, float dropout_p, uint64_t seed, uint32_t offset, uint32_t sub,
+                                  void* stream) {
+  const xtrl::AttnProblem pr = xtrl::rows_problem(lens, b, H, n, dh, ldp, ldp, scale, dropout_p, seed, offset, sub);
+  xtrl::AttnFold f;
+  f.proj = proj;
+  f.ldp = ldp;
+  f.vfirst = vfirst;
+  f.ld_vfirst = ld_vfirst;
+  f.inv_freq = inv_freq;
+  f.rot_tab = rot_tab;
+  f.rot_tab_n = rot_tab_n;
+  f.rot_dim = rot_dim;
+  f.mix_col = mix_col;
+  return xtrl::attn_fwd_fold(pr, f, o, lse, og ? proj + gate_col : nullptr, og, xtrl::as_stream(stream));
+}
+
+extern "C" int xtrl_attn_bwd_fold(const float* proj, int ldp, const float* vfirst, int ld_vfirst, const int32_t* lens,
+                                  const float* o, const float* lse, const float* dout, float* dproj, float* dvfirst,
+                                  float* delta_ws, const float* inv_freq, const float* rot_tab, int rot_tab_n,
+                                  int rot_dim, int mix_col, int first_layer, int accumulate, int b, int H, int n, int dh,
+                                  float scale, float dropout_p, uint64_t seed, uint32_t offset, uint32_t sub,
+                                  void* stream) {
+  const xtrl::AttnProblem pr = xtrl::rows_problem(lens, b, H, n, dh, ldp, ldp, scale, dropout_p, seed, offset, sub);
+  xtrl::AttnFold f;
+  f.proj = proj;
+  f.ldp = ldp;
+  f.vfirst = vfirst;
+  f.ld_vfirst = ld_vfirst;
+  f.dproj = dproj;
+  f.dvfirst = dvfirst;
+  f.inv_freq = inv_freq;
+  f.rot_tab = rot_tab;
+  f.rot_tab_n = rot_tab_n;
+  f.rot_dim = rot_dim;
+  f.mix_col = mix_col;
+  f.first_layer = first_layer;
+  f.accumulate = accumulate;
+  return xtrl::attn_bwd_fold(pr, f, o, lse, dout, delta_ws, xtrl::as_stream(stream));
+}
diff --git a/x-transformers-rl_amd/csrc/common.h b/x-transformers-rl_amd/csrc/common.h
--- a/x-transformers-rl_amd/csrc/common.h
+++ b/x-transformers-rl_amd/csrc/common.h
@@ -130,4 +130,43 @@
   return (fabsf(w) < 0.5f) ? s + w * (e - s) : e - (e - s) * (1.0f - w);
 }
 
+__device__ __forceinline__ float2 rot_sincos(const float2* tab, int half, const float* inv_freq, int pos, int p) {
+  if (tab) return tab[pos * half + p];
+  float2 sc;
+  sincosf((float)pos * inv_freq[p], &sc.x, &sc.y);
+  return sc;
 }
+__device__ __forceinline__ float2 rot_pair(float2 x, float2 sc) {
+#pragma clang fp contract(off)
+  float2 y;
+  y.x = __builtin_fmaf(x.x, sc.y, (-x.y) * sc.x);
+  y.y = __builtin_fmaf(x.y, sc.y, x.x * sc.x);
+  return y;
+}
+__device__ __forceinline__ float2 rot_pair_inv(float2 g, float2 sc) {
+#pragma clang fp contract(off)
+  float2 y;
+  y.x = g.x * sc.y + g.y * sc.x;
+  y.y = __builtin_fmaf(g.y, sc.y, (-g.x) * sc.x);
+  return y;
+}
+__device__ __forceinline__ float lerp_bwd_first(float g, float m, bool accumulate, float old) {
+#pragma clang fp contract(off)
+  float f = g * m;
+  if (accumulate) f += old;
+  return f;
+}
+__device__ __forceinline__ float lerp_bwd_self(float g, float m) {
+#pragma clang fp contract(off)
+  return g * (1.0f - m);
+}
+__device__ __forceinline__ float mix_dm_pair(float2 g, float2 v, float2 vf) {
+#pragma clang fp contract(off)
+  return __builtin_fmaf(g.x, vf.x - v.x, g.y * (vf.y - v.y));
+}
+__device__ __forceinline__ float mix_dlogit(float dm, float m) {
+#pragma clang fp contract(off)
+  return dm * (1.0f - m) * m;
+}
+
+}
diff --git a/x-transformers-rl_amd/csrc/kernels.h b/x-transformers-rl_amd/csrc/kernels.h
--- a/x-transformers-rl_amd/csrc/kernels.h
+++ b/x-transformers-rl_amd/csrc/kernels.h
@@ -198,4 +198,23 @@
                 const float* lse, const float* dout, float* dq, float* dk, float* dv, float* delta_ws,
                 hipStream_t s);
 
-}
+struct AttnFold {
+  const float* proj = nullptr;   int ldp = 0;
+  const float* vfirst = nullptr; int ld_vfirst = 0;
+  float* dproj = nullptr;
+  float* dvfirst = nullptr;
+  const float* inv_freq = nullptr;
+  const float* rot_tab = nullptr;
+  int rot_tab_n = 0;
+  int rot_dim = 0, mix_col = -1;
+  int first_layer = 0, accumulate = 0;
+  int qk_norm = 0;
+  float xpos_base = 0.f;
+};
+bool attn_fold_ok(const AttnProblem& p, const AttnFold& f);
+int attn_fwd_fold(const AttnProblem& p, const AttnFold& f, float* o, float* lse, const float* gate, float* og,
+                  hipStream_t s);
+int attn_bwd_fold(const AttnProblem& p, const AttnFold& f, const float* o, const float* lse, const float* dout,
+                  float* delta_ws, hipStream_t s);
+
+}
diff --git a/x-transformers-rl_amd/csrc/train.hip b/x-transformers-rl_amd/csrc/train.hip
--- a/x-transformers-rl_amd/csrc/train.hip
+++ b/x-transformers-rl_amd/csrc/train.hip
@@ -1,4 +1,5 @@
 #include <cstdlib>
+#include <unordered_set>
 #include <vector>
 
 #include <hip/hip_ext.h>
@@ -322,6 +323,7 @@
   float xpos_base;
   const int32_t* rows;
   int Ikv;
+  const float2* rot_tab;
 };
 
 __device__ __forceinline__ void qkv_segment(int col, int I, int Ikv, int& seg, int& within) {
@@ -359,11 +361,7 @@
       x.y = x.y / nrm;
     }
     if (j < a.rot_dim) {
-      const float f = (float)pos * a.inv_freq[j >> 1];
-      float sn, cs;
-      sincosf(f, &sn, &cs);
-      y.x = x.x * cs + (-x.y) * sn;
-      y.y = x.y * cs + x.x * sn;
+      y = rot_pair(x, rot_sincos(a.rot_tab, a.rot_dim >> 1, a.inv_freq, pos, j >> 1));
       if (a.xpos_base > 0.f) {
         const float xf = xpos_factor(j, a.rot_dim, pos, a.n, a.xpos_base);
         const float sf = seg == 0 ? xf : 1.0f / xf;
@@ -395,6 +393,7 @@
   float xpos_base;
   const int32_t* rows;
   int Ikv;
+  const float2* rot_tab;
 };
 
 __global__ __launch_bounds__(PREP_T) void k_qkv_prep_bwd(const PrepBwdArgs a) {
@@ -414,9 +413,7 @@
     float2 gv = *reinterpret_cast<float2*>(g);
     if (seg < 2) {
       if (j < a.rot_dim) {
-        const float f = (float)pos * a.inv_freq[j >> 1];
-        float sn, cs;
-        sincosf(f, &sn, &cs);
+        const float2 sc = rot_sincos(a.rot_tab, a.rot_dim >> 1, a.inv_freq, pos, j >> 1);
         float g0 = gv.x, g1 = gv.y;
         if (a.xpos_base > 0.f) {
           const float xf = xpos_factor(j, a.rot_dim, pos, a.n, a.xpos_base);
@@ -424,8 +421,7 @@
           g0 *= sf;
           g1 *= sf;
         }
-        gv.x = g0 * cs + g1 * sn;
-        gv.y = g1 * cs + (-g0) * sn;
+        gv = rot_pair_inv(make_float2(g0, g1), sc);
         if (!a.qk_norm) *reinterpret_cast<float2*>(g) = gv;
       }
       gqk = gv;
@@ -436,18 +432,14 @@
         m = sigmoidf_(pr[a.mix_col + h]);
         const float2 v = *reinterpret_cast<const float2*>(pr + col);
         const float2 vf = *reinterpret_cast<const float2*>(a.vfirst + (int64_t)t * a.ld_vfirst + col);
-        dm = gv.x * (vf.x - v.x) + gv.y * (vf.y - v.y);
+        dm = mix_dm_pair(gv, v, vf);
+        const float2 o = a.accumulate ? *dvf : make_float2(0.f, 0.f);
         float2 f;
-        f.x = gv.x * m;
-        f.y = gv.y * m;
-        if (a.accumulate) {
-          const float2 o = *dvf;
-          f.x += o.x;
-          f.y += o.y;
-        }
+        f.x = lerp_bwd_first(gv.x, m, a.accumulate != 0, o.x);
+        f.y = lerp_bwd_first(gv.y, m, a.accumulate != 0, o.y);
         *dvf = f;
-        gv.x = gv.x * (1.0f - m);
-        gv.y = gv.y * (1.0f - m);
+        gv.x = lerp_bwd_self(gv.x, m);
+        gv.y = lerp_bwd_self(gv.y, m);
         *reinterpret_cast<float2*>(g) = gv;
       } else if (a.first_layer && a.accumulate) {
         const float2 o = *dvf;
@@ -480,7 +472,7 @@
   }
   if (a.mix_col >= 0) {
     for (int o = a.dh >> 2; o > 0; o >>= 1) dm += __shfl_xor(dm, o, 64);
-    if (valid && seg == 2 && j == 0) a.dproj[(int64_t)t * a.n_qkv + a.mix_col + h] = dm * (1.0f - m) * m;
+    if (valid && seg == 2 && j == 0) a.dproj[(int64_t)t * a.n_qkv + a.mix_col + h] = mix_dlogit(dm, m);
   }
 }
 
@@ -1067,6 +1059,50 @@
   return p;
 }
 
+const float2* rot_table(const XtrlTrainDesc* D) {
+  return (D->rot_tab && D->rot_tab_n >= D->n) ? reinterpret_cast<const float2*>(D->rot_tab) : nullptr;
+}
+
+AttnFold attn_fold(const Ctx& c, const XtrlTrainLayer& Ly, int mix_col, float* dproj, int first_layer,
+                   int accumulate) {
+  const XtrlTrainDesc* D = c.D;
+  AttnFold f;
+  f.proj = Ly.proj;
+  f.ldp = Ly.n_qkv;
+  f.vfirst = D->layers[0].proj;
+  f.ld_vfirst = D->layers[0].n_qkv;
+  f.dproj = dproj;
+  f.dvfirst = D->dvfirst;
+  f.inv_freq = D->inv_freq;
+  f.rot_tab = D->rot_tab;
+  f.rot_tab_n = D->rot_tab_n;
+  f.rot_dim = D->rot_dim;
+  f.mix_col = mix_col;
+  f.first_layer = first_layer;
+  f.accumulate = accumulate;
+  f.qk_norm = D->qk_norm;
+  f.xpos_base = D->xpos_base;
+  return f;
+}
+
+std::unordered_set<const float*>& qkv_stale() {
+  static std::unordered_set<const float*> set;
+  return set;
+}
+
+int qkv_prep(const Ctx& c, const XtrlTrainLayer& Ly, int mix_col) {
+  const XtrlTrainDesc* D = c.D;
+  const int32_t* rows = D->packed ? D->vrows : nullptr;
+  const int I = D->H * D->dh, Ikv = kv_heads(D) * D->dh, nq3 = I + 2 * Ikv;
+  PrepArgs pa{Ly.proj, D->layers[0].proj, Ly.qkv, D->inv_freq, c.T, D->n, D->H, D->dh, I, Ly.n_qkv,
+              D->layers[0].n_qkv, D->rot_dim, mix_col, D->qk_norm, D->xpos_base, rows, Ikv, rot_table(D)};
+  const dim3 pg = rows ? dim3(blocks(nq3 / 2, PREP_T), c.T) : dim3(blocks(nq3 / 2, PREP_T), D->n, D->b);
+  hipLaunchKernelGGL(k_qkv_prep, pg, dim3(PREP_T), 0, c.s, pa);
+  XTRL_LAUNCHED("train qkv_prep");
+  qkv_stale().erase(Ly.qkv);
+  return XTRL_OK;
+}
+
 int validate(const XtrlTrainDesc* D) {
   XTRL_REQUIRE(D && D->layers && D->flat && D->grad, "train: null descriptor / layers / parameters");
   XTRL_REQUIRE(D->b > 0 && D->n > 0 && D->d > 0 && D->L > 0 && D->H > 0 && D->dh > 0, "train: bad sizes");
@@ -1312,15 +1348,19 @@
                          EPI_NONE, nullptr, nullptr, 0, 1 << 30, nq3)))
       return rc;
     const int mix_col = Ly.mix ? nq3 + (D->gate_values ? I : 0) : -1;
-    PrepArgs pa{Ly.proj, D->layers[0].proj, Ly.qkv, D->inv_freq, T, D->n, D->H, D->dh, I, Ly.n_qkv,
-                D->layers[0].n_qkv, D->rot_dim, mix_col, D->qk_norm, D->xpos_base, rows, Ikv};
-    const dim3 pg = rows ? dim3(blocks(nq3 / 2, PREP_T), T) : dim3(blocks(nq3 / 2, PREP_T), D->n, D->b);
-    hipLaunchKernelGGL(k_qkv_prep, pg, dim3(PREP_T), 0, s, pa);
-    XTRL_LAUNCHED("train qkv_prep");
     const AttnProblem ap = attn_problem(c, Ly, li);
-    if ((rc = attn_fwd_ex(ap, Ly.qkv, Ly.qkv + I, Ly.qkv + I + Ikv, Ly.o, Ly.lse,
-                          D->gate_values ? Ly.proj + nq3 : nullptr, D->gate_values ? Ly.og : nullptr, s)))
-      return rc;
+    const AttnFold af = attn_fold(c, Ly, mix_col, nullptr, 0, 0);
+    if (attn_fold_ok(ap, af)) {
+      if ((rc = attn_fwd_fold(ap, af, Ly.o, Ly.lse, D->gate_values ? Ly.proj + nq3 : nullptr,
+                              D->gate_values ? Ly.og : nullptr, s)))
+        return rc;
+      qkv_stale().insert(Ly.qkv);
+    } else {
+      if ((rc = qkv_prep(c, Ly, mix_col))) return rc;
+      if ((rc = attn_fwd_ex(ap, Ly.qkv, Ly.qkv + I, Ly.qkv + I + Ikv, Ly.o, Ly.lse,
+                            D->gate_values ? Ly.proj + nq3 : nullptr, D->gate_values ? Ly.og : nullptr, s)))
+        return rc;
+    }
     if (fuse) {
       if ((rc = linear_res_ln(c, D->gate_values ? Ly.og : Ly.o, I, c.P(Ly.w_out), nullptr, Ly.x_attn, Ly.x_ff, I,
                               c.P(Ly.ln_ff), Ly.xn_ff, d, nullptr, 0, Ly.st_ff)))
@@ -1483,9 +1523,6 @@
       if ((rc = linear_dgrad(c, xg, d, c.P(Ly.w_out), D->dog, I, T, d, I, EPI_NONE))) return rc;
     }
     const AttnProblem ap = attn_problem(c, Ly, li);
-    if ((rc = attn_bwd_ex(ap, Ly.qkv, Ly.qkv + I, Ly.qkv + I + Ikv, Ly.o, Ly.lse, D->dog, dproj, dproj + I,
-                          dproj + I + Ikv, D->delta, s)))
-      return rc;
     const int mix_col = Ly.mix ? nq3 + (D->gate_values ? I : 0) : -1;
     const bool any_mix = [&] {
       for (int j = 1; j < D->L; ++j)
@@ -1494,12 +1531,23 @@
     }();
     bool deeper_mix = false;
     for (int j = li + 1; j < D->L; ++j) deeper_mix = deeper_mix || D->layers[j].mix;
-    PrepBwdArgs pb{dproj, Ly.proj, D->layers[0].proj, D->dvfirst, D->inv_freq, T, D->n, D->H, D->dh, I,
-                   Ly.n_qkv, D->layers[0].n_qkv, D->rot_dim, mix_col, li == 0 ? 1 : 0,
-                   (li == 0 ? any_mix : deeper_mix) ? 1 : 0, D->qk_norm, D->xpos_base, rows, Ikv};
-    const dim3 pg = rows ? dim3(blocks(nq3 / 2, PREP_T), T) : dim3(blocks(nq3 / 2, PREP_T), D->n, D->b);
-    hipLaunchKernelGGL(k_qkv_prep_bwd, pg, dim3(PREP_T), 0, s, pb);
-    XTRL_LAUNCHED("train qkv_prep_bwd");
+    const int first_layer = li == 0 ? 1 : 0, accumulate = (li == 0 ? any_mix : deeper_mix) ? 1 : 0;
+    const AttnFold af = attn_fold(c, Ly, mix_col, dproj, first_layer, accumulate);
+    if (attn_fold_ok(ap, af)) {
+      if ((rc = attn_bwd_fold(ap, af, Ly.o, Ly.lse, D->dog, D->delta, s))) return rc;
+    } else {
+      if (qkv_stale().count(Ly.qkv))
+        if ((rc = qkv_prep(c, Ly, mix_col))) return rc;
+      if ((rc = attn_bwd_ex(ap, Ly.qkv, Ly.qkv + I, Ly.qkv + I + Ikv, Ly.o, Ly.lse, D->dog, dproj, dproj + I,
+                            dproj + I + Ikv, D->delta, s)))
+        return rc;
+      PrepBwdArgs pb{dproj, Ly.proj, D->layers[0].proj, D->dvfirst, D->inv_freq, T, D->n, D->H, D->dh, I,
+                     Ly.n_qkv, D->layers[0].n_qkv, D->rot_dim, mix_col, first_layer, accumulate, D->qk_norm,
+                     D->xpos_base, rows, Ikv, rot_table(D)};
+      const dim3 pg = rows ? dim3(blocks(nq3 / 2, PREP_T), T) : dim3(blocks(nq3 / 2, PREP_T), D->n, D->b);
+      hipLaunchKernelGGL(k_qkv_prep_bwd, pg, dim3(PREP_T), 0, s, pb);
+      XTRL_LAUNCHED("train qkv_prep_bwd");
+    }
     if ((rc = F.fork())) return rc;
     if ((rc = wgrad(cw, dproj, Ly.n_qkv, Ly.xn_attn, d, c.G(Ly.w_proj), T, Ly.n_qkv, d, c.G(Ly.b_proj), nq3)))
       return rc;
@@ -2082,6 +2130,39 @@
   return xtrl::glu_bwd(dh, lddh, u, ldu, du, lddu, M, ff, p, seed, offset, layer, xtrl::as_stream(stream));
 }
 
+extern "C" int xtrl_qkv_prep(const float* proj, int n_qkv, const float* vfirst, int ld_vfirst, float* qkv,
+                             const float* inv_freq, const float* rot_tab, int rot_tab_n, int b, int n, int H, int dh,
+                             int rot_dim, int mix_col, void* stream) {
+  XTRL_REQUIRE(proj && qkv && b > 0 && n > 0 && H > 0 && dh > 0 && n_qkv >= 3 * H * dh, "qkv_prep: bad arguments");
+  XTRL_REQUIRE(mix_col < 0 || vfirst, "qkv_prep: the value mix needs vfirst");
+  XTRL_REQUIRE(rot_dim == 0 || inv_freq || (rot_tab && rot_tab_n >= n), "qkv_prep: rotary without inv_freq or a table");
+  const int I = H * dh;
+  const float2* tab = (rot_tab && rot_tab_n >= n) ? reinterpret_cast<const float2*>(rot_tab) : nullptr;
+  xtrl::PrepArgs pa{proj, vfirst, qkv, inv_freq, b * n, n, H, dh, I, n_qkv, ld_vfirst, rot_dim, mix_col, 0, 0.f, nullptr,
+                    I, tab};
+  hipLaunchKernelGGL(xtrl::k_qkv_prep, dim3(xtrl::blocks(3 * I / 2, xtrl::PREP_T), n, b), dim3(xtrl::PREP_T), 0,
+                     xtrl::as_stream(stream), pa);
+  XTRL_LAUNCHED("qkv_prep");
+  return XTRL_OK;
+}
+
+extern "C" int xtrl_qkv_prep_bwd(float* dproj, const float* proj, int n_qkv, const float* vfirst, int ld_vfirst,
+                                 float* dvfirst, const float* inv_freq, const float* rot_tab, int rot_tab_n, int b, int n,
+                                 int H, int dh, int rot_dim, int mix_col, int first_layer, int accumulate, void* stream) {
+  XTRL_REQUIRE(dproj && proj && b > 0 && n > 0 && H > 0 && dh > 0 && n_qkv >= 3 * H * dh, "qkv_prep_bwd: bad arguments");
+  XTRL_REQUIRE(dvfirst || (mix_col < 0 && !(first_layer && accumulate)), "qkv_prep_bwd: null dvfirst");
+  XTRL_REQUIRE(mix_col < 0 || vfirst, "qkv_prep_bwd: the value mix needs vfirst");
+  XTRL_REQUIRE(rot_dim == 0 || inv_freq || (rot_tab && rot_tab_n >= n), "qkv_prep_bwd: rotary without inv_freq or a table");
+  const int I = H * dh;
+  const float2* tab = (rot_tab && rot_tab_n >= n) ? reinterpret_cast<const float2*>(rot_tab) : nullptr;
+  xtrl::PrepBwdArgs pb{dproj, proj, vfirst, dvfirst, inv_freq, b * n, n, H, dh, I, n_qkv, ld_vfirst, rot_dim, mix_col,
+                       first_layer, accumulate, 0, 0.f, nullptr, I, tab};
+  hipLaunchKernelGGL(xtrl::k_qkv_prep_bwd, dim3(xtrl::blocks(3 * I / 2, xtrl::PREP_T), n, b), dim3(xtrl::PREP_T), 0,
+                     xtrl::as_stream(stream), pb);
+  XTRL_LAUNCHED("qkv_prep_bwd");
+  return XTRL_OK;
+}
+
 extern "C" int xtrl_ff_dropout_mask(uint8_t* mask, int M, int N, float p, uint64_t seed, uint32_t offset,
                                     uint32_t layer, void* stream) {
   XTRL_REQUIRE(layer < (1u << 22), "ff_dropout_mask: layer %u out of range", layer);
diff --git a/x-transformers-rl_amd/xtrl_amd/_lib.py b/x-transformers-rl_amd/xtrl_amd/_lib.py
--- a/x-transformers-rl_amd/xtrl_amd/_lib.py
+++ b/x-transformers-rl_amd/xtrl_amd/_lib.py
@@ -7,7 +7,7 @@
 import torch
 
 LIB_PATH = Path(os.environ.get('XTRL_LIB', Path(__file__).resolve().parent / 'libxtrl_hip.so'))
-ABI_VERSION = 25
+ABI_VERSION = 26
 
 P = C.c_void_p
 I32, I64, U32, U64, F32 = C.c_int, C.c_int64, C.c_uint32, C.c_uint64, C.c_float
@@ -116,6 +116,7 @@
                    ('packed', I32), ('ep_off', P), ('pack_ws', P), ('pack_ws_floats', I64), ('attn_window', I32),
                    ('Hkv', I32), ('wimg', P), ('wimg_bytes', I64), ('wimg_tab', P),
                    ('wimg_tab_host', C.POINTER(WimgEntry)), ('wimg_n', I32),
+                   ('rot_tab_n', I32), ('rot_tab', P),
                    ('num_mem_kv', I32), ('add_zero_kv', I32), ('sink_ws', P), ('sink_ws_floats', I64)])
 
 
@@ -201,6 +202,16 @@
                                I32, P]),
     'xtrl_ema_lerp': (I32, [P, P, I64, F32, P]),
     'xtrl_sim_reset': (I32, [P, I32, I32, U64, U32, P, P]),
+    'xtrl_rotary_table': (I32, [P, I32, I32, P, P]),
+    'xtrl_qkv_prep': (I32, [P, I32, P, I32, P, P, P, I32, I32, I32, I32, I32, I32, I32, P]),
+    'xtrl_qkv_prep_bwd': (I32, [P, P, I32, P, I32, P, P, P, I32, I32, I32, I32, I32, I32, I32, I32, I32, P]),
+    'xtrl_attn_fwd_rows': (I32, [P, P, P, P, P, I32, P, I32, I32, I32, I32, F32, F32, U64, U32, U32, P]),
+    'xtrl_attn_bwd_rows': (I32, [P, P, P, P, P, P, I32, P, I32, I32, I32, I32, F32, F32, U64, U32, U32, P]),
+    'xtrl_attn_fwd_fold': (I32, [P, I32, P, I32, P, P, P, I32, P, P, P, I32, I32, I32, I32, I32, I32, I32, F32, F32, U64,
+                                 U32, U32, P]),
+    'xtrl_attn_bwd_fold': (I32, [P, I32, P, I32, P, P, P, P, P, P, P, P, P, I32, I32, I32, I32, I32, I32, I32, I32, I32,
+                                 F32, F32, U64, U32, U32, P]),
+    'xtrl_attn_fold_launch_count': (I64, []),
     'xtrl_train_forward': (I32, [C.POINTER(TrainDesc), P]),
     'xtrl_train_backward': (I32, [C.POINTER(TrainDesc), P]),
     'xtrl_ff_dropout_mask': (I32, [P, I32, I32, F32, U64, U32, U32, P]),
diff --git a/x-transformers-rl_amd/xtrl_amd/ops.py b/x-transformers-rl_amd/xtrl_amd/ops.py
--- a/x-transformers-rl_amd/xtrl_amd/ops.py
+++ b/x-transformers-rl_amd/xtrl_amd/ops.py
@@ -181,6 +181,16 @@
     return out
 
 
+
+
+def rotary_table(inv_freq, n_max):
+    half = int(inv_freq.numel())
+    if half == 0 or n_max <= 0:
+        return None
+    _f32c(inv_freq)
+    out = torch.empty(n_max, half, 2, device=inv_freq.device, dtype=torch.float32)
+    L.check(L.lib().xtrl_rotary_table(L.ptr(inv_freq), half, int(n_max), L.ptr(out), L.stream()), 'rotary_table')
+    return out
 
 
 def kv_head_index(heads, kv_heads, device=None):
diff --git a/x-transformers-rl_amd/xtrl_amd/train.py b/x-transformers-rl_amd/xtrl_amd/train.py
--- a/x-transformers-rl_amd/xtrl_amd/train.py
+++ b/x-transformers-rl_amd/xtrl_amd/train.py
@@ -174,6 +174,10 @@
             self.sink_ws = E(int(L.lib().xtrl_attn_sink_ws_floats(b_max, H, D.num_mem_kv, dh)))
             D.sink_ws, D.sink_ws_floats = self.sink_ws.data_ptr(), self.sink_ws.numel()
         D.inv_freq = self.inv_freq.data_ptr()
+        from .ops import rotary_table
+        self.rot_tab = rotary_table(self.inv_freq, n_max)
+        if self.rot_tab is not None:
+            D.rot_tab, D.rot_tab_n = self.rot_tab.data_ptr(), n_max
         for k, t in self.buf.items():
             setattr(D, k, t.data_ptr())
         D.part_floats = self.buf['part'].numel()
```

New measurement: 447,000 env-steps/s, median of 6. No clear change (+0.5%).
